# Ryan-Faulkner/Simultaneous-Diffusion-for-Pointclouds

Hardware: AMD Instinct MI355X
Metric: Langevin denoising steps/sec on 64×1024 range images, 1/2/4/8 MI355X (higher is better)
Workload: dtype fp32x3; 1 GPU; Line.yml simultaneous sampling step (score-net fwd + Langevin update + consistency merge), 64x1024x2 range images; views_per_gpu=4, megabatch_views=4, mode=viewsplit, conv_arithmetic=fp32x3, parallelism=views1

## Files before the change

simultaneous-diffusion-for-pointclouds_amd/csrc/common.h:

```cpp
#pragma once
#include <hip/hip_runtime.h>
#include <stdint.h>
#include <stdlib.h>

#include <type_traits>

#define SDP_DEV __device__ __forceinline__

typedef __attribute__((ext_vector_type(8))) __bf16 bf16x8;
typedef __attribute__((ext_vector_type(4))) __bf16 bf16x4;
typedef __attribute__((ext_vector_type(16))) float f32x16;
typedef __attribute__((ext_vector_type(4))) float f32x4;

namespace sdp {

template <int B, int E, class F>
SDP_DEV void static_for(F&& f) {
  if constexpr (B < E) {
    f(std::integral_constant<int, B>{});
    static_for<B + 1, E>(f);
  }
}

enum { MODE_F32 = 0, MODE_F32X3 = 1, MODE_BF16 = 2 };
enum { PRO_NONE = 0, PRO_ELU = 1, PRO_AFFINE_ELU = 2 };

typedef __attribute__((ext_vector_type(4))) int i32x4;
SDP_DEV i32x4 buffer_desc(const void* base, uint32_t bytes) {
  const uint64_t p = reinterpret_cast<uint64_t>(base);
  return i32x4{__builtin_amdgcn_readfirstlane((int)(uint32_t)p), __builtin_amdgcn_readfirstlane((int)((p >> 32) & 0xffff)),
               __builtin_amdgcn_readfirstlane((int)bytes), 0x00020000};
}
SDP_DEV void dma16_lds_opaque(i32x4 rsrc, uint32_t lds_byte, int voff, int soff) {
  asm volatile("s_mov_b32 m0, %0\n\ts_nop 0\n\tbuffer_load_dwordx4 %1, %2, %3 offen lds"
               :
               : "s"(__builtin_amdgcn_readfirstlane((int)lds_byte)), "v"(voff), "s"(rsrc),
                 "s"(__builtin_amdgcn_readfirstlane(soff))
               : "memory");
}

SDP_DEV float4 ldg4(const float* p, size_t i) { return *reinterpret_cast<const float4*>(p + i); }
SDP_DEV float4 bf4_to_f4(uint2 u) {
  return make_float4(__uint_as_float(u.x << 16), __uint_as_float(u.x & 0xffff0000u), __uint_as_float(u.y << 16),
                     __uint_as_float(u.y & 0xffff0000u));
}
SDP_DEV float4 ldg4(const __bf16* p, size_t i) { return bf4_to_f4(*reinterpret_cast<const uint2*>(p + i)); }
SDP_DEV uint32_t pack_bf2(float a, float b) {
  typedef __attribute__((ext_vector_type(2))) __bf16 bf16x2_t;
  const bf16x2_t v = {(__bf16)a, (__bf16)b};
  return __builtin_bit_cast(uint32_t, v);
}
SDP_DEV uint2 f4_to_bf4(float4 v) { return make_uint2(pack_bf2(v.x, v.y), pack_bf2(v.z, v.w)); }
SDP_DEV void stg4(float* p, size_t i, float4 v) { *reinterpret_cast<float4*>(p + i) = v; }
SDP_DEV void stg4(__bf16* p, size_t i, float4 v) { *reinterpret_cast<uint2*>(p + i) = f4_to_bf4(v); }
SDP_DEV float ldg1(const float* p, size_t i) { return p[i]; }
SDP_DEV float ldg1(const __bf16* p, size_t i) { return (float)p[i]; }

SDP_DEV float elu(float x) { return x > 0.f ? x : (__expf(x) - 1.0f); }
SDP_DEV float elu_max(float x) { return fmaxf(x, __expf(fminf(x, 0.f)) - 1.0f); }
SDP_DEV float elu_grad(float t, int form) {
  if (form == 2) return t > 0.f ? 1.f : t + 1.f;
  return t > 0.f ? 1.f : __expf(t);
}

struct ConvArgs {
  const float* in;
  const uint4* wf;
  const uint4* wf16;
  const float* bias;
  float* out;
  const float* res;
  float* out2;
  const float* res2;
  const float* up;
  const float* pro_ss;
  int ss_bstride;
  float* stats;
  int B, H, W, Cin, Cout;
  int dil, circular, pro_mode, epi_elu;
  int tiles_per_img;
  int strip_w;
  int groups_per_img;
  int cpair;
  unsigned long long* dbg;
  const float* aux;
  const float* epi_ss;
  int dact;
  int io16;
};

struct WgradArgs {
  const float* in;
  const float* pro_ss;
  int ss_bstride;
  int pro_mode;
  const float* dy;
  float* part;
  size_t part_floats;
  float* bpart;
  int B, H, W, Cin, Cout, dil, circular;
};

inline int conv_strip_w(int tile_rows, int tile_cols) {
  int sw = 1;
  while (sw * 2 * tile_rows <= 32 && tile_cols % (sw * 2) == 0) sw *= 2;
  return sw;
}

}
```

simultaneous-diffusion-for-pointclouds_amd/csrc/conv.hip:

```cpp
#include "conv_launch.h"

namespace sdp {

#ifndef SDP_CONV_NJ2
#define SDP_CONV_NJ2 1
#endif
#ifndef SDP_CONV_NJ2_BF16_W8
#define SDP_CONV_NJ2_BF16_W8 1
#endif

template <int MODE, bool PELU>
static hipError_t launch_elu(const ConvArgs& a, int ks, bool pool, int wm, int tc, bool half, hipStream_t st) {
  if (ks == 1)
    return pool ? conv_launch<MODE, 1, 64, 1, true, PELU>(a, st) : conv_launch<MODE, 1, 64, 1, false, PELU>(a, st);
  if (pool) return conv_launch<MODE, 1, 64, 3, true, PELU>(a, st);
  if constexpr (MODE != MODE_F32) {
    if (half) return SDP_CONV_NJ2 ? conv_launch_nj2<MODE, PELU, 4>(a, st) : conv_launch_half<MODE, PELU>(a, st);
    if (tc == 16) {
      if (!SDP_CONV_NJ2) return conv_launch<MODE, 1, 16, 3, false, PELU>(a, st);
      return (MODE == MODE_BF16 && SDP_CONV_NJ2_BF16_W8) ? conv_launch_nj2<MODE, PELU, 8>(a, st)
                                                         : conv_launch_nj2<MODE, PELU, 4>(a, st);
    }
  }
  if (wm == 2) return conv_launch<MODE, 2, 32, 3, false, PELU>(a, st);
  return tc == 64 ? conv_launch<MODE, 1, 64, 3, false, PELU>(a, st) : conv_launch<MODE, 1, 32, 3, false, PELU>(a, st);
}

template <int MODE>
static hipError_t launch_mode(const ConvArgs& a, int ks, bool pool, int wm, int tc, hipStream_t st, bool half = false) {
#ifdef SDP_CONV_BENCH_ONLY
  if constexpr (MODE != MODE_F32) {
    if (half) return SDP_CONV_NJ2 ? conv_launch_nj2<MODE, true, 4>(a, st) : conv_launch_half<MODE, true>(a, st);
    if (!SDP_CONV_NJ2) return conv_launch<MODE, 1, 16, 3, false, true>(a, st);
    return (MODE == MODE_BF16 && SDP_CONV_NJ2_BF16_W8) ? conv_launch_nj2<MODE, true, 8>(a, st)
                                                       : conv_launch_nj2<MODE, true, 4>(a, st);
  }
  if (wm == 2) return conv_launch<MODE, 2, 32, 3, false, true>(a, st);
  return conv_launch<MODE, 1, 32, 3, false, true>(a, st);
#else
  return a.pro_mode == PRO_NONE ? launch_elu<MODE, false>(a, ks, pool, wm, tc, half, st)
                                : launch_elu<MODE, true>(a, ks, pool, wm, tc, half, st);
#endif
}

hipError_t conv_mfma(int mode, ConvArgs a, int ks, bool pool, hipStream_t st, const char** why) {
  const int d = a.dil;
  if (a.Cin % 64 || a.Cout % 128) { *why = "conv: Cin%64 and Cout%128 required"; return hipErrorInvalidValue; }
  if (a.H % d || a.W % d) { *why = "conv: H,W must be multiples of the dilation"; return hipErrorInvalidValue; }
  const int Hs = a.H / d, Ws = a.W / d;
  const int wm = (a.Cout % 256 == 0) ? 1 : 2;
  const bool sh16 = mode != MODE_F32;
  int tc;
  if (sh16 && Ws % 16 == 0 && Hs % 8 == 0) tc = 16;
  else if (wm == 2) tc = 32;
  else tc = (Ws % 32 == 0 && Hs % 4 == 0) ? 32 : 64;
  if (!sh16 && tc == 16) tc = 32;
  if (ks == 1 || pool) tc = 64;
  const bool half = sh16 && wm == 2 && tc == 16 && ks == 3 && !pool;
  const int tr = (half ? 128 : wm * 128) / tc;
  if (Ws % tc || Hs % tr) { *why = "conv: sub-grid not divisible by the pixel tile"; return hipErrorInvalidValue; }
  if (sh16 && !a.wf16) { *why = "conv: bf16 modes need the 16x16 weight packing (#frag16)"; return hipErrorInvalidValue; }
  if (!sh16 && !a.wf) { *why = "conv: exact fp32 needs the 32x32 weight packing (#frag)"; return hipErrorInvalidValue; }
  if (ks == 1 && !pool && (d != 1 || wm != 1)) { *why = "conv: 1x1 needs d=1 and 256-multiple Cout"; return hipErrorInvalidValue; }
  if (pool && (d != 1 || wm != 1 || (a.H & 1) || (a.W & 1))) {
    *why = "conv: pooling needs d=1, even H,W and 256-multiple Cout";
    return hipErrorInvalidValue;
  }
  if (a.up && ((a.H & 1) || (a.W & 1) || a.H < 2 || a.W < 2)) { *why = "conv: upsample needs even H,W"; return hipErrorInvalidValue; }
  if (!a.circular && d != 1) { *why = "conv: zero padding only for d=1"; return hipErrorInvalidValue; }
  if (!a.pro_ss) { *why = "conv: prologue scale/shift table missing"; return hipErrorInvalidValue; }
  if (a.Cin > 1024 && a.ss_bstride == 0) { *why = "conv: identity table holds 1024 channels"; return hipErrorInvalidValue; }
  if (a.io16) {
#ifdef SDP_CONV_BENCH_ONLY
    if (mode == MODE_BF16 && ks == 3 && tc == 16 && !pool) return conv_launch_nj2<MODE_BF16, true, 4, true>(a, st);
#else
    if (mode != MODE_BF16) { *why = "conv: bf16 tensors (io16) need bf16 mode"; return hipErrorInvalidValue; }
    const bool pe = a.pro_mode != PRO_NONE;
    if (pool && ks == 1) return pe ? conv_launch<MODE_BF16, 1, 64, 1, true, true, true>(a, st)
                                   : conv_launch<MODE_BF16, 1, 64, 1, true, false, true>(a, st);
    if (pool) return pe ? conv_launch<MODE_BF16, 1, 64, 3, true, true, true>(a, st)
                        : conv_launch<MODE_BF16, 1, 64, 3, true, false, true>(a, st);
    if (ks == 3 && tc == 16)
      return pe ? conv_launch_nj2<MODE_BF16, true, 4, true>(a, st) : conv_launch_nj2<MODE_BF16, false, 4, true>(a, st);
#endif
    *why = "conv: no bf16-tensor (io16) kernel for this shape";
    return hipErrorInvalidValue;
  }
  switch (mode) {
    case MODE_F32: return launch_mode<MODE_F32>(a, ks, pool, wm, tc, st);
    case MODE_F32X3: return launch_mode<MODE_F32X3>(a, ks, pool, wm, tc, st, half);
    default: return launch_mode<MODE_BF16>(a, ks, pool, wm, tc, st, half);
  }
}

}
```

simultaneous-diffusion-for-pointclouds_amd/csrc/conv_inst.hip:

```cpp
#include "conv_kernel.h"
#include "conv_launch.h"

namespace sdp {


#ifndef SDP_FWD_TRN
#define SDP_FWD_TRN 0
#endif

#ifndef SDP_CONV_CPAIR
#define SDP_CONV_CPAIR 1
#endif

#ifndef SDP_NJ2_STRIP
#define SDP_NJ2_STRIP 1
#endif

template <int MODE, int WM, int TC, int KS, bool POOL, bool PELU, bool IO16>
hipError_t conv_launch(ConvArgs a, hipStream_t st) {
  using T = ConvTile<WM, TC, KS, 4, 4, IO16>;
  a.tiles_per_img = a.H * a.W / (T::TR * TC);
  a.groups_per_img = a.H * a.W / 128;
  a.strip_w = conv_strip_w(a.H / a.dil / T::TR, a.W / a.dil / TC);
  dim3 grid(a.B * a.tiles_per_img, a.Cout / T::NTILE);
  if constexpr (MODE != MODE_F32) {
    hipLaunchKernelGGL((conv_mfma_kernel<MODE, WM, TC, KS, POOL, POOL, PELU, 16, 4, (SDP_FWD_TRN && TC == 16 && !POOL), 4, IO16>),
                       grid, dim3(256), 0, st, a);
    return hipGetLastError();
  } else if constexpr (TC >= 32) {
    hipLaunchKernelGGL((conv_mfma_kernel<MODE, WM, TC, KS, POOL, POOL, PELU>), grid, dim3(256), 0, st, a);
    return hipGetLastError();
  }
  return hipErrorInvalidValue;
}

template <int MODE, bool PELU>
hipError_t conv_launch_half(ConvArgs a, hipStream_t st) {
  using T = ConvTile<1, 16, 3, 2>;
  a.tiles_per_img = a.H * a.W / (T::TR * 16);
  a.groups_per_img = a.H * a.W / 128;
  a.strip_w = 0;
  dim3 grid(a.B * a.tiles_per_img, a.Cout / T::NTILE);
  hipLaunchKernelGGL((conv_mfma_kernel<MODE, 1, 16, 3, false, false, PELU, 16, 2, (SDP_FWD_TRN != 0)>), grid,
                     dim3(T::NTH), 0, st, a);
  return hipGetLastError();
}

template <int MODE, bool PELU, int NW, bool IO16>
hipError_t conv_launch_nj2(ConvArgs a, hipStream_t st) {
  using T = ConvTile<1, 16, 3, NW, 2, IO16>;
  a.tiles_per_img = a.H * a.W / (T::TR * 16);
  a.groups_per_img = a.H * a.W / 128;
  a.cpair = (SDP_CONV_CPAIR && a.Cout == 2 * T::NTILE) ? 1 : 0;
  const bool strip = NW == 8 || SDP_NJ2_STRIP == 2 || (SDP_NJ2_STRIP == 1 && a.cpair);
  a.strip_w = strip ? conv_strip_w(a.H / a.dil / T::TR, a.W / a.dil / 16) : 0;
  dim3 grid(a.B * a.tiles_per_img * (a.cpair ? 2 : 1), a.cpair ? 1 : a.Cout / T::NTILE);
  hipLaunchKernelGGL((conv_mfma_kernel<MODE, 1, 16, 3, false, false, PELU, 16, NW, false, 2, IO16>), grid, dim3(T::NTH), 0,
                     st, a);
  return hipGetLastError();
}

template <int MODE, int WM, int TC, int KS, bool ZP, bool IO16>
hipError_t dgrad_launch(ConvArgs a, hipStream_t st) {
  using T = ConvTile<WM, TC, KS, 4, 4, IO16>;
  a.tiles_per_img = a.H * a.W / (T::TR * TC);
  a.groups_per_img = a.H * a.W / 128;
  dim3 grid(a.B * a.tiles_per_img, a.Cout / T::NTILE);
  if constexpr (TC < 32) {
    hipLaunchKernelGGL((conv_mfma_kernel<MODE, WM, TC, KS, false, ZP, false, 16, 4, true, 4, IO16>), grid, dim3(256), 0, st, a);
  } else {
    hipLaunchKernelGGL((conv_mfma_kernel<MODE, WM, TC, KS, false, ZP, false, 16, 4, false, 4, IO16>), grid, dim3(256), 0, st, a);
  }
  return hipGetLastError();
}

template <int S> struct FwdShape;
template <> struct FwdShape<0> { static constexpr int WM = 1, TC = 64, KS = 1; static constexpr bool POOL = true; };
template <> struct FwdShape<1> { static constexpr int WM = 1, TC = 64, KS = 3; static constexpr bool POOL = true; };
template <> struct FwdShape<2> { static constexpr int WM = 2, TC = 32, KS = 3; static constexpr bool POOL = false; };
template <> struct FwdShape<3> { static constexpr int WM = 1, TC = 64, KS = 3; static constexpr bool POOL = false; };
template <> struct FwdShape<4> { static constexpr int WM = 1, TC = 32, KS = 3; static constexpr bool POOL = false; };
template <> struct FwdShape<5> { static constexpr int WM = 1, TC = 16, KS = 3; static constexpr bool POOL = false; };
template <> struct FwdShape<8> { static constexpr int WM = 1, TC = 64, KS = 1; static constexpr bool POOL = false; };
template <int MODE>
hipError_t dgrad_launch_half(ConvArgs a, hipStream_t st) {
  using T = ConvTile<1, 16, 3, 2>;
  a.tiles_per_img = a.H * a.W / (T::TR * 16);
  a.groups_per_img = a.H * a.W / 128;
  dim3 grid(a.B * a.tiles_per_img, a.Cout / T::NTILE);
  hipLaunchKernelGGL((conv_mfma_kernel<MODE, 1, 16, 3, false, false, false, 16, 2, true>), grid, dim3(T::NTH), 0, st, a);
  return hipGetLastError();
}

template <int MODE, int NW, bool IO16>
hipError_t dgrad_launch_nj2(ConvArgs a, hipStream_t st) {
  using T = ConvTile<1, 16, 3, NW, 2, IO16>;
  a.tiles_per_img = a.H * a.W / (T::TR * 16);
  a.groups_per_img = a.H * a.W / 128;
  dim3 grid(a.B * a.tiles_per_img, a.Cout / T::NTILE);
  hipLaunchKernelGGL((conv_mfma_kernel<MODE, 1, 16, 3, false, false, false, 16, NW, true, 2, IO16>), grid, dim3(T::NTH), 0,
                     st, a);
  return hipGetLastError();
}

template <int S> struct DgradShape;
template <> struct DgradShape<0> { static constexpr int WM = 2, TC = 32, KS = 1; static constexpr bool ZP = false; };
template <> struct DgradShape<1> { static constexpr int WM = 2, TC = 32, KS = 3; static constexpr bool ZP = true; };
template <> struct DgradShape<2> { static constexpr int WM = 2, TC = 32, KS = 3; static constexpr bool ZP = false; };
template <> struct DgradShape<3> { static constexpr int WM = 1, TC = 64, KS = 3; static constexpr bool ZP = false; };
template <> struct DgradShape<4> { static constexpr int WM = 1, TC = 32, KS = 3; static constexpr bool ZP = false; };
template <> struct DgradShape<5> { static constexpr int WM = 1, TC = 16, KS = 3; static constexpr bool ZP = false; };

#if defined(SDP_INST) && SDP_INST >= 3000
constexpr int kS = SDP_INST % 10;
static_assert(kS == 0 || kS == 1 || kS == 7 || kS == 8, "SDP_INST: bad IO16 dgrad code");
#if SDP_INST % 10 == 0
template hipError_t dgrad_launch<MODE_BF16, 2, 32, 1, false, true>(ConvArgs, hipStream_t);
#elif SDP_INST % 10 == 1
template hipError_t dgrad_launch<MODE_BF16, 2, 32, 3, true, true>(ConvArgs, hipStream_t);
#else
template hipError_t dgrad_launch_nj2<MODE_BF16, kS == 7 ? 4 : 8, true>(ConvArgs, hipStream_t);
#endif
#elif defined(SDP_INST) && SDP_INST >= 2000
constexpr int kPelu = (SDP_INST / 10) % 10, kS = SDP_INST % 10;
static_assert(kPelu <= 1 && (kS == 0 || kS == 1 || kS == 6 || kS == 9), "SDP_INST: bad IO16 forward code");
#if SDP_INST % 10 == 0
template hipError_t conv_launch<MODE_BF16, 1, 64, 1, true, (kPelu != 0), true>(ConvArgs, hipStream_t);
#elif SDP_INST % 10 == 1
template hipError_t conv_launch<MODE_BF16, 1, 64, 3, true, (kPelu != 0), true>(ConvArgs, hipStream_t);
#else
template hipError_t conv_launch_nj2<MODE_BF16, (kPelu != 0), kS == 9 ? 4 : 8, true>(ConvArgs, hipStream_t);
#endif
#elif defined(SDP_INST) && SDP_INST < 1000 && (SDP_INST % 10 == 6 || SDP_INST % 10 == 9)
constexpr int kMode = SDP_INST / 100 - 1, kPelu = (SDP_INST / 10) % 10;
static_assert(kMode >= 1 && kMode <= 2 && kPelu <= 1, "SDP_INST: bad 32-Cout-wave forward code");
template hipError_t conv_launch_nj2<kMode, (kPelu != 0), SDP_INST % 10 == 9 ? 4 : 8>(ConvArgs, hipStream_t);
#elif defined(SDP_INST) && SDP_INST < 1000 && SDP_INST % 10 == 7
constexpr int kMode = SDP_INST / 100 - 1, kPelu = (SDP_INST / 10) % 10;
static_assert(kMode >= 1 && kMode <= 2 && kPelu <= 1, "SDP_INST: bad 2-wave forward code");
template hipError_t conv_launch_half<kMode, (kPelu != 0)>(ConvArgs, hipStream_t);
#elif defined(SDP_INST) && SDP_INST < 1000
constexpr int kMode = SDP_INST / 100 - 1, kPelu = (SDP_INST / 10) % 10, kShape = SDP_INST % 10;
static_assert(kMode >= 0 && kMode <= 2 && kPelu <= 1 && (kShape <= 5 || kShape == 8) &&
                  (kShape < 5 || kShape == 8 || kMode != MODE_F32),
              "SDP_INST: bad forward code");
using FS = FwdShape<kShape>;
template hipError_t conv_launch<kMode, FS::WM, FS::TC, FS::KS, FS::POOL, (kPelu != 0)>(ConvArgs, hipStream_t);
#elif defined(SDP_INST) && (SDP_INST % 10 == 7 || SDP_INST % 10 == 8)
constexpr int kMode = (SDP_INST / 10) % 10;
static_assert(SDP_INST / 100 == 10 && (kMode == MODE_F32X3 || kMode == MODE_BF16), "SDP_INST: bad dgrad code");
template hipError_t dgrad_launch_nj2<kMode, SDP_INST % 10 == 7 ? 4 : 8>(ConvArgs, hipStream_t);
#elif defined(SDP_INST) && SDP_INST % 10 == 6
constexpr int kMode = (SDP_INST / 10) % 10;
static_assert(SDP_INST / 100 == 10 && (kMode == MODE_F32X3 || kMode == MODE_BF16), "SDP_INST: bad dgrad code");
template hipError_t dgrad_launch_half<kMode>(ConvArgs, hipStream_t);
#elif defined(SDP_INST)
constexpr int kMode = (SDP_INST / 10) % 10, kShape = SDP_INST % 10;
static_assert(SDP_INST / 100 == 10 && (kMode == MODE_F32X3 || kMode == MODE_BF16) && kShape <= 5,
              "SDP_INST: bad dgrad code");
using DS = DgradShape<kShape>;
template hipError_t dgrad_launch<kMode, DS::WM, DS::TC, DS::KS, DS::ZP>(ConvArgs, hipStream_t);
#elif defined(SDP_CONV_BENCH_ONLY)
template hipError_t conv_launch<MODE_F32, 2, 32, 3, false, true>(ConvArgs, hipStream_t);
template hipError_t conv_launch<MODE_F32, 1, 32, 3, false, true>(ConvArgs, hipStream_t);
template hipError_t conv_launch<MODE_F32X3, 1, 16, 3, false, true>(ConvArgs, hipStream_t);
template hipError_t conv_launch<MODE_BF16, 1, 16, 3, false, true>(ConvArgs, hipStream_t);
template hipError_t conv_launch_half<MODE_F32X3, true>(ConvArgs, hipStream_t);
template hipError_t conv_launch_half<MODE_BF16, true>(ConvArgs, hipStream_t);
template hipError_t conv_launch_nj2<MODE_F32X3, true, 4>(ConvArgs, hipStream_t);
template hipError_t conv_launch_nj2<MODE_F32X3, true, 8>(ConvArgs, hipStream_t);
template hipError_t conv_launch_nj2<MODE_BF16, true, 4>(ConvArgs, hipStream_t);
template hipError_t conv_launch_nj2<MODE_BF16, true, 8>(ConvArgs, hipStream_t);
template hipError_t conv_launch_nj2<MODE_BF16, true, 4, true>(ConvArgs, hipStream_t);
template hipError_t dgrad_launch_nj2<MODE_BF16, 4, true>(ConvArgs, hipStream_t);
#else
#error "conv_inst.hip: build with -DSDP_INST=<code> (Makefile) or -DSDP_CONV_BENCH_ONLY (tools/conv_bench)"
#endif

}
```

simultaneous-diffusion-for-pointclouds_amd/csrc/conv_kernel.h:

```cpp
#pragma once
#include <type_traits>

#include "common.h"

namespace sdp {

#ifndef SDP_KO
#define SDP_KO 0
#endif

#ifndef SDP_DMA_AUX
#define SDP_DMA_AUX 0
#endif
#ifndef SDP_STORE_AUX
#define SDP_STORE_AUX 0
#endif
#ifndef SDP_STORE_AUX16
#define SDP_STORE_AUX16 SDP_STORE_AUX
#endif

#ifdef SDP_TIMING
#define SDP_T(i) do { if (tid == 0) tclk[i] = __builtin_amdgcn_s_memtime(); } while (0)
#else
#define SDP_T(i) do { } while (0)
#endif

constexpr int PSTRIDE = 144;

template <int WM, int TC, int KS, int NW = 4, int NJ = 4, bool IO16 = false>
struct ConvTile {
  static constexpr int NTH = 64 * NW;
  static constexpr int WN = NW / WM;
  static constexpr int RW = 128 / TC;
  static constexpr int TR = WM * RW;
  static constexpr int NTILE = WN * 16 * NJ;
  static constexpr int WPC = 4 * (NJ == 2 ? 2 : 1) / NW;
  static constexpr int HALO = KS == 3 ? 1 : 0;
  static constexpr int PC = TC + 2 * HALO;
  static constexpr int PR = TR + 2 * HALO;
  static constexpr int NPIX = PR * PC;
  static constexpr int UPP = IO16 ? 4 : 8;
  static constexpr int NU = (NPIX * UPP + NTH - 1) / NTH;
  static constexpr int PATCH_BYTES = NU * (NTH / UPP) * PSTRIDE;
  static constexpr int RAW_BYTES = NU * NTH * 16;
  static constexpr int PIPE_BYTES = 2 * PATCH_BYTES + RAW_BYTES;
  static constexpr int EPI_BYTES = WM * 64 * (NTILE + 8) * 4;
  static constexpr int LDS_BYTES = PIPE_BYTES > EPI_BYTES ? PIPE_BYTES : EPI_BYTES;
  static_assert(LDS_BYTES * WPC <= 160 * 1024, "LDS budget (WPC workgroups per CU)");
};

SDP_DEV float4 ld4(const float* p) { return *reinterpret_cast<const float4*>(p); }

template <int NU, int NT, int NSTG_ = 5>
struct XformPlan {
  static constexpr int tap_of(int k) { return k * NT / NU; }
  static constexpr int first(int tap) {
    int k = 0;
    while (k < NU && tap_of(k) < tap) ++k;
    return k;
  }
  static constexpr int count(int tap) {
    int n = 0;
    for (int k = 0; k < NU; ++k) n += tap_of(k) == tap ? 1 : 0;
    return n;
  }
  static constexpr int max_count() {
    int m = 0;
    for (int t = 0; t < NT; ++t) m = count(t) > m ? count(t) : m;
    return m;
  }
  static constexpr int NSTG = NSTG_;
  static constexpr int stage_blk(int q, int Q, int NBLK) { return 2 + q * (NBLK - 2) / (Q > 0 ? Q : 1); }
};

template <int MODE, int WM, int TC, int KS, bool POOL, bool ZP, bool PELU, int SH = 32, int NW = 4, bool TRN = false,
          int NJ = 4, bool IO16 = false>
__global__ __launch_bounds__(64 * NW, NJ == 2 ? 2 : 1) void conv_mfma_kernel(ConvArgs a) {
#if defined(__HIP_DEVICE_COMPILE__)
  static_assert(!IO16 || MODE == MODE_BF16, "the bf16 tape runs in bf16 mode");
  constexpr int ES = IO16 ? 2 : 4;
  constexpr int CPU = IO16 ? 8 : 4;
  constexpr int USH = IO16 ? 2 : 3;
  constexpr int PPU = CPU / 2;
  constexpr bool COPY = IO16 && !PELU;
  static_assert((SH == 32) == (MODE == MODE_F32), "bf16 modes: 16x16 shape; exact fp32: 32x32");
  static_assert(NW == 4 || (SH == 16 && !POOL), "2-wave workgroups: the 16x16 non-pooled forward only");
  static_assert(NJ == 4 || (SH == 16 && !POOL && KS == 3 && WM == 1), "32-Cout waves: the 16x16 3x3 tiles only");
  using T = ConvTile<WM, TC, KS, NW, NJ, IO16>;
  constexpr int NTH = T::NTH;
  constexpr int NT = KS * KS;
  constexpr bool TRANS = TRN && SH == 16 && !POOL;
  constexpr int NU = T::NU;
  constexpr int XT = NT >= 4 ? 4 : NT;
  __shared__ __attribute__((aligned(16))) char lds[T::LDS_BYTES];
  char* const raw = lds + 2 * T::PATCH_BYTES;

  const int tid = threadIdx.x, lane = tid & 63, wave = tid >> 6;
#ifdef SDP_TIMING
  unsigned long long tclk[8] = {0, 0, 0, 0, 0, 0, 0, 0};
  unsigned long long tbar = 0;
  const unsigned long long rt0 = __builtin_amdgcn_s_memrealtime();
#endif
  SDP_T(0);
  const int wm = WM == 1 ? 0 : (wave & 1), wn = WM == 1 ? wave : (wave >> 1);
  const int d = a.dil, Hs = a.H / d, Ws = a.W / d;
  const int tiles_c = Ws / TC, tiles_rc = (Hs / T::TR) * tiles_c;
  const int nwg = gridDim.x;
  int t = (nwg & 7) ? (int)blockIdx.x : ((int)blockIdx.x & 7) * (nwg >> 3) + ((int)blockIdx.x >> 3);
  const int cblk = a.cpair ? (t & 1) : (int)blockIdx.y;
  if (a.cpair) t >>= 1;
  const int b = t / a.tiles_per_img;
  const int tile = t - b * a.tiles_per_img;
  t = tile;
  const int ph = t / tiles_rc;
  t -= ph * tiles_rc;
  const int ph_r = ph / d, ph_c = ph - (ph / d) * d;
  int trow, tcol;
  if (a.strip_w) {
    const int R = Hs / T::TR, sw = a.strip_w;
    const int strip = t / (R * sw), w_ = t - strip * (R * sw);
    trow = w_ / sw;
    tcol = strip * sw + (w_ - trow * sw);
  } else {
    trow = t / tiles_c;
    tcol = t % tiles_c;
  }
  const int sr0 = trow * T::TR, sc0 = tcol * TC;
  const int n0 = cblk * T::NTILE;
  const int wrow0 = wm * T::RW;

  const int Cin = a.Cin, Cout = a.Cout;
  const int nchunks = Cin / 32;
  const int NB = Cout / 32;
  const int f0 = n0 / 16 + wn * NJ;
  const int nbg0 = f0 / 2;

  f32x16 acc[4][2];
  f32x4 acc4[8][NJ];
  if constexpr (SH == 32) {
    static_for<0, 4>([&](auto i) {
      static_for<0, 2>([&](auto j) {
#pragma unroll
        for (int r = 0; r < 16; ++r) acc[i][j][r] = 0.f;
      });
    });
  } else {
    static_for<0, 8>([&](auto i) {
      static_for<0, NJ>([&](auto j) {
#pragma unroll
        for (int r = 0; r < 4; ++r) acc4[i][j][r] = 0.f;
      });
    });
  }

  const bool c16 = SH == 16 && a.wf16 != nullptr;
  const __amdgpu_buffer_rsrc_t wrs =
      __builtin_amdgcn_make_buffer_rsrc((void*)(c16 ? a.wf16 : a.wf), 0, 0x7fffffff, 0x00020000);
  const int wv0 = ((nbg0 + 0) * 64 + lane) * 64, wv1 = ((nbg0 + 1) * 64 + lane) * 64;
  typedef __attribute__((ext_vector_type(4))) unsigned u32x4;
  constexpr int NBUF = (NT % 3 == 0) ? 3 : 2;
  uint4 bq[NBUF][NJ / 2][4];
  int wq16[NJ];
  const int wlo16 = __builtin_amdgcn_readfirstlane(c16 ? 1024 : 16);
  {
    const int g = lane >> 4, h = g & 1, sg = g >> 1;
    static_for<0, NJ>([&](auto njc) {
      constexpr int nj = decltype(njc)::value;
      const int L = 16 * (nj & 1) + (lane & 15) + 32 * h;
      wq16[nj] = c16 ? ((f0 + nj) * 128 + lane) * 16 : ((nbg0 + (nj >> 1)) * 64 + L) * 64 + sg * 32;
    });
  }
  auto load_b = [&](auto buf, int chunk, int tap) __attribute__((always_inline)) {
    constexpr int J = decltype(buf)::value;
    if constexpr (SDP_KO & 4) return;
    const int so = __builtin_amdgcn_readfirstlane(((chunk * NT + tap) * NB) * 4096);
    if constexpr (SH == 32) {
      static_for<0, 4>([&](auto q) {
        const u32x4 v0 = __builtin_amdgcn_raw_buffer_load_b128(wrs, wv0 + q * 16, so, 0);
        const u32x4 v1 = __builtin_amdgcn_raw_buffer_load_b128(wrs, wv1 + q * 16, so, 0);
        bq[J][0][q] = make_uint4(v0.x, v0.y, v0.z, v0.w);
        bq[J][1][q] = make_uint4(v1.x, v1.y, v1.z, v1.w);
      });
    } else {
      static_for<0, NJ>([&](auto njc) {
        constexpr int nj = decltype(njc)::value;
        const u32x4 vh = __builtin_amdgcn_raw_buffer_load_b128(wrs, wq16[nj], so, 0);
        bq[J][nj >> 1][2 * (nj & 1)] = make_uint4(vh.x, vh.y, vh.z, vh.w);
        if constexpr (MODE != MODE_BF16) {
          const u32x4 vl = __builtin_amdgcn_raw_buffer_load_b128(wrs, wq16[nj] + wlo16, so, 0);
          bq[J][nj >> 1][2 * (nj & 1) + 1] = make_uint4(vl.x, vl.y, vl.z, vl.w);
        }
      });
    }
  };

  const char* inb = reinterpret_cast<const char*>(a.in) + (size_t)b * a.H * a.W * Cin * ES;
  const float* ssb = a.pro_ss + (size_t)b * a.ss_bstride;
  const int my_cv = tid & (T::UPP - 1);
  float4 ssv[2][PPU];
  auto load_ss = [&](auto buf, int chunk) __attribute__((always_inline)) {
    constexpr int SB = decltype(buf)::value;
    static_for<0, PPU>([&](auto kc) { ssv[SB][kc] = ld4(ssb + (chunk * 32 + my_cv * CPU) * 2 + 4 * decltype(kc)::value); });
  };

  const __amdgpu_buffer_rsrc_t irs =
      __builtin_amdgcn_make_buffer_rsrc((void*)inb, 0, a.H * a.W * Cin * ES, 0x00020000);
  int uoff[NU];
  unsigned uvalid = 0;
  static_for<0, NU>([&](auto kc) {
    constexpr int k = decltype(kc)::value;
    int u = tid + k * NTH;
    bool valid = u < T::NPIX * T::UPP;
    u = valid ? u : 0;
    const int pix = u >> USH, cv = u & (T::UPP - 1);
    const int pr = pix / T::PC, pc = pix - pr * T::PC;
    int sr = sr0 - T::HALO + pr, sc = sc0 - T::HALO + pc;
    if (a.circular) {
      sr = sr < 0 ? sr + Hs : (sr >= Hs ? sr - Hs : sr);
      sc = sc < 0 ? sc + Ws : (sc >= Ws ? sc - Ws : sc);
    } else {
      valid = valid && sr >= 0 && sr < Hs && sc >= 0 && sc < Ws;
      sr = min(max(sr, 0), Hs - 1);
      sc = min(max(sc, 0), Ws - 1);
    }
    const int y = sr * d + ph_r, x = sc * d + ph_c;
    uoff[k] = ((y * a.W + x) * Cin + cv * CPU) * ES;
    uvalid |= (valid ? 1u : 0u) << k;
  });
  auto load_unit = [&](auto kc, int chunk) __attribute__((always_inline)) {
    constexpr int k = decltype(kc)::value;
    if constexpr (SDP_KO & 1) return;
    const int base = __builtin_amdgcn_readfirstlane(((tid & ~63) + k * NTH) * 16);
    __builtin_amdgcn_raw_ptr_buffer_load_lds(
        irs, reinterpret_cast<__attribute__((address_space(3))) void*>(reinterpret_cast<uintptr_t>(raw + base)), 16,
        uoff[k], chunk * 32 * ES, 0, SDP_DMA_AUX);
  };
  const i32x4 irs_o = buffer_desc(inb, (uint32_t)(a.H * a.W * Cin * ES));
  auto load_unit_o = [&](auto kc, int chunk) __attribute__((always_inline)) {
    constexpr int k = decltype(kc)::value;
    if constexpr (SDP_KO & 1) return;
    const uint32_t base = (uint32_t)(uintptr_t)(raw + ((tid & ~63) + k * NTH) * 16);
    dma16_lds_opaque(irs_o, base, uoff[k], chunk * 32 * ES);
  };
  auto xform_load = [&](auto kc) __attribute__((always_inline)) {
    constexpr int k = decltype(kc)::value;
    return *reinterpret_cast<const float4*>(raw + (tid + k * NTH) * 16);
  };
  auto xform_store = [&](auto kc, auto pb, float4 v) __attribute__((always_inline)) {
    constexpr int k = decltype(kc)::value;
    constexpr int PB = decltype(pb)::value;
    const int pix = (tid + k * NTH) >> USH;
    if constexpr (COPY) {
      uint4 u = __builtin_bit_cast(uint4, v);
      if constexpr (ZP) {
        if (!((uvalid >> k) & 1u)) u = make_uint4(0u, 0u, 0u, 0u);
      }
      *reinterpret_cast<uint4*>(lds + PB * T::PATCH_BYTES + pix * PSTRIDE + my_cv * 16) = u;
      return;
    }
    if constexpr (IO16) {
      const uint4 u = __builtin_bit_cast(uint4, v);
      const float4 lo = bf4_to_f4(make_uint2(u.x, u.y)), hi = bf4_to_f4(make_uint2(u.z, u.w));
      float x8[8] = {lo.x, lo.y, lo.z, lo.w, hi.x, hi.y, hi.z, hi.w};
#pragma unroll
      for (int e = 0; e < 8; ++e) {
        const float4 sv = ssv[PB][e >> 1];
        x8[e] = fmaf(x8[e], (e & 1) ? sv.z : sv.x, (e & 1) ? sv.w : sv.y);
        if constexpr (PELU) x8[e] = elu_max(x8[e]);
        if constexpr (ZP) {
          if (!((uvalid >> k) & 1u)) x8[e] = 0.f;
        }
      }
      *reinterpret_cast<uint4*>(lds + PB * T::PATCH_BYTES + pix * PSTRIDE + my_cv * 16) =
          make_uint4(pack_bf2(x8[0], x8[1]), pack_bf2(x8[2], x8[3]), pack_bf2(x8[4], x8[5]), pack_bf2(x8[6], x8[7]));
      return;
    }
    const float4 ssv0 = ssv[PB][0], ssv1 = ssv[PB][1];
    v.x = fmaf(v.x, ssv0.x, ssv0.y);
    v.y = fmaf(v.y, ssv0.z, ssv0.w);
    v.z = fmaf(v.z, ssv1.x, ssv1.y);
    v.w = fmaf(v.w, ssv1.z, ssv1.w);
    if constexpr (PELU) {
      v.x = elu_max(v.x); v.y = elu_max(v.y); v.z = elu_max(v.z); v.w = elu_max(v.w);
    }
    if constexpr (ZP) {
      if (!((uvalid >> k) & 1u)) v = make_float4(0.f, 0.f, 0.f, 0.f);
    }
    char* dst = lds + PB * T::PATCH_BYTES + pix * PSTRIDE;
    if constexpr (MODE == MODE_F32) {
      *reinterpret_cast<float4*>(dst + my_cv * 16) = v;
    } else {
      bf16x4 hi;
      hi[0] = (__bf16)v.x; hi[1] = (__bf16)v.y; hi[2] = (__bf16)v.z; hi[3] = (__bf16)v.w;
      *reinterpret_cast<bf16x4*>(dst + my_cv * 8) = hi;
      if constexpr (MODE == MODE_F32X3) {
        bf16x4 lo;
        lo[0] = (__bf16)(v.x - (float)hi[0]);
        lo[1] = (__bf16)(v.y - (float)hi[1]);
        lo[2] = (__bf16)(v.z - (float)hi[2]);
        lo[3] = (__bf16)(v.w - (float)hi[3]);
        *reinterpret_cast<bf16x4*>(dst + 64 + my_cv * 8) = lo;
      }
    }
  };
  auto xform_unit = [&](auto kc, auto pb) __attribute__((always_inline)) { xform_store(kc, pb, xform_load(kc)); };
  auto xform_piece = [&](auto kc, auto hc, auto pb, float4 v4) __attribute__((always_inline)) {
    constexpr int k = decltype(kc)::value, h = decltype(hc)::value, PB = decltype(pb)::value;
    if constexpr (SDP_KO & 2) return;
    const int pix = (tid + k * NTH) >> USH;
    float x0, x1;
    if constexpr (IO16) {
      const uint32_t w = __float_as_uint(h == 0 ? v4.x : h == 1 ? v4.y : h == 2 ? v4.z : v4.w);
      x0 = __uint_as_float(w << 16);
      x1 = __uint_as_float(w & 0xffff0000u);
    } else {
      x0 = h ? v4.z : v4.x;
      x1 = h ? v4.w : v4.y;
    }
    const float4 sv = ssv[PB][h];
    x0 = fmaf(x0, sv.x, sv.y);
    x1 = fmaf(x1, sv.z, sv.w);
    if constexpr (PELU) {
      x0 = elu_max(x0);
      x1 = elu_max(x1);
    }
    if constexpr (ZP) {
      const bool ok = (uvalid >> k) & 1u;
      x0 = ok ? x0 : 0.f;
      x1 = ok ? x1 : 0.f;
    }
    typedef __attribute__((ext_vector_type(2))) __bf16 bf16x2;
    bf16x2 hi;
    hi[0] = (__bf16)x0;
    hi[1] = (__bf16)x1;
    char* dst = lds + PB * T::PATCH_BYTES + pix * PSTRIDE + my_cv * (2 * CPU) + h * 4;
    *reinterpret_cast<bf16x2*>(dst) = hi;
    if constexpr (MODE == MODE_F32X3) {
      bf16x2 lo;
      lo[0] = (__bf16)(x0 - (float)hi[0]);
      lo[1] = (__bf16)(x1 - (float)hi[1]);
      *reinterpret_cast<bf16x2*>(dst + 64) = lo;
    }
  };

  SDP_T(1);
  load_b(std::integral_constant<int, 0>{}, 0, 0);
  static_for<1, NBUF - 1>([&](auto j) { load_b(j, 0, decltype(j)::value); });
  load_ss(std::integral_constant<int, 0>{}, 0);
  static_for<0, NU>([&](auto k) { load_unit(k, 0); });
  static_for<0, NU>([&](auto k) { xform_unit(k, std::integral_constant<int, 0>{}); });
  if (nchunks > 1) {
    load_ss(std::integral_constant<int, 1>{}, 1);
    static_for<0, NU>([&](auto k) { load_unit(k, 1); });
  }
  __syncthreads();
  SDP_T(2);

  const int a_lane_off16 = (lane & 15) * PSTRIDE + (lane >> 4) * 16;
  auto read_a = [&](const char* pat, auto tap_c, auto s_c, bf16x8* hi, bf16x8* lo) __attribute__((always_inline)) {
    constexpr int tap = decltype(tap_c)::value, s = decltype(s_c)::value;
    constexpr int kh = (KS == 3) ? tap / 3 : 0, kw = (KS == 3) ? tap % 3 : 0;
    static_for<0, 4>([&](auto mbc) {
      constexpr int i = decltype(mbc)::value, mb = 4 * s + i;
      constexpr int mr = mb / (TC / 16), mc = (mb % (TC / 16)) * 16;
      const char* src = pat + ((wrow0 + mr + kh) * T::PC + mc + kw) * PSTRIDE + a_lane_off16;
      hi[i] = *reinterpret_cast<const bf16x8*>(src);
      if constexpr (MODE == MODE_F32X3) lo[i] = *reinterpret_cast<const bf16x8*>(src + 64);
    });
  };

  auto do_chunk = [&](auto parity, int chunk) __attribute__((always_inline)) {
    constexpr int P = decltype(parity)::value;
    const char* pat = lds + P * T::PATCH_BYTES;
    bf16x8 pre_hi[4], pre_lo[4];
    if constexpr (MODE != MODE_F32) read_a(pat, std::integral_constant<int, 0>{}, std::integral_constant<int, 0>{},
                                           pre_hi, pre_lo);
    static_for<0, NT>([&](auto tap_c) {
      constexpr int tap = decltype(tap_c)::value;
      constexpr int DIST = NBUF - 1;
      constexpr int CUR = NBUF >= 3 ? tap % NBUF : (tap + P) & 1;
      constexpr int NXT = NBUF >= 3 ? (tap + DIST) % NBUF : (tap + 1 + P) & 1;
      if constexpr (tap + DIST < NT) load_b(std::integral_constant<int, NXT>{}, chunk, tap + DIST);
      else load_b(std::integral_constant<int, NXT>{}, min(chunk + 1, nchunks - 1), tap + DIST - NT);
      __builtin_amdgcn_sched_barrier(0);
      constexpr int NX = (tap < XT) ? (NU - tap + XT - 1) / XT : 0;
      float4 xv[NX > 0 ? NX : 1];
      auto xform_loads = [&]() __attribute__((always_inline)) {
        static_for<0, NX>([&](auto j) { xv[j] = xform_load(std::integral_constant<int, tap + XT * j>{}); });
      };
      auto xform_stores = [&]() __attribute__((always_inline)) {
        static_for<0, NX>([&](auto j) {
          xform_store(std::integral_constant<int, tap + XT * j>{}, std::integral_constant<int, 1 - P>{}, xv[j]);
        });
      };
      auto dmas = [&]() __attribute__((always_inline)) {
        if constexpr (tap == NT - 1) load_ss(std::integral_constant<int, P>{}, min(chunk + 2, nchunks - 1));
        static_for<0, NU>([&](auto kc) {
          constexpr int dt = NT > XT ? XT : 0;
          if constexpr (dt == tap) load_unit(kc, chunk + 2);
        });
      };
      if constexpr (MODE == MODE_F32) {
        xform_loads();
        xform_stores();
        if constexpr (NT == 1) __builtin_amdgcn_sched_barrier(0);
        dmas();
        const int kh = (KS == 3) ? tap / 3 : 0, kw = (KS == 3) ? tap % 3 : 0;
#pragma unroll
        for (int half = 0; half < 2; ++half) {
          float av[4][8];
          static_for<0, 4>([&](auto mbc) {
            constexpr int mb = decltype(mbc)::value;
            constexpr int mr = mb / (TC / 32), mc = (mb % (TC / 32)) * 32;
            const int pix = (wrow0 + mr + kh) * T::PC + mc + (lane & 31) + kw;
            const char* src = pat + pix * PSTRIDE + (lane >> 5) * 64 + half * 32;
            const float4 f0 = *reinterpret_cast<const float4*>(src);
            const float4 f1 = *reinterpret_cast<const float4*>(src + 16);
            av[mb][0] = f0.x; av[mb][1] = f0.y; av[mb][2] = f0.z; av[mb][3] = f0.w;
            av[mb][4] = f1.x; av[mb][5] = f1.y; av[mb][6] = f1.z; av[mb][7] = f1.w;
          });
#pragma unroll
          for (int kk = 0; kk < 8; ++kk) {
            const int k = half * 8 + kk;
            static_for<0, 2>([&](auto nbc) {
              constexpr int nb = decltype(nbc)::value;
              const uint4 bv = bq[CUR][nb][k >> 2];
              const uint32_t bw = (k & 3) == 0 ? bv.x : (k & 3) == 1 ? bv.y : (k & 3) == 2 ? bv.z : bv.w;
              const float bf = __uint_as_float(bw);
              static_for<0, 4>([&](auto mbc) {
                constexpr int mb = decltype(mbc)::value;
                acc[mb][nb] = __builtin_amdgcn_mfma_f32_32x32x2f32(av[mb][kk], bf, acc[mb][nb], 0, 0, 0);
              });
            });
          }
        }
      } else {
        float4 xv[NX > 0 ? NX : 1];
        static_for<0, NX>([&](auto j) { xv[j] = xform_load(std::integral_constant<int, tap + XT * j>{}); });
        bf16x8 c0_hi[4], c0_lo[4], c1_hi[4], c1_lo[4];
        static_for<0, 4>([&](auto mb) {
          c0_hi[mb] = pre_hi[mb];
          if constexpr (MODE == MODE_F32X3) c0_lo[mb] = pre_lo[mb];
        });
        read_a(pat, tap_c, std::integral_constant<int, 1>{}, c1_hi, c1_lo);
        if constexpr (tap + 1 < NT)
          read_a(pat, std::integral_constant<int, tap + 1>{}, std::integral_constant<int, 0>{}, pre_hi, pre_lo);
        if constexpr (NT > 1) dmas();
        constexpr int NBLK = 8 * NJ;
        static_for<0, NBLK>([&](auto blk_c) {
          constexpr int blk = decltype(blk_c)::value;
          {
            constexpr int s = blk / (4 * NJ), nj = (blk / 4) % NJ, i = blk & 3, mb = 4 * s + i;
            const uint4 h4 = bq[CUR][nj >> 1][2 * (nj & 1)], l4 = bq[CUR][nj >> 1][2 * (nj & 1) + 1];
            const bf16x8 bhi = *reinterpret_cast<const bf16x8*>(&h4);
            const bf16x8 blo = *reinterpret_cast<const bf16x8*>(&l4);
            const bf16x8 ahi = s == 0 ? c0_hi[i] : c1_hi[i];
            if constexpr (TRANS) {
              if constexpr (MODE == MODE_F32X3) {
                const bf16x8 alo = s == 0 ? c0_lo[i] : c1_lo[i];
                acc4[mb][nj] = __builtin_amdgcn_mfma_f32_16x16x32_bf16(bhi, alo, acc4[mb][nj], 0, 0, 0);
                acc4[mb][nj] = __builtin_amdgcn_mfma_f32_16x16x32_bf16(blo, ahi, acc4[mb][nj], 0, 0, 0);
              }
              acc4[mb][nj] = __builtin_amdgcn_mfma_f32_16x16x32_bf16(bhi, ahi, acc4[mb][nj], 0, 0, 0);
            } else {
              if constexpr (MODE == MODE_F32X3) {
                const bf16x8 alo = s == 0 ? c0_lo[i] : c1_lo[i];
                acc4[mb][nj] = __builtin_amdgcn_mfma_f32_16x16x32_bf16(alo, bhi, acc4[mb][nj], 0, 0, 0);
                acc4[mb][nj] = __builtin_amdgcn_mfma_f32_16x16x32_bf16(ahi, blo, acc4[mb][nj], 0, 0, 0);
              }
              acc4[mb][nj] = __builtin_amdgcn_mfma_f32_16x16x32_bf16(ahi, bhi, acc4[mb][nj], 0, 0, 0);
            }
          }
          if constexpr (COPY) {
            if constexpr (blk < NX) xform_store(std::integral_constant<int, tap + XT * blk>{}, std::integral_constant<int, 1 - P>{},
                                                xv[blk]);
          } else if constexpr (blk < PPU * NX) {
            xform_piece(std::integral_constant<int, tap + XT * (blk / PPU)>{}, std::integral_constant<int, blk % PPU>{},
                        std::integral_constant<int, 1 - P>{}, xv[blk / PPU]);
          }
          __builtin_amdgcn_sched_barrier(0);
        });
        if constexpr (NT == 1) dmas();
      }
    });
#ifdef SDP_TIMING
    const unsigned long long tb0 = __builtin_amdgcn_s_memtime();
#endif
    __builtin_amdgcn_s_waitcnt(0xc07f);
    if constexpr (!(SDP_KO & 8)) __builtin_amdgcn_s_barrier();
#ifdef SDP_TIMING
    tbar += __builtin_amdgcn_s_memtime() - tb0;
#endif
  };
  using XP = XformPlan<NU, NT, (MODE == MODE_BF16 && !IO16) ? 8 : 5>;
  constexpr int NQ = MODE == MODE_F32X3 ? 8 : 4;
  constexpr int NWL = NJ * (MODE == MODE_F32X3 ? 2 : 1);
  constexpr int NBLK = 8 * NJ;
  static_assert(NQ <= NBLK / 2 && 2 * NWL <= NBLK, "the tap's fillers fit its blocks");
  using I0 = std::integral_constant<int, 0>;
  using I1 = std::integral_constant<int, 1>;
  auto read_a1 = [&](const char* pat, auto tap_c, auto s_c, auto i_c, auto lo_c) __attribute__((always_inline)) {
    constexpr int tap = decltype(tap_c)::value, s = decltype(s_c)::value, i = decltype(i_c)::value;
    constexpr int kh = tap / 3, kw = tap % 3, mb = 4 * s + i;
    constexpr int mr = mb / (TC / 16), mc = (mb % (TC / 16)) * 16;
    return *reinterpret_cast<const bf16x8*>(pat + ((wrow0 + mr + kh) * T::PC + mc + kw) * PSTRIDE + a_lane_off16 +
                                            (decltype(lo_c)::value ? 64 : 0));
  };
  auto load_b1 = [&](auto buf, auto q_c, int chunk, int tap) __attribute__((always_inline)) {
    constexpr int J = decltype(buf)::value, q = decltype(q_c)::value;
    constexpr int nj = MODE == MODE_F32X3 ? (q >> 1) : q, part = MODE == MODE_F32X3 ? (q & 1) : 0;
    if constexpr (SDP_KO & 4) return;
    const int so = __builtin_amdgcn_readfirstlane(((chunk * NT + tap) * NB) * 4096 + (part ? wlo16 : 0));
    const u32x4 v = __builtin_amdgcn_raw_buffer_load_b128(wrs, wq16[nj], so, 0);
    bq[J][nj >> 1][2 * (nj & 1) + part] = make_uint4(v.x, v.y, v.z, v.w);
  };
  auto do_chunk9 = [&](auto parity, int chunk) __attribute__((always_inline)) {
    constexpr int P = decltype(parity)::value;
    const char* pat = lds + P * T::PATCH_BYTES;
    bf16x8 ca[2][4], cb[2][4];
    static_for<0, 4>([&](auto i) {
      ca[0][i] = read_a1(pat, I0{}, I0{}, i, I0{});
      if constexpr (MODE == MODE_F32X3) ca[1][i] = read_a1(pat, I0{}, I0{}, i, I1{});
    });
    load_ss(std::integral_constant<int, P>{}, min(chunk + 2, nchunks - 1));
    static_for<0, NT>([&](auto tap_c) {
      constexpr int tap = decltype(tap_c)::value;
      constexpr int CUR = tap % 3, NXT = (tap + 2) % 3;
      constexpr int U0 = XP::first(tap), UN = XP::count(tap), Q = COPY ? UN : UN * PPU * XP::NSTG;
      constexpr int UNA = UN > 0 ? UN : 1;
      const int wchunk = tap + 2 < NT ? chunk : min(chunk + 1, nchunks - 1);
      constexpr int wtap = tap + 2 < NT ? tap + 2 : tap + 2 - NT;
      float4 xr[UNA];
      float py0[PPU * UNA], py1[PPU * UNA], pe0[PPU * UNA], pe1[PPU * UNA];
      uint32_t phi[PPU * UNA], plo[PPU * UNA];
      auto stage = [&](auto pc_c, auto st_c) __attribute__((always_inline)) {
        constexpr int pc = decltype(pc_c)::value, st = decltype(st_c)::value;
        constexpr int j = pc / PPU, h = pc % PPU, k = U0 + j, PB = 1 - P;
        if constexpr (SDP_KO & 2) return;
        if constexpr (COPY) {
          xform_store(std::integral_constant<int, U0 + decltype(pc_c)::value>{}, std::integral_constant<int, PB>{},
                      xr[decltype(pc_c)::value]);
          return;
        }
        auto raw2 = [&](float& r0, float& r1) __attribute__((always_inline)) {
          const float4 v = xr[j];
          if constexpr (IO16) {
            const uint32_t w = __float_as_uint(h == 0 ? v.x : h == 1 ? v.y : h == 2 ? v.z : v.w);
            r0 = __uint_as_float(w << 16);
            r1 = __uint_as_float(w & 0xffff0000u);
          } else {
            r0 = h ? v.z : v.x;
            r1 = h ? v.w : v.y;
          }
        };
        if constexpr (XP::NSTG == 8) {
          const float4 v = xr[j];
          const float4 sv = ssv[PB][h];
          if constexpr (st == 0) {
            py0[pc] = fmaf(h ? v.z : v.x, sv.x, sv.y);
            if constexpr (PELU) pe0[pc] = fminf(py0[pc], 0.f);
          } else if constexpr (st == 1) {
            py1[pc] = fmaf(h ? v.w : v.y, sv.z, sv.w);
            if constexpr (PELU) pe1[pc] = fminf(py1[pc], 0.f);
          } else if constexpr (st == 2) {
            if constexpr (PELU) pe0[pc] = __expf(pe0[pc]);
          } else if constexpr (st == 3) {
            if constexpr (PELU) pe1[pc] = __expf(pe1[pc]);
          } else if constexpr (st == 4) {
            if constexpr (PELU) py0[pc] = fmaxf(py0[pc], pe0[pc] - 1.0f);
            if constexpr (ZP) py0[pc] = ((uvalid >> k) & 1u) ? py0[pc] : 0.f;
          } else if constexpr (st == 5) {
            if constexpr (PELU) py1[pc] = fmaxf(py1[pc], pe1[pc] - 1.0f);
            if constexpr (ZP) py1[pc] = ((uvalid >> k) & 1u) ? py1[pc] : 0.f;
          } else if constexpr (st == 6) {
            typedef __attribute__((ext_vector_type(2))) __bf16 bf16x2;
            bf16x2 hi;
            hi[0] = (__bf16)py0[pc];
            hi[1] = (__bf16)py1[pc];
            phi[pc] = *reinterpret_cast<const uint32_t*>(&hi);
          } else {
            const int pix = (tid + k * NTH) >> 3;
            *reinterpret_cast<uint32_t*>(lds + PB * T::PATCH_BYTES + pix * PSTRIDE + my_cv * 8 + h * 4) = phi[pc];
          }
          return;
        }
        if constexpr (st == 0) {
          float r0, r1;
          raw2(r0, r1);
          const float4 sv = ssv[PB][h];
          py0[pc] = fmaf(r0, sv.x, sv.y);
          py1[pc] = fmaf(r1, sv.z, sv.w);
          if constexpr (PELU) {
            pe0[pc] = fminf(py0[pc], 0.f);
            pe1[pc] = fminf(py1[pc], 0.f);
          }
        } else if constexpr (st == 1) {
          if constexpr (PELU) {
            pe0[pc] = __expf(pe0[pc]);
            pe1[pc] = __expf(pe1[pc]);
          }
        } else if constexpr (st == 2) {
          if constexpr (PELU) {
            py0[pc] = fmaxf(py0[pc], pe0[pc] - 1.0f);
            py1[pc] = fmaxf(py1[pc], pe1[pc] - 1.0f);
          }
          if constexpr (ZP) {
            const bool ok = (uvalid >> k) & 1u;
            py0[pc] = ok ? py0[pc] : 0.f;
            py1[pc] = ok ? py1[pc] : 0.f;
          }
        } else if constexpr (st == 3) {
          typedef __attribute__((ext_vector_type(2))) __bf16 bf16x2;
          bf16x2 hi;
          hi[0] = (__bf16)py0[pc];
          hi[1] = (__bf16)py1[pc];
          phi[pc] = *reinterpret_cast<const uint32_t*>(&hi);
          if constexpr (MODE == MODE_F32X3) {
            bf16x2 lo;
            lo[0] = (__bf16)(py0[pc] - (float)hi[0]);
            lo[1] = (__bf16)(py1[pc] - (float)hi[1]);
            plo[pc] = *reinterpret_cast<const uint32_t*>(&lo);
          }
        } else {
          const int pix = (tid + k * NTH) >> USH;
          char* dst = lds + PB * T::PATCH_BYTES + pix * PSTRIDE + my_cv * (2 * CPU) + h * 4;
          *reinterpret_cast<uint32_t*>(dst) = phi[pc];
          if constexpr (MODE == MODE_F32X3) *reinterpret_cast<uint32_t*>(dst + 64) = plo[pc];
        }
      };
      static_for<0, NBLK>([&](auto blk_c) {
        constexpr int blk = decltype(blk_c)::value;
        constexpr int s = blk / (4 * NJ), nj = (blk / 4) % NJ, i = blk & 3, mb = 4 * s + i;
        if constexpr (blk < UN) xr[blk] = xform_load(std::integral_constant<int, U0 + blk>{});
        {
          const uint4 h4 = bq[CUR][nj >> 1][2 * (nj & 1)], l4 = bq[CUR][nj >> 1][2 * (nj & 1) + 1];
          const bf16x8 bhi = *reinterpret_cast<const bf16x8*>(&h4);
          const bf16x8 blo = *reinterpret_cast<const bf16x8*>(&l4);
          const bf16x8 ahi = s == 0 ? ca[0][i] : cb[0][i];
          if constexpr (TRANS) {
            if constexpr (MODE == MODE_F32X3) {
              const bf16x8 alo = s == 0 ? ca[1][i] : cb[1][i];
              acc4[mb][nj] = __builtin_amdgcn_mfma_f32_16x16x32_bf16(bhi, alo, acc4[mb][nj], 0, 0, 0);
              acc4[mb][nj] = __builtin_amdgcn_mfma_f32_16x16x32_bf16(blo, ahi, acc4[mb][nj], 0, 0, 0);
            }
            acc4[mb][nj] = __builtin_amdgcn_mfma_f32_16x16x32_bf16(bhi, ahi, acc4[mb][nj], 0, 0, 0);
          } else {
            if constexpr (MODE == MODE_F32X3) {
              const bf16x8 alo = s == 0 ? ca[1][i] : cb[1][i];
              acc4[mb][nj] = __builtin_amdgcn_mfma_f32_16x16x32_bf16(alo, bhi, acc4[mb][nj], 0, 0, 0);
              acc4[mb][nj] = __builtin_amdgcn_mfma_f32_16x16x32_bf16(ahi, blo, acc4[mb][nj], 0, 0, 0);
            }
            acc4[mb][nj] = __builtin_amdgcn_mfma_f32_16x16x32_bf16(ahi, bhi, acc4[mb][nj], 0, 0, 0);
          }
        }
        if constexpr (blk < NQ) {
          constexpr int q = blk, ii = MODE == MODE_F32X3 ? (q >> 1) : q, lo = MODE == MODE_F32X3 ? (q & 1) : 0;
          cb[lo][ii] = read_a1(pat, tap_c, I1{}, std::integral_constant<int, ii>{}, std::integral_constant<int, lo>{});
        }
        if constexpr ((blk & 1) && (blk >> 1) < NWL)
          load_b1(std::integral_constant<int, NXT>{}, std::integral_constant<int, (blk >> 1)>{}, wchunk, wtap);
        if constexpr (tap + 1 < NT && blk >= NBLK / 2 && blk < NBLK / 2 + NQ) {
          constexpr int q = blk - NBLK / 2, ii = MODE == MODE_F32X3 ? (q >> 1) : q, lo = MODE == MODE_F32X3 ? (q & 1) : 0;
          ca[lo][ii] = read_a1(pat, std::integral_constant<int, tap + 1>{}, I0{}, std::integral_constant<int, ii>{},
                               std::integral_constant<int, lo>{});
        }
        static_for<0, Q>([&](auto q_c) {
          constexpr int q = decltype(q_c)::value;
          if constexpr (XP::stage_blk(q, Q, NBLK) == blk) {
            if constexpr (COPY) stage(std::integral_constant<int, q>{}, std::integral_constant<int, 0>{});
            else stage(std::integral_constant<int, q / XP::NSTG>{}, std::integral_constant<int, q % XP::NSTG>{});
          }
        });
        if constexpr (UN > 0 && blk >= NBLK - UN)
          load_unit_o(std::integral_constant<int, U0 + blk - (NBLK - UN)>{}, chunk + 2);
        __builtin_amdgcn_sched_barrier(0);
      });
    });
    __builtin_amdgcn_s_waitcnt(0xc07f);
    if constexpr (!(SDP_KO & 8)) __builtin_amdgcn_s_barrier();
  };
  static_assert(NT % 2 == 1, "parity bookkeeping assumes an odd tap count");
#ifndef SDP_DGRAD16_TAPS
#define SDP_DGRAD16_TAPS 0
#endif
  if constexpr (MODE != MODE_F32 && NT == 9 && (!TRANS || (IO16 && SDP_DGRAD16_TAPS))) {
    static_assert(XP::max_count() * PPU * XP::NSTG <= 2 * (NBLK - 2), "at most two transform stages per block");
    for (int chunk = 0; chunk < nchunks; chunk += 2) {
      do_chunk9(std::integral_constant<int, 0>{}, chunk);
      do_chunk9(std::integral_constant<int, 1>{}, chunk + 1);
    }
  } else {
    for (int chunk = 0; chunk < nchunks; chunk += 2) {
      do_chunk(std::integral_constant<int, 0>{}, chunk);
      do_chunk(std::integral_constant<int, 1>{}, chunk + 1);
    }
  }

  SDP_T(3);
  if (TRANS && (!a.dact || TC < 32 || NW != 4)) {
    if constexpr (TRANS) {
    __builtin_amdgcn_s_waitcnt(0);
    const int Ho = a.H, Wo = a.W;
    const size_t bo = (size_t)b * Ho * Wo * Cout;
    const int img_bytes = Ho * Wo * Cout * ES;
    auto rs = [&](const float* p) {
      return __builtin_amdgcn_make_buffer_rsrc((void*)(reinterpret_cast<const char*>(p) + bo * ES), 0, img_bytes, 0x00020000);
    };
    const int lq = lane >> 4, lcol = lane & 15;
    constexpr int CB = TC / 16;
    const int voff = (lcol * d * Cout + 4 * lq) * ES;
    auto soff = [&](int mb, int nj) {
      const int mr = mb / CB, mc = (mb % CB) * 16;
      const int y = (sr0 + wrow0 + mr) * d + ph_r, x = (sc0 + mc) * d + ph_c;
      return __builtin_amdgcn_readfirstlane(((y * Wo + x) * Cout + n0 + wn * 16 * NJ + nj * 16) * ES);
    };
    auto ld = [&](__amdgpu_buffer_rsrc_t r, int so) {
      if constexpr (IO16) {
        typedef __attribute__((ext_vector_type(2))) unsigned u32x2;
        const u32x2 q = __builtin_amdgcn_raw_buffer_load_b64(r, voff, so, 0);
        return bf4_to_f4(make_uint2(q.x, q.y));
      } else {
        const u32x4 q = __builtin_amdgcn_raw_buffer_load_b128(r, voff, so, 0);
        return make_float4(__uint_as_float(q.x), __uint_as_float(q.y), __uint_as_float(q.z), __uint_as_float(q.w));
      }
    };
    auto st = [&](float4 v, __amdgpu_buffer_rsrc_t r, int so, auto aux_c) {
      constexpr int AUX = decltype(aux_c)::value;
      if constexpr (IO16) {
        typedef __attribute__((ext_vector_type(2))) unsigned u32x2;
        const uint2 w = f4_to_bf4(v);
        __builtin_amdgcn_raw_buffer_store_b64(u32x2{w.x, w.y}, r, voff, so, AUX);
      } else {
        const u32x4 q = {__float_as_uint(v.x), __float_as_uint(v.y), __float_as_uint(v.z), __float_as_uint(v.w)};
        __builtin_amdgcn_raw_buffer_store_b128(q, r, voff, so, AUX);
      }
    };
    auto rs_or_out = [&](const float* p) { return rs(p ? p : a.out); };
    const __amdgpu_buffer_rsrc_t ors = rs(a.out), xrs = rs_or_out(a.aux), rrs = rs_or_out(a.res), o2rs = rs_or_out(a.out2),
                                 r2rs = rs_or_out(a.res2);
    static_for<0, NJ>([&](auto njc) {
      constexpr int nj = decltype(njc)::value;
      __builtin_amdgcn_sched_barrier(0);
      const int co0 = n0 + wn * 16 * NJ + nj * 16 + 4 * lq;
      float4 hq[8], rq[8], s0 = make_float4(1.f, 0.f, 1.f, 0.f), s1 = s0;
      if (a.dact) static_for<0, 8>([&](auto mb) { hq[mb] = ld(xrs, soff(mb, nj)); });
      if (a.dact == 3) {
        s0 = ld4(a.epi_ss + ((size_t)b * Cout + co0) * 2);
        s1 = ld4(a.epi_ss + ((size_t)b * Cout + co0) * 2 + 4);
      }
      if (a.res) static_for<0, 8>([&](auto mb) { rq[mb] = ld(rrs, soff(mb, nj)); });
      const float4 bias4 = a.bias ? ld4(a.bias + co0) : make_float4(0.f, 0.f, 0.f, 0.f);
      const float4 esc = make_float4(s0.x, s0.z, s1.x, s1.z), esh = make_float4(s0.y, s0.w, s1.y, s1.w);
      float4 v[8];
      static_for<0, 8>([&](auto mbc) {
        constexpr int mb = decltype(mbc)::value;
        const f32x4 q = acc4[mb][nj];
        v[mb] = make_float4(q[0] + bias4.x, q[1] + bias4.y, q[2] + bias4.z, q[3] + bias4.w);
      });
      if (a.up) {
        const int Hi = a.H / 2, Wi = a.W / 2;
        const float shh = (float)(Hi - 1) / (float)(a.H - 1), sww = (float)(Wi - 1) / (float)(a.W - 1);
        const size_t ub = (size_t)b * Hi * Wi * Cout + co0;
        auto lup = [&](size_t e) { return IO16 ? ldg4(reinterpret_cast<const __bf16*>(a.up), e) : ldg4(a.up, e); };
#pragma unroll
        for (int mb = 0; mb < 8; ++mb) {
          const int mr = mb / CB, mc = (mb % CB) * 16;
          const int y = (sr0 + wrow0 + mr) * d + ph_r, x = (sc0 + mc + lcol) * d + ph_c;
          const float fy = shh * (float)y, fx = sww * (float)x;
          const int y0 = (int)fy, x0 = (int)fx;
          const int yp = y0 < Hi - 1 ? 1 : 0, xp = x0 < Wi - 1 ? 1 : 0;
          const float ly1 = fy - (float)y0, ly0 = 1.f - ly1, lx1 = fx - (float)x0, lx0 = 1.f - lx1;
          const float4 v00 = lup(ub + ((size_t)y0 * Wi + x0) * Cout), v01 = lup(ub + ((size_t)y0 * Wi + x0 + xp) * Cout);
          const float4 v10 = lup(ub + ((size_t)(y0 + yp) * Wi + x0) * Cout);
          const float4 v11 = lup(ub + ((size_t)(y0 + yp) * Wi + x0 + xp) * Cout);
          auto bil = [&](float a00, float a01, float a10, float a11) {
            return ly0 * (lx0 * a00 + lx1 * a01) + ly1 * (lx0 * a10 + lx1 * a11);
          };
          v[mb].x = v[mb].x + bil(v00.x, v01.x, v10.x, v11.x);
          v[mb].y = v[mb].y + bil(v00.y, v01.y, v10.y, v11.y);
          v[mb].z = v[mb].z + bil(v00.z, v01.z, v10.z, v11.z);
          v[mb].w = v[mb].w + bil(v00.w, v01.w, v10.w, v11.w);
        }
      }
      if (a.dact) {
        static_for<0, 8>([&](auto mbc) {
          constexpr int mb = decltype(mbc)::value;
          float4 h = hq[mb];
          if (a.dact == 3) h = make_float4(fmaf(h.x, esc.x, esh.x), fmaf(h.y, esc.y, esh.y), fmaf(h.z, esc.z, esh.z),
                                           fmaf(h.w, esc.w, esh.w));
          v[mb] = make_float4(v[mb].x * elu_grad(h.x, a.dact), v[mb].y * elu_grad(h.y, a.dact),
                              v[mb].z * elu_grad(h.z, a.dact), v[mb].w * elu_grad(h.w, a.dact));
        });
      }
      if (a.res) {
        static_for<0, 8>([&](auto mbc) {
          constexpr int mb = decltype(mbc)::value;
          const float4 r = rq[mb];
          v[mb] = make_float4(r.x + v[mb].x, r.y + v[mb].y, r.z + v[mb].z, r.w + v[mb].w);
        });
      }
      if (a.out2) {
        static_for<0, 8>([&](auto mbc) {
          constexpr int mb = decltype(mbc)::value;
          const float4 r2 = ld(r2rs, soff(mb, nj));
          st(make_float4(v[mb].x + r2.x, v[mb].y + r2.y, v[mb].z + r2.z, v[mb].w + r2.w), o2rs, soff(mb, nj),
             std::integral_constant<int, 0>{});
        });
      }
      if (a.epi_elu) {
#pragma unroll
        for (int mb = 0; mb < 8; ++mb) v[mb] = make_float4(elu(v[mb].x), elu(v[mb].y), elu(v[mb].z), elu(v[mb].w));
      }
      if constexpr (!(SDP_KO & 16)) {
        static_for<0, 8>([&](auto mbc) {
          constexpr int mb = decltype(mbc)::value;
          st(v[mb], ors, soff(mb, nj), std::integral_constant<int, IO16 ? SDP_STORE_AUX16 : SDP_STORE_AUX>{});
        });
      }
      if (a.stats) {
        float mean[4], m2[4];
        static_for<0, 4>([&](auto rc) {
          constexpr int r = decltype(rc)::value;
          auto comp = [&](const float4& q) { return r == 0 ? q.x : r == 1 ? q.y : r == 2 ? q.z : q.w; };
          float s = 0.f;
#pragma unroll
          for (int mb = 0; mb < 8; ++mb) s += comp(v[mb]);
          mean[r] = s * 0.125f;
          float q2 = 0.f;
#pragma unroll
          for (int mb = 0; mb < 8; ++mb) {
            const float dv = comp(v[mb]) - mean[r];
            q2 = fmaf(dv, dv, q2);
          }
          m2[r] = q2;
        });
        auto merge = [&](auto ctl_c, float n) {
          constexpr int CTL = decltype(ctl_c)::value;
#pragma unroll
          for (int r = 0; r < 4; ++r) {
            const float mp = __int_as_float(__builtin_amdgcn_mov_dpp(__float_as_int(mean[r]), CTL, 0xf, 0xf, false));
            const float qp = __int_as_float(__builtin_amdgcn_mov_dpp(__float_as_int(m2[r]), CTL, 0xf, 0xf, false));
            const float dm = mean[r] - mp;
            m2[r] = m2[r] + qp + dm * dm * (0.5f * n);
            mean[r] = 0.5f * (mean[r] + mp);
          }
        };
        merge(std::integral_constant<int, 0xB1>{}, 8.f);
        merge(std::integral_constant<int, 0x4E>{}, 16.f);
        merge(std::integral_constant<int, 0x141>{}, 32.f);
        merge(std::integral_constant<int, 0x140>{}, 64.f);
        if (lcol == 0) {
          float4* sp = reinterpret_cast<float4*>(reinterpret_cast<float2*>(a.stats) +
                                                 ((size_t)b * a.groups_per_img + tile * WM + wm) * Cout + co0);
          sp[0] = make_float4(mean[0], m2[0], mean[1], m2[1]);
          sp[1] = make_float4(mean[2], m2[2], mean[3], m2[3]);
        }
      }
    });
    }
  } else if (SH == 16 && !TRANS && (!a.dact || TC < 32 || NW != 4)) {
    if constexpr (SH == 16 && !TRANS) {
    __builtin_amdgcn_s_waitcnt(0);
    const int Ho = POOL ? a.H / 2 : a.H, Wo = POOL ? a.W / 2 : a.W;
    const size_t bo = (size_t)b * Ho * Wo * Cout;
    const int img_bytes = Ho * Wo * Cout * ES;
    auto rs = [&](const float* p) {
      return __builtin_amdgcn_make_buffer_rsrc((void*)(reinterpret_cast<const char*>(p ? p : a.out) + bo * ES), 0, img_bytes,
                                               0x00020000);
    };
    const __amdgpu_buffer_rsrc_t ors = rs(a.out), rrs = rs(a.res), o2rs = rs(a.out2), r2rs = rs(a.res2), xrs = rs(a.aux);
    const int lq = lane >> 4, lcol = lane & 15;
    constexpr int CB = TC / 16;
    constexpr int NF = POOL ? CB : 8;
    constexpr int PER = POOL ? 2 : 4;
    constexpr int NV = NF * PER;
    const int xs = (POOL ? 1 : d) * Cout * ES;
    int vbase[NF];
    static_for<0, NF>([&](auto fc) {
      constexpr int f = decltype(fc)::value;
      const int co = n0 + wn * 16 * NJ + lcol;
      if constexpr (POOL) {
        vbase[f] = (((sr0 >> 1) * Wo + ((sc0 + f * 16) >> 1) + 2 * lq) * Cout + co) * ES;
      } else {
        constexpr int mr = f / CB, mc = (f % CB) * 16;
        const int y = (sr0 + wrow0 + mr) * d + ph_r, x = (sc0 + mc + 4 * lq) * d + ph_c;
        vbase[f] = ((y * Wo + x) * Cout + co) * ES;
      }
    });
#define SDP_EPI16_OFF(i, nj) vbase[(i) / PER], __builtin_amdgcn_readfirstlane(((i) % PER) * xs + (nj) * 16 * ES)
    auto ld1 = [&](__amdgpu_buffer_rsrc_t r, int vo, int so) __attribute__((always_inline)) {
      if constexpr (IO16) return __uint_as_float((uint32_t)__builtin_amdgcn_raw_buffer_load_b16(r, vo, so, 0) << 16);
      else return __uint_as_float(__builtin_amdgcn_raw_buffer_load_b32(r, vo, so, 0));
    };
    auto store_vals = [&](const float (&w)[NV], __amdgpu_buffer_rsrc_t r, auto nj_c, auto aux_c) __attribute__((always_inline)) {
      constexpr int NJC = decltype(nj_c)::value, AUX = decltype(aux_c)::value;
      if constexpr (IO16) {
        constexpr int HP = PER / 2;
        const bool odd = lane & 1;
#pragma unroll
        for (int f = 0; f < NF; ++f) {
          const int vb = vbase[f] + (odd ? HP * xs - 2 : 0);
#pragma unroll
          for (int k = 0; k < HP; ++k) {
            const float mine = odd ? w[f * PER + HP + k] : w[f * PER + k];
            const float send = odd ? w[f * PER + k] : w[f * PER + HP + k];
            const float got = __int_as_float(__builtin_amdgcn_mov_dpp(__float_as_int(send), 0xB1, 0xf, 0xf, false));
            const uint32_t pk = odd ? pack_bf2(got, mine) : pack_bf2(mine, got);
            __builtin_amdgcn_raw_buffer_store_b32(pk, r, vb, __builtin_amdgcn_readfirstlane(k * xs + NJC * 16 * ES), AUX);
          }
        }
      } else {
#pragma unroll
        for (int i = 0; i < NV; ++i) __builtin_amdgcn_raw_buffer_store_b32(__float_as_uint(w[i]), r, SDP_EPI16_OFF(i, NJC), AUX);
      }
    };
    float pre[NJ][NV], biasv[NJ];
    static_for<0, NJ>([&](auto nj) { biasv[nj] = a.bias ? a.bias[n0 + wn * 16 * NJ + nj * 16 + lcol] : 0.f; });
    if (a.res || a.out2) {
      const __amdgpu_buffer_rsrc_t prs = a.res ? rrs : r2rs;
      static_for<0, NJ>([&](auto njc) {
#pragma unroll
        for (int i = 0; i < NV; ++i) pre[njc][i] = ld1(prs, SDP_EPI16_OFF(i, decltype(njc)::value));
      });
    }
    static_for<0, NJ>([&](auto njc) {
      constexpr int nj = decltype(njc)::value;
      const int co = n0 + wn * 16 * NJ + nj * 16 + lcol;
      const float bias = biasv[nj];
      float v[NV];
      if constexpr (POOL) {
        static_for<0, CB>([&](auto fc) {
          constexpr int f = decltype(fc)::value;
          static_for<0, 2>([&](auto kc) {
            constexpr int k = decltype(kc)::value;
            const float a00 = acc4[f][nj][2 * k], a01 = acc4[f][nj][2 * k + 1];
            const float a10 = acc4[f + CB][nj][2 * k], a11 = acc4[f + CB][nj][2 * k + 1];
            v[f * 2 + k] = ((((a00 + bias) + (a10 + bias)) + (a01 + bias)) + (a11 + bias)) / 4.0f;
          });
        });
      } else {
        static_for<0, 8>([&](auto fc) {
          constexpr int f = decltype(fc)::value;
#pragma unroll
          for (int r = 0; r < 4; ++r) v[f * 4 + r] = acc4[f][nj][r] + bias;
        });
      }
      if (a.up) {
        const int Hi = a.H / 2, Wi = a.W / 2;
        const float shh = (float)(Hi - 1) / (float)(a.H - 1), sww = (float)(Wi - 1) / (float)(a.W - 1);
        const size_t ub = (size_t)b * Hi * Wi * Cout + co;
        auto lu = [&](size_t e) { return IO16 ? ldg1(reinterpret_cast<const __bf16*>(a.up), e) : ldg1(a.up, e); };
#pragma unroll
        for (int i = 0; i < NV; ++i) {
          const int f = i / PER, k = i % PER;
          const int mr = f / CB, mc = (f % CB) * 16;
          const int y = (sr0 + wrow0 + mr) * d + ph_r, x = (sc0 + mc + 4 * lq + k) * d + ph_c;
          const float fy = shh * (float)y, fx = sww * (float)x;
          const int y0 = (int)fy, x0 = (int)fx;
          const int yp = y0 < Hi - 1 ? 1 : 0, xp = x0 < Wi - 1 ? 1 : 0;
          const float ly1 = fy - (float)y0, ly0 = 1.f - ly1, lx1 = fx - (float)x0, lx0 = 1.f - lx1;
          const float v00 = lu(ub + ((size_t)y0 * Wi + x0) * Cout), v01 = lu(ub + ((size_t)y0 * Wi + x0 + xp) * Cout);
          const float v10 = lu(ub + ((size_t)(y0 + yp) * Wi + x0) * Cout);
          const float v11 = lu(ub + ((size_t)(y0 + yp) * Wi + x0 + xp) * Cout);
          v[i] = v[i] + (ly0 * (lx0 * v00 + lx1 * v01) + ly1 * (lx0 * v10 + lx1 * v11));
        }
      }
      if (a.dact) {
        float esc = 1.f, esh = 0.f;
        if (a.dact == 3) {
          esc = a.epi_ss[((size_t)b * Cout + co) * 2];
          esh = a.epi_ss[((size_t)b * Cout + co) * 2 + 1];
        }
#pragma unroll
        for (int i = 0; i < NV; ++i) {
          float h = ld1(xrs, SDP_EPI16_OFF(i, nj));
          if (a.dact == 3) h = fmaf(h, esc, esh);
          v[i] = v[i] * elu_grad(h, a.dact);
        }
      }
      if (a.res) {
#pragma unroll
        for (int i = 0; i < NV; ++i) v[i] = pre[nj][i] + v[i];
      }
      if (a.out2) {
        float r2[NV];
#pragma unroll
        for (int i = 0; i < NV; ++i)
          r2[i] = a.res ? ld1(r2rs, SDP_EPI16_OFF(i, nj)) : pre[nj][i];
#pragma unroll
        for (int i = 0; i < NV; ++i) r2[i] = v[i] + r2[i];
        store_vals(r2, o2rs, njc, std::integral_constant<int, 0>{});
      }
      if (a.epi_elu) {
#pragma unroll
        for (int i = 0; i < NV; ++i) v[i] = elu(v[i]);
      }
      if constexpr (!(SDP_KO & 16))
        store_vals(v, ors, njc, std::integral_constant<int, IO16 ? SDP_STORE_AUX16 : SDP_STORE_AUX>{});
      if (a.stats) {
        float sum = 0.f;
#pragma unroll
        for (int i = 0; i < NV; ++i) sum += v[i];
        float mean = sum * (1.0f / NV);
        float m2 = 0.f;
#pragma unroll
        for (int i = 0; i < NV; ++i) {
          const float dv = v[i] - mean;
          m2 = fmaf(dv, dv, m2);
        }
        float mp = __shfl_xor(mean, 16), qp = __shfl_xor(m2, 16), dm = mean - mp;
        m2 = m2 + qp + dm * dm * (0.5f * NV);
        mean = 0.5f * (mean + mp);
        mp = __shfl_xor(mean, 32);
        qp = __shfl_xor(m2, 32);
        dm = mean - mp;
        m2 = m2 + qp + dm * dm * (float)NV;
        mean = 0.5f * (mean + mp);
        if (lq == 0) {
          float2* st = reinterpret_cast<float2*>(a.stats) + ((size_t)b * a.groups_per_img + tile * WM + wm) * Cout + co;
          *st = make_float2(mean, m2);
        }
      }
    });
#undef SDP_EPI16_OFF
    }
  } else if (a.dact) {
    if constexpr (TC >= 32 && NW == 4 && SH == 16) {
    __builtin_amdgcn_s_waitcnt(0);
    __syncthreads();
    constexpr int SROW = T::NTILE + 8;
    constexpr int SP = WM * 64;
    constexpr int CG = T::NTILE / 4;
    constexpr int PL = 256 / CG;
    constexpr int NPO = POOL ? SP / 4 : SP;
    static_assert(SP * SROW * 4 <= T::LDS_BYTES, "epilogue staging fits the LDS");
    float* stage = reinterpret_cast<float*>(lds);
    const int cg = tid % CG, pl = tid / CG;
    const int co0 = n0 + cg * 4;
    const float4 bias4 = a.bias ? ld4(a.bias + co0) : make_float4(0.f, 0.f, 0.f, 0.f);
    float4 es0 = make_float4(1.f, 0.f, 1.f, 0.f), es1 = es0;
    if (a.dact == 3) {
      es0 = ld4(a.epi_ss + ((size_t)b * Cout + co0) * 2);
      es1 = ld4(a.epi_ss + ((size_t)b * Cout + co0) * 2 + 4);
    }
    const int Ho = POOL ? a.H / 2 : a.H, Wo = POOL ? a.W / 2 : a.W;
    using TA = std::conditional_t<IO16, __bf16, float>;
    auto tp = [](const float* p) { return reinterpret_cast<const TA*>(p); };
    TA* const outb = reinterpret_cast<TA*>(a.out) + (size_t)b * Ho * Wo * Cout;
    float4 sK[WM], s1[WM], s2[WM];
    int sn[WM];
    static_for<0, WM>([&](auto g) {
      sK[g] = make_float4(0.f, 0.f, 0.f, 0.f); s1[g] = sK[g]; s2[g] = sK[g]; sn[g] = 0;
    });
    static_for<0, 2>([&](auto hc) {
      constexpr int h = decltype(hc)::value;
      {
        if constexpr (!POOL && TRANS) {
          static_for<0, 4>([&](auto ic) {
            constexpr int i = decltype(ic)::value;
            static_for<0, 4>([&](auto njc) {
              constexpr int nj = decltype(njc)::value;
              float* dst = stage + (wm * 64 + 16 * i + (lane & 15)) * SROW + wn * 64 + nj * 16 + 4 * (lane >> 4);
              const f32x4 q = acc4[4 * h + i][nj];
              *reinterpret_cast<float4*>(dst) = make_float4(q[0], q[1], q[2], q[3]);
            });
          });
        } else if constexpr (!POOL) {
          static_for<0, 4>([&](auto ic) {
            constexpr int i = decltype(ic)::value;
            static_for<0, 4>([&](auto njc) {
              constexpr int nj = decltype(njc)::value;
              float* dst = stage + (wm * 64 + 16 * i + 4 * (lane >> 4)) * SROW + wn * 64 + nj * 16 + (lane & 15);
  #pragma unroll
              for (int r = 0; r < 4; ++r) dst[r * SROW] = acc4[4 * h + i][nj][r];
            });
          });
        }
      }
      __syncthreads();
      auto pix = [&](int j, int& y, int& x, int& g) __attribute__((always_inline)) {
        if constexpr (POOL) {
          y = (sr0 + wrow0) >> 1;
          x = (sc0 + 32 * h + 2 * j) >> 1;
          g = 0;
        } else {
          const int ws = j >> 6, q = j & 63;
          const int mb = 2 * h + (q >> 5);
          const int row = ws * T::RW + mb / (TC / 32), col = (mb % (TC / 32)) * 32 + (q & 31);
          y = (sr0 + row) * d + ph_r;
          x = (sc0 + col) * d + ph_c;
          g = ws;
        }
      };
      const size_t bo = (size_t)b * Ho * Wo * Cout;
      struct Ops { float4 h, r, q; };
      auto fetch = [&](int j) __attribute__((always_inline)) {
        Ops o;
        int y, x, g;
        pix(min(j, NPO - 1), y, x, g);
        const size_t oi = bo + ((size_t)y * Wo + x) * Cout + co0;
        o.h = a.aux ? ldg4(tp(a.aux), oi) : make_float4(0.f, 0.f, 0.f, 0.f);
        o.r = a.res ? ldg4(tp(a.res), oi) : make_float4(0.f, 0.f, 0.f, 0.f);
        o.q = a.out2 ? ldg4(tp(a.res2), oi) : make_float4(0.f, 0.f, 0.f, 0.f);
        return o;
      };
      Ops nx = fetch(pl);
      for (int j = pl; j < NPO; j += PL) {
        const Ops cu = nx;
        nx = fetch(j + PL);
        float4 v;
        int y, x, g;
        pix(j, y, x, g);
        if constexpr (POOL) {
          const float* s0 = stage + (2 * j) * SROW + cg * 4;
          const float4 o00 = ld4(s0), o01 = ld4(s0 + SROW), o10 = ld4(s0 + 32 * SROW), o11 = ld4(s0 + 33 * SROW);
          auto pool1 = [&](float a00, float a10, float a01, float a11, float bb) {
            return ((((a00 + bb) + (a10 + bb)) + (a01 + bb)) + (a11 + bb)) / 4.0f;
          };
          v.x = pool1(o00.x, o10.x, o01.x, o11.x, bias4.x);
          v.y = pool1(o00.y, o10.y, o01.y, o11.y, bias4.y);
          v.z = pool1(o00.z, o10.z, o01.z, o11.z, bias4.z);
          v.w = pool1(o00.w, o10.w, o01.w, o11.w, bias4.w);
        } else {
          const float4 o = ld4(stage + j * SROW + cg * 4);
          v = make_float4(o.x + bias4.x, o.y + bias4.y, o.z + bias4.z, o.w + bias4.w);
        }
        const size_t oidx = ((size_t)y * Wo + x) * Cout + co0;
        if (a.up) {
          const int Hi = a.H / 2, Wi = a.W / 2;
          const float sh = (float)(Hi - 1) / (float)(a.H - 1), sw = (float)(Wi - 1) / (float)(a.W - 1);
          const float fy = sh * (float)y, fx = sw * (float)x;
          const int y0 = (int)fy, x0 = (int)fx;
          const int yp = y0 < Hi - 1 ? 1 : 0, xp = x0 < Wi - 1 ? 1 : 0;
          const float ly1 = fy - (float)y0, ly0 = 1.f - ly1, lx1 = fx - (float)x0, lx0 = 1.f - lx1;
          const TA* ub = tp(a.up) + (size_t)b * Hi * Wi * Cout + co0;
          const float4 v00 = ldg4(ub, ((size_t)y0 * Wi + x0) * Cout), v01 = ldg4(ub, ((size_t)y0 * Wi + x0 + xp) * Cout);
          const float4 v10 = ldg4(ub, ((size_t)(y0 + yp) * Wi + x0) * Cout);
          const float4 v11 = ldg4(ub, ((size_t)(y0 + yp) * Wi + x0 + xp) * Cout);
          auto bil = [&](float a00, float a01, float a10, float a11) {
            return ly0 * (lx0 * a00 + lx1 * a01) + ly1 * (lx0 * a10 + lx1 * a11);
          };
          v.x = v.x + bil(v00.x, v01.x, v10.x, v11.x);
          v.y = v.y + bil(v00.y, v01.y, v10.y, v11.y);
          v.z = v.z + bil(v00.z, v01.z, v10.z, v11.z);
          v.w = v.w + bil(v00.w, v01.w, v10.w, v11.w);
        }
        if (a.dact) {
          float4 h4 = cu.h;
          if (a.dact == 3)
            h4 = make_float4(fmaf(h4.x, es0.x, es0.y), fmaf(h4.y, es0.z, es0.w), fmaf(h4.z, es1.x, es1.y),
                             fmaf(h4.w, es1.z, es1.w));
          v = make_float4(v.x * elu_grad(h4.x, a.dact), v.y * elu_grad(h4.y, a.dact), v.z * elu_grad(h4.z, a.dact),
                          v.w * elu_grad(h4.w, a.dact));
        }
        if (a.res) v = make_float4(cu.r.x + v.x, cu.r.y + v.y, cu.r.z + v.z, cu.r.w + v.w);
        if (a.out2)
          stg4(reinterpret_cast<TA*>(a.out2), bo + oidx, make_float4(v.x + cu.q.x, v.y + cu.q.y, v.z + cu.q.z, v.w + cu.q.w));
        if (a.epi_elu) v = make_float4(elu(v.x), elu(v.y), elu(v.z), elu(v.w));
        if constexpr (!(SDP_KO & 16)) stg4(outb, oidx, v);
        static_for<0, WM>([&](auto gc) {
          constexpr int gg = decltype(gc)::value;
          if (gg == g) {
            if (sn[gg] == 0) sK[gg] = v;
            const float4 dv = make_float4(v.x - sK[gg].x, v.y - sK[gg].y, v.z - sK[gg].z, v.w - sK[gg].w);
            s1[gg] = make_float4(s1[gg].x + dv.x, s1[gg].y + dv.y, s1[gg].z + dv.z, s1[gg].w + dv.w);
            s2[gg] = make_float4(fmaf(dv.x, dv.x, s2[gg].x), fmaf(dv.y, dv.y, s2[gg].y), fmaf(dv.z, dv.z, s2[gg].z),
                                 fmaf(dv.w, dv.w, s2[gg].w));
            ++sn[gg];
          }
        });
      }
      __syncthreads();
    });

    if (a.stats) {
      float2* part = reinterpret_cast<float2*>(lds);
      static_for<0, WM>([&](auto gc) {
        constexpr int gg = decltype(gc)::value;
        const float n = (float)sn[gg], inv = sn[gg] ? 1.f / n : 0.f;
        const float k4[4] = {sK[gg].x, sK[gg].y, sK[gg].z, sK[gg].w};
        const float a4[4] = {s1[gg].x, s1[gg].y, s1[gg].z, s1[gg].w};
        const float q4[4] = {s2[gg].x, s2[gg].y, s2[gg].z, s2[gg].w};
  #pragma unroll
        for (int c = 0; c < 4; ++c) {
          const float mean = k4[c] + a4[c] * inv;
          const float m2 = fmaxf(q4[c] - a4[c] * a4[c] * inv, 0.f);
          part[(gg * PL + pl) * T::NTILE + cg * 4 + c] = make_float2(mean, m2);
        }
      });
      __syncthreads();
      constexpr int PER = (POOL ? 32 : 128) / PL;
      for (int i = tid; i < WM * T::NTILE; i += 256) {
        const int gg = i / T::NTILE, co = i % T::NTILE;
        float mean = 0.f;
        for (int k = 0; k < PL; ++k) mean += part[(gg * PL + k) * T::NTILE + co].x;
        mean *= 1.f / PL;
        float m2 = 0.f;
        for (int k = 0; k < PL; ++k) {
          const float2 pk = part[(gg * PL + k) * T::NTILE + co];
          const float dm = pk.x - mean;
          m2 += pk.y + (float)PER * dm * dm;
        }
        float2* st = reinterpret_cast<float2*>(a.stats) + ((size_t)b * a.groups_per_img + tile * WM + gg) * Cout + n0 + co;
        *st = make_float2(mean, m2);
      }
    }
    }
  } else {
    if constexpr (SH == 32) {
    __builtin_amdgcn_s_waitcnt(0);
    {
      const int Ho = POOL ? a.H / 2 : a.H, Wo = POOL ? a.W / 2 : a.W;
      const size_t bo = (size_t)b * Ho * Wo * Cout;
      const int img_bytes = Ho * Wo * Cout * 4;
      auto rs = [&](const float* p) { return __builtin_amdgcn_make_buffer_rsrc((void*)(p ? p + bo : a.out + bo), 0, img_bytes, 0x00020000); };
      const __amdgpu_buffer_rsrc_t ors = rs(a.out), rrs = rs(a.res), xrs = rs(a.aux), o2rs = rs(a.out2), r2rs = rs(a.res2);
      const int lhalf = lane >> 5, lcol = lane & 31;
      constexpr int CB = TC / 32;
      constexpr int NV = POOL ? 16 : 64;
      constexpr int PER = POOL ? 8 : 16;
      const int xs = (POOL ? 1 : d) * Cout * 4;
      int vbase[POOL ? CB : 4];
      static_for<0, (POOL ? CB : 4)>([&](auto fc) {
        constexpr int f = decltype(fc)::value;
        const int co = n0 + wn * 64 + lcol;
        if constexpr (POOL) {
          vbase[f] = (((sr0 >> 1) * Wo + ((sc0 + f * 32) >> 1) + 2 * lhalf) * Cout + co) * 4;
        } else {
          constexpr int mr = f / CB, mc = (f % CB) * 32;
          const int y = (sr0 + wrow0 + mr) * d + ph_r, x = (sc0 + mc + 4 * lhalf) * d + ph_c;
          vbase[f] = ((y * Wo + x) * Cout + co) * 4;
        }
      });
      auto mstep = [](int k) { return POOL ? ((((k & 1) * 2 + (k >> 1) * 4) & 3) + 8 * (((k & 1) * 2 + (k >> 1) * 4) >> 2)) / 2
                                           : (k & 3) + 8 * (k >> 2); };
  #define SDP_EPI_OFF(i, nb) vbase[(i) / PER], __builtin_amdgcn_readfirstlane(mstep((i) % PER) * xs + (nb) * 128)
      float pre[2][NV], biasv[2];
      static_for<0, 2>([&](auto nb) { biasv[nb] = a.bias ? a.bias[n0 + wn * 64 + nb * 32 + lcol] : 0.f; });
      if (a.res || a.out2) {
        const __amdgpu_buffer_rsrc_t prs = a.res ? rrs : r2rs;
        static_for<0, 2>([&](auto nbc) {
  #pragma unroll
          for (int i = 0; i < NV; ++i)
            pre[nbc][i] = __uint_as_float(__builtin_amdgcn_raw_buffer_load_b32(prs, SDP_EPI_OFF(i, decltype(nbc)::value), 0));
        });
      }
      static_for<0, 2>([&](auto nbc) {
        constexpr int nb = decltype(nbc)::value;
        const int co = n0 + wn * 64 + nb * 32 + lcol;
        const float bias = biasv[nb];
        float v[NV];
        if constexpr (POOL) {
          static_for<0, CB>([&](auto mbc) {
            constexpr int mb = decltype(mbc)::value;
            static_for<0, 8>([&](auto kc) {
              constexpr int k = decltype(kc)::value;
              constexpr int r = (k & 1) * 2 + (k >> 1) * 4;
              const float a00 = acc[mb][nb][r], a01 = acc[mb][nb][r + 1];
              const float a10 = acc[mb + CB][nb][r], a11 = acc[mb + CB][nb][r + 1];
              v[mb * 8 + k] = ((((a00 + bias) + (a10 + bias)) + (a01 + bias)) + (a11 + bias)) / 4.0f;
            });
          });
        } else {
          static_for<0, 4>([&](auto mbc) {
            constexpr int mb = decltype(mbc)::value;
  #pragma unroll
            for (int r = 0; r < 16; ++r) v[mb * 16 + r] = acc[mb][nb][r] + bias;
          });
        }
        if (a.up) {
          const int Hi = a.H / 2, Wi = a.W / 2;
          const float shh = (float)(Hi - 1) / (float)(a.H - 1), sww = (float)(Wi - 1) / (float)(a.W - 1);
          const float* ub = a.up + (size_t)b * Hi * Wi * Cout + co;
  #pragma unroll
          for (int i = 0; i < NV; ++i) {
            const int f = i / PER, k = i % PER;
            const int mr = f / CB, mc = (f % CB) * 32;
            const int y = (sr0 + wrow0 + mr) * d + ph_r, x = (sc0 + mc + 4 * lhalf + mstep(k)) * d + ph_c;
            const float fy = shh * (float)y, fx = sww * (float)x;
            const int y0 = (int)fy, x0 = (int)fx;
            const int yp = y0 < Hi - 1 ? 1 : 0, xp = x0 < Wi - 1 ? 1 : 0;
            const float ly1 = fy - (float)y0, ly0 = 1.f - ly1, lx1 = fx - (float)x0, lx0 = 1.f - lx1;
            const float v00 = ub[((size_t)y0 * Wi + x0) * Cout], v01 = ub[((size_t)y0 * Wi + x0 + xp) * Cout];
            const float v10 = ub[((size_t)(y0 + yp) * Wi + x0) * Cout];
            const float v11 = ub[((size_t)(y0 + yp) * Wi + x0 + xp) * Cout];
            v[i] = v[i] + (ly0 * (lx0 * v00 + lx1 * v01) + ly1 * (lx0 * v10 + lx1 * v11));
          }
        }
        if (a.dact) {
          float esc = 1.f, esh = 0.f;
          if (a.dact == 3) {
            esc = a.epi_ss[((size_t)b * Cout + co) * 2];
            esh = a.epi_ss[((size_t)b * Cout + co) * 2 + 1];
          }
  #pragma unroll
          for (int i = 0; i < NV; ++i) {
            float h = __uint_as_float(__builtin_amdgcn_raw_buffer_load_b32(xrs, SDP_EPI_OFF(i, nb), 0));
            if (a.dact == 3) h = fmaf(h, esc, esh);
            v[i] = v[i] * elu_grad(h, a.dact);
          }
        }
        if (a.res) {
  #pragma unroll
          for (int i = 0; i < NV; ++i) v[i] = pre[nb][i] + v[i];
        }
        if (a.out2) {
          float r2[NV];
  #pragma unroll
          for (int i = 0; i < NV; ++i)
            r2[i] = a.res ? __uint_as_float(__builtin_amdgcn_raw_buffer_load_b32(r2rs, SDP_EPI_OFF(i, nb), 0)) : pre[nb][i];
  #pragma unroll
          for (int i = 0; i < NV; ++i) __builtin_amdgcn_raw_buffer_store_b32(__float_as_uint(v[i] + r2[i]), o2rs, SDP_EPI_OFF(i, nb), 0);
        }
        if (a.epi_elu) {
  #pragma unroll
          for (int i = 0; i < NV; ++i) v[i] = elu(v[i]);
        }
        if constexpr (!(SDP_KO & 16)) {
  #pragma unroll
          for (int i = 0; i < NV; ++i) __builtin_amdgcn_raw_buffer_store_b32(__float_as_uint(v[i]), ors, SDP_EPI_OFF(i, nb), SDP_STORE_AUX);
        }
        if (a.stats) {
          float sum = 0.f;
  #pragma unroll
          for (int i = 0; i < NV; ++i) sum += v[i];
          const float mean_l = sum * (1.0f / NV);
          float m2_l = 0.f;
  #pragma unroll
          for (int i = 0; i < NV; ++i) {
            const float dv = v[i] - mean_l;
            m2_l = fmaf(dv, dv, m2_l);
          }
          const float mean_p = __shfl_xor(mean_l, 32), m2_p = __shfl_xor(m2_l, 32);
          const float dm = mean_l - mean_p;
          const float mean = 0.5f * (mean_l + mean_p);
          const float m2 = m2_l + m2_p + dm * dm * (0.5f * NV);
          if (lhalf == 0) {
            float2* st = reinterpret_cast<float2*>(a.stats) + ((size_t)b * a.groups_per_img + tile * WM + wm) * Cout + co;
            *st = make_float2(mean, m2);
          }
        }
      });
  #undef SDP_EPI_OFF
    }
    }
  }
#ifdef SDP_TIMING
  SDP_T(4);
  if (tid == 0) {
    unsigned long long* o = a.dbg + blockIdx.x * 8;
    o[0] = tclk[0]; o[1] = tclk[1]; o[2] = tclk[2]; o[3] = tclk[3]; o[4] = tclk[4]; o[5] = tbar;
    o[6] = rt0; o[7] = __builtin_amdgcn_s_memrealtime();
  }
#endif
#endif
}

}
```

simultaneous-diffusion-for-pointclouds_amd/csrc/conv_launch.h:

```cpp
#pragma once
#include "common.h"

namespace sdp {

template <int MODE, int WM, int TC, int KS, bool POOL, bool PELU, bool IO16 = false>
hipError_t conv_launch(ConvArgs a, hipStream_t st);

template <int MODE, bool PELU>
hipError_t conv_launch_half(ConvArgs a, hipStream_t st);

template <int MODE, bool PELU, int NW, bool IO16 = false>
hipError_t conv_launch_nj2(ConvArgs a, hipStream_t st);

template <int MODE>
hipError_t dgrad_launch_half(ConvArgs a, hipStream_t st);

template <int MODE, int NW, bool IO16 = false>
hipError_t dgrad_launch_nj2(ConvArgs a, hipStream_t st);

template <int MODE, int WM, int TC, int KS, bool ZP, bool IO16 = false>
hipError_t dgrad_launch(ConvArgs a, hipStream_t st);


}
```

simultaneous-diffusion-for-pointclouds_amd/csrc/net.hip:

```cpp
#include <algorithm>
#include <cmath>
#include <cstdlib>
#include <cstring>
#include <map>
#include <stdexcept>
#include <string>
#include <vector>


#include "net_internal.h"

using namespace sdp;

namespace {

struct Buf {
  float* p;
  int H, W, C;
};

struct Fwd {
  sdp_net* net;
  int B;
  hipStream_t st;
  float* stats;
  float* ss;
  float* mv;

  struct Opt {
    int pro = PRO_NONE;
    bool bias = true;
    const float* res = nullptr;
    const float* up = nullptr;
    float* out2 = nullptr;
    const float* res2 = nullptr;
    bool epi_elu = false;
    bool stats = false;
    int dil = 1;
    bool circular = true;
    bool pool = false;
  };

  void conv(const Buf& in, const std::string& wkey, const Buf& out, const Opt& o) {
    const auto& hp = net->host.at(wkey + ".weight");
    ConvArgs a{};
    a.in = in.p;
    a.wf = net->mode == MODE_F32 ? reinterpret_cast<const uint4*>(net->P(wkey + ".weight#frag")) : nullptr;
    a.wf16 = net->mode == MODE_F32 ? nullptr : reinterpret_cast<const uint4*>(net->P(wkey + ".weight#frag16"));
    a.bias = o.bias ? net->P(wkey + ".bias") : nullptr;
    a.out = out.p;
    a.res = o.res;
    a.out2 = o.out2;
    a.res2 = o.res2;
    a.up = o.up;
    a.pro_ss = o.pro == PRO_AFFINE_ELU ? ss : net->P("#ident_ss");
    a.ss_bstride = o.pro == PRO_AFFINE_ELU ? 2 * in.C : 0;
    a.stats = o.stats ? stats : nullptr;
    a.B = B;
    a.H = in.H;
    a.W = in.W;
    a.Cin = in.C;
    a.Cout = out.C;
    a.dil = o.dil;
    a.circular = o.circular ? 1 : 0;
    a.pro_mode = o.pro;
    a.epi_elu = o.epi_elu ? 1 : 0;
    if ((int)hp.shape[1] != in.C || (int)hp.shape[0] != out.C) throw std::runtime_error("conv shape mismatch " + wkey);
    const char* why = "conv launch";
    const int ks = (int)hp.shape[2];
    sdp_net::ProfRec rec;
    if (net->profile) {
      rec.cls = "conv" + std::to_string(ks) + "x" + std::to_string(ks) + " " + std::to_string(in.C) + "->" +
                std::to_string(out.C) + " @" + std::to_string(in.H) + "x" + std::to_string(in.W) + " d" +
                std::to_string(o.dil) + (o.pool ? " pool" : "");
      rec.flops = 2.0 * B * in.H * in.W * (double)in.C * out.C * ks * ks;
      rec.bytes = 4.0 * B * ((double)in.H * in.W * in.C + (double)out.H * out.W * out.C) + 4.0 * out.C * in.C * ks * ks;
      rec.a = net->event();
      rec.b = net->event();
      chk(hipEventRecord(rec.a, st), "hipEventRecord");
    }
    hipError_t e = conv_mfma(net->mode, a, ks, o.pool, st, &why);
    if (e != hipSuccess) throw std::runtime_error(std::string(why) + " (" + wkey + ")");
    if (net->profile) {
      chk(hipEventRecord(rec.b, st), "hipEventRecord");
      net->prof.push_back(rec);
    }
  }

  template <class F>
  void prof_launch(const std::string& cls, double bytes, F&& launch) {
    sdp_net::ProfRec rec;
    if (net->profile) {
      rec.cls = cls;
      rec.flops = 0;
      rec.bytes = bytes;
      rec.a = net->event();
      rec.b = net->event();
      chk(hipEventRecord(rec.a, st), "hipEventRecord");
    }
    launch();
    if (net->profile) {
      chk(hipEventRecord(rec.b, st), "hipEventRecord");
      net->prof.push_back(rec);
    }
  }

  void norm(const std::string& nkey, int T, float cnt, int C) {
    prof_launch("inpp_finalize C" + std::to_string(C), (double)B * T * C * 8 + (double)B * C * 8, [&] {
      chk(inpp_finalize(stats, B, T, cnt, C, net->P(nkey + ".alpha"), net->P(nkey + ".gamma"), net->P(nkey + ".beta"),
                        ss, st, nullptr, mv),
          "inpp_finalize");
    });
  }
  void pool(const Buf& X, const Buf& P) {
    const double bytes = 2.0 * B * X.H * X.W * X.C * 4;
    prof_launch("maxpool5 " + std::to_string(X.C) + " @" + std::to_string(X.H) + "x" + std::to_string(X.W), bytes,
                [&] { chk(maxpool5(X.p, P.p, B, X.H, X.W, X.C, st), "maxpool5"); });
  }
  static int tiles(const Buf& b) { return b.H * b.W / 128; }

  void resblock(const std::string& k, const Buf& x, const Buf& t1, const Buf& t2, const Buf& out, bool down, int dil,
                bool want_stats, int x_tiles, float x_cnt) {
    norm(k + ".normalize1", x_tiles, x_cnt, x.C);
    Opt o1;
    o1.pro = PRO_AFFINE_ELU;
    o1.stats = true;
    o1.dil = dil;
    conv(x, k + ".conv1", t1, o1);
    norm(k + ".normalize2", tiles(t1), 128.f, t1.C);
    Opt o2;
    o2.pro = PRO_AFFINE_ELU;
    o2.stats = want_stats;
    o2.dil = dil;
    if (down && dil == 1) {
      const Buf xp{out.p, x.H / 2, x.W / 2, x.C};
      prof_launch("avgpool2 " + std::to_string(x.C) + " @" + std::to_string(x.H) + "x" + std::to_string(x.W),
                  1.25 * B * x.H * x.W * x.C * 4, [&] { chk(avgpool2(x.p, xp.p, B, x.H, x.W, x.C, st), "avgpool2"); });
      Opt os;
      os.circular = false;
      conv(xp, k + ".shortcut.conv", t2, os);
      o2.circular = false;
      o2.pool = true;
      o2.res = t2.p;
      conv(t1, k + ".conv2.conv", out, o2);
    } else if (down) {
      Opt os;
      os.dil = dil;
      conv(x, k + ".shortcut", t2, os);
      o2.res = t2.p;
      conv(t1, k + ".conv2", out, o2);
    } else {
      o2.res = x.p;
      conv(t1, k + ".conv2", out, o2);
    }
  }

  Buf rcu(const std::string& k, Buf x, int nblocks, const Buf& tmp, const Buf& o0, const Buf& o1, bool final_elu,
          bool final_stats) {
    Buf outs[2] = {o0, o1};
    for (int i = 0; i < nblocks; ++i) {
      Opt a;
      a.pro = PRO_ELU;
      a.bias = false;
      conv(x, k + "." + std::to_string(i + 1) + "_1_conv", tmp, a);
      Opt b;
      b.pro = PRO_ELU;
      b.bias = false;
      b.res = x.p;
      b.epi_elu = final_elu && i == nblocks - 1;
      b.stats = final_stats && i == nblocks - 1;
      const Buf& y = outs[i & 1];
      conv(tmp, k + "." + std::to_string(i + 1) + "_2_conv", y, b);
      x = y;
    }
    return x;
  }

  Buf crp(const std::string& k, const Buf& X, const Buf& P, const Buf& Qp, const Buf& R, const Buf& S) {
    pool(X, P);
    Opt a;
    a.bias = false;
    a.out2 = R.p;
    a.res2 = X.p;
    conv(P, k + ".convs.0", Qp, a);
    pool(Buf{Qp.p, X.H, X.W, X.C}, P);
    Opt b;
    b.bias = false;
    b.res = R.p;
    conv(P, k + ".convs.1", S, b);
    return S;
  }
};

}

static void forward_impl(sdp_net* net, const float* x, const int64_t* labels, float* out, int B, void* ws,
                         size_t ws_bytes, hipStream_t st, const LangevinArgs* lg = nullptr) {
  const int H = net->d.H, W = net->d.W, C = net->d.ngf, C2 = 2 * C;
  const int h = H / 2, w = W / 2;
  const size_t F = (size_t)B * H * W * C, Q = (size_t)B * h * w * C2;
  char* p = reinterpret_cast<char*>(ws);
  char* end = p + ws_bytes;
  auto take = [&](size_t n) {
    float* q = reinterpret_cast<float*>(p);
    p += ((n * 4 + 255) / 256) * 256;
    if (p > end) throw std::runtime_error("workspace too small");
    return q;
  };
  Fwd f{net, B, st, nullptr, nullptr, nullptr};
  f.stats = take((size_t)B * (H * W / 64) * C2 * 2);
  f.ss = take((size_t)B * C2 * 2);
  f.mv = take((size_t)B * C2 * 4);
  auto full = [&]() { return Buf{take(F), H, W, C}; };
  auto half = [&]() { return Buf{take(Q), h, w, C2}; };
  Buf L1 = full(), FA = full(), FB = full(), FC = full(), FD = full(), FE = full();
  Buf L2 = half(), L3 = half(), L4 = half(), QA = half(), QB = half(), QC = half(), QD = half(), QE = half();
  auto half128 = [&](const Buf& b) { return Buf{b.p, h, w, C}; };

  using Opt = Fwd::Opt;
  f.prof_launch("begin_conv 4->128 @" + std::to_string(H) + "x" + std::to_string(W),
                (double)B * H * W * (2 * 4 + C * 4) + (double)B * (H * W / 64) * C * 8, [&] {
                  chk(begin_conv(x, net->P("begin_conv.weight"), net->P("begin_conv.bias"), FA.p, f.stats, B, H, W, st, net->mode),
                      "begin_conv");
                });
  f.resblock("res1.0", FA, FB, FD, FC, false, 1, true, H * W / 64, 64.f);
  f.resblock("res1.1", FC, FB, FD, L1, false, 1, true, Fwd::tiles(FC), 128.f);
  f.resblock("res2.0", L1, FB, QA, QB, true, 1, true, Fwd::tiles(L1), 128.f);
  f.resblock("res2.1", QB, QA, QC, L2, false, 1, true, Fwd::tiles(L1), 32.f);
  f.resblock("res3.0", L2, QA, QB, QC, true, 2, true, Fwd::tiles(L2), 128.f);
  f.resblock("res3.1", QC, QA, QB, L3, false, 2, true, Fwd::tiles(QC), 128.f);
  f.resblock("res4.0", L3, QA, QB, QC, true, 4, true, Fwd::tiles(L3), 128.f);
  f.resblock("res4.1", QC, QA, QB, L4, false, 4, false, Fwd::tiles(QC), 128.f);

  Buf a1 = f.rcu("refine1.adapt_convs.0", L4, 2, QA, QB, QC, true, false);
  Buf x2 = f.crp("refine1.crp", a1, QA, QB, QD, QE);
  Buf ref1 = f.rcu("refine1.output_convs", x2, 1, QA, QB, QC, false, false);
  Buf hA = f.rcu("refine2.adapt_convs.0", L3, 2, QA, QC, QD, false, false);
  Buf hB = f.rcu("refine2.adapt_convs.1", ref1, 2, QA, QC, QE, false, false);
  {
    Opt o;
    f.conv(hA, "refine2.msf.convs.0", QA, o);
    Opt o1;
    o1.res = QA.p;
    o1.epi_elu = true;
    f.conv(hB, "refine2.msf.convs.1", QB, o1);
  }
  x2 = f.crp("refine2.crp", QB, QA, QC, QD, QE);
  Buf ref2 = f.rcu("refine2.output_convs", x2, 1, QA, QB, QC, false, false);
  hA = f.rcu("refine3.adapt_convs.0", L2, 2, QA, QC, QD, false, false);
  hB = f.rcu("refine3.adapt_convs.1", ref2, 2, QA, QC, QE, false, false);
  {
    Opt o;
    f.conv(hA, "refine3.msf.convs.0", half128(QA), o);
    Opt o1;
    o1.res = QA.p;
    o1.epi_elu = true;
    f.conv(hB, "refine3.msf.convs.1", half128(QB), o1);
  }
  x2 = f.crp("refine3.crp", half128(QB), half128(QA), half128(QC), half128(QD), half128(QE));
  Buf ref3 = f.rcu("refine3.output_convs", x2, 1, half128(QA), half128(QB), half128(QC), false, false);
  hA = f.rcu("refine4.adapt_convs.0", L1, 2, FA, FB, FC, false, false);
  hB = f.rcu("refine4.adapt_convs.1", ref3, 2, half128(QA), half128(QC), half128(QD), false, false);
  {
    Opt o;
    f.conv(hB, "refine4.msf.convs.1", half128(QA), o);
    Opt o1;
    o1.up = QA.p;
    o1.epi_elu = true;
    f.conv(hA, "refine4.msf.convs.0", FD, o1);
  }
  x2 = f.crp("refine4.crp", FD, FA, FB, FE, FC);
  Buf o = f.rcu("refine4.output_convs", x2, 3, FA, FB, FD, false, true);
  f.norm("normalizer", Fwd::tiles(o), 128.f, C);
  const double lg_bytes = lg ? (double)B * 2 * H * W * (20 + (out ? 4 : 0) + (lg->noise ? 4 : 0)) : B * 2.0 * H * W * 4;
  f.prof_launch(std::string(lg ? "end_conv+langevin" : "end_conv") + " 128->2 @" + std::to_string(H) + "x" +
                    std::to_string(W),
                (double)B * H * W * C * 4 + lg_bytes, [&] {
                  chk(end_conv(o.p, f.ss, net->P("end_conv.weight"), net->P("end_conv.bias"), net->P("sigmas"), labels,
                               out, B, H, W, C, st, lg, net->mode),
                      "end_conv");
                });
}

static size_t workspace_bytes_one(const sdp_net* net, int B) {
  const int H = net->d.H, W = net->d.W, C = net->d.ngf, C2 = 2 * C;
  const size_t F = (size_t)B * H * W * C, Q = (size_t)B * (H / 2) * (W / 2) * C2;
  auto r = [](size_t n) { return ((n * 4 + 255) / 256) * 256; };
  return r((size_t)B * (H * W / 64) * C2 * 2) + r((size_t)B * C2 * 2) + r((size_t)B * C2 * 4) + 6 * r(F) + 8 * r(Q);
}

constexpr int kSplitDefault = 2;
static int split_ways(const sdp_net* net) { return net->split > 0 ? net->split : kSplitDefault; }

static void split_part(int B, int k, int p, int& first, int& count) {
  first = (int)((long)B * p / k);
  count = (int)((long)B * (p + 1) / k) - first;
}

static size_t workspace_bytes(const sdp_net* net, int B) {
  size_t need = workspace_bytes_one(net, B);
  const int k = std::min(B, split_ways(net));
  if (k > 1) {
    size_t sum = 0;
    for (int p = 0; p < k; ++p) {
      int f, c;
      split_part(B, k, p, f, c);
      sum += workspace_bytes_one(net, c);
    }
    need = std::max(need, sum);
  }
  return need;
}

static void forward_split(sdp_net* net, const float* x, const int64_t* labels, float* out, int B, void* ws,
                          size_t ws_bytes, hipStream_t st, const LangevinArgs* lg) {
  const int k = std::min(B, split_ways(net));
  if (k < 2 || net->profile) {
    forward_impl(net, x, labels, out, B, ws, ws_bytes, st, lg);
    return;
  }
  for (int p = 0; p + 1 < k; ++p) {
    if (!net->aux_stream[p])
      chk(hipStreamCreateWithFlags(&net->aux_stream[p], hipStreamNonBlocking), "hipStreamCreate");
    if (!net->ev_join[p]) chk(hipEventCreateWithFlags(&net->ev_join[p], hipEventDisableTiming), "hipEventCreate");
  }
  if (!net->ev_fork) chk(hipEventCreateWithFlags(&net->ev_fork, hipEventDisableTiming), "hipEventCreate");
  const size_t per = (size_t)2 * net->d.H * net->d.W;
  char* w = reinterpret_cast<char*>(ws);
  chk(hipEventRecord(net->ev_fork, st), "hipEventRecord");
  for (int p = k - 1; p >= 0; --p) {
    int f, c;
    split_part(B, k, p, f, c);
    const size_t wb = workspace_bytes_one(net, c);
    hipStream_t s = p ? net->aux_stream[p - 1] : st;
    if (p) chk(hipStreamWaitEvent(s, net->ev_fork, 0), "hipStreamWaitEvent");
    LangevinArgs l{};
    if (lg) {
      l = *lg;
      l.x = lg->x + f * per;
      l.ref = lg->ref + f * per;
      l.mask = lg->mask + f * per;
      if (lg->noise) l.noise = lg->noise + f * per;
      if (lg->lik) l.lik = lg->lik + f * per;
      l.offset = lg->offset + f * per / 4;
    }
    forward_impl(net, x + f * per, labels + f, out ? out + f * per : nullptr, c, w, wb, s, lg ? &l : nullptr);
    w += wb;
    if (p) chk(hipEventRecord(net->ev_join[p - 1], s), "hipEventRecord");
  }
  for (int p = 0; p + 1 < k; ++p) chk(hipStreamWaitEvent(st, net->ev_join[p], 0), "hipStreamWaitEvent");
}

static thread_local std::string g_err;

int sdp_fail(const std::string& m) {
  g_err = m;
  return -1;
}
static int fail(const std::string& m) { return sdp_fail(m); }

extern "C" {

int sdp_version(void) { return SDP_VERSION; }
const char* sdp_last_error(void) { return g_err.c_str(); }

int sdp_net_create(const sdp_net_desc* desc, sdp_net** out) {
  if (!desc || !out) return fail("sdp_net_create: null argument");
  if (desc->ngf != 128 || desc->channels != 2) return fail("sdp_net_create: only ngf=128, channels=2 are built");
  if (desc->H % 8 || desc->W % 128) return fail("sdp_net_create: H must be a multiple of 8 and W of 128");
  if (desc->precision < 0 || desc->precision > 2) return fail("sdp_net_create: bad precision");
  sdp_net* n = new sdp_net();
  n->d = *desc;
  n->mode = desc->precision;
  *out = n;
  return 0;
}

int sdp_net_set_param(sdp_net* net, const char* key, const float* data, const int64_t* shape, int ndim) {
  if (!net || !key || !data || (ndim > 0 && !shape)) return fail("sdp_net_set_param: null argument");
  HostParam hp;
  size_t n = 1;
  for (int i = 0; i < ndim; ++i) {
    hp.shape.push_back(shape[i]);
    n *= (size_t)shape[i];
  }
  hp.data.assign(data, data + n);
  net->host[key] = std::move(hp);
  net->finalized = false;
  return 0;
}

int sdp_net_finalize(sdp_net* net) {
  if (!net) return fail("sdp_net_finalize: null net");
  try {
    net->release();
    if (!net->host.count("sigmas")) return fail("sdp_net_finalize: missing sigmas");
    auto upload = [&](const std::string& k, const void* src, size_t bytes) {
      void* d = nullptr;
      chk(hipMalloc(&d, bytes), "hipMalloc");
      chk(hipMemcpy(d, src, bytes, hipMemcpyHostToDevice), "hipMemcpy");
      net->dev[k] = d;
    };
    net->layout.clear();
    size_t off = 0;
    std::vector<std::string> order;
    try {
      order = grad_completion_order(net);
    } catch (const std::exception&) {
      order.clear();
    }
    std::map<std::string, bool> placed;
    for (auto& kv : net->host)
      if (kv.first != "sigmas") order.push_back(kv.first);
    for (const auto& k : order) {
      auto it = net->host.find(k);
      if (it == net->host.end() || k == "sigmas" || placed[k]) continue;
      placed[k] = true;
      net->layout.push_back({k, off, it->second.data.size()});
      off += (it->second.data.size() + 63) / 64 * 64;
    }
    net->arena_floats = off;
    chk(hipMalloc(&net->arena, off * 4), "hipMalloc");
    net->arena_owned = true;
    for (auto& e : net->layout) {
      chk(hipMemcpy(net->arena + e.offset, net->host[e.key].data.data(), e.numel * 4, hipMemcpyHostToDevice), "hipMemcpy");
      net->dev[e.key] = net->arena + e.offset;
    }
    upload("sigmas", net->host["sigmas"].data.data(), net->host["sigmas"].data.size() * 4);
    for (auto& kv : net->host) {
      const HostParam& hp = kv.second;
      if (net->is_conv_w(kv.first) && (hp.shape[0] % 32 || hp.shape[1] % 32))
        return fail("sdp_net_finalize: conv channels must be /32: " + kv.first);
    }
    std::vector<float> ident(2 * 1024);
    for (size_t i = 0; i < ident.size(); i += 2) ident[i] = 1.f;
    upload("#ident_ss", ident.data(), ident.size() * 4);
    hipStream_t st;
    chk(hipStreamCreateWithFlags(&st, hipStreamNonBlocking), "hipStreamCreate");
    net->repack(st);
    chk(hipStreamSynchronize(st), "hipStreamSynchronize");
    chk(hipStreamDestroy(st), "hipStreamDestroy");
    net->finalized = true;
  } catch (const std::exception& e) {
    return fail(std::string("sdp_net_finalize: ") + e.what());
  }
  return 0;
}

int sdp_net_param_arena_floats(const sdp_net* net, size_t* n) {
  if (!net || !n || !net->finalized) return fail("sdp_net_param_arena_floats: finalize first");
  *n = net->arena_floats;
  return 0;
}

int sdp_net_param_count(const sdp_net* net, int* n) {
  if (!net || !n || !net->finalized) return fail("sdp_net_param_count: finalize first");
  *n = (int)net->layout.size();
  return 0;
}

int sdp_net_param_info(const sdp_net* net, int i, char* key, size_t cap, size_t* offset, size_t* numel) {
  if (!net || !net->finalized || i < 0 || i >= (int)net->layout.size() || !key || cap == 0)
    return fail("sdp_net_param_info: bad argument");
  const auto& e = net->layout[i];
  std::strncpy(key, e.key.c_str(), cap - 1);
  key[cap - 1] = 0;
  if (offset) *offset = e.offset;
  if (numel) *numel = e.numel;
  return 0;
}

int sdp_net_bind_params(sdp_net* net, float* arena, void* stream) {
  if (!net || !arena || !net->finalized) return fail("sdp_net_bind_params: bad argument");
  try {
    hipStream_t st = reinterpret_cast<hipStream_t>(stream);
    if (arena != net->arena)
      chk(hipMemcpyAsync(arena, net->arena, net->arena_floats * 4, hipMemcpyDeviceToDevice, st), "hipMemcpyAsync");
    chk(hipStreamSynchronize(st), "hipStreamSynchronize");
    if (net->arena_owned) chk(hipFree(net->arena), "hipFree");
    net->arena = arena;
    net->arena_owned = false;
    for (auto& e : net->layout) net->dev[e.key] = arena + e.offset;
  } catch (const std::exception& e) {
    return fail(std::string("sdp_net_bind_params: ") + e.what());
  }
  return 0;
}

int sdp_net_repack(sdp_net* net, void* stream) {
  if (!net || !net->finalized) return fail("sdp_net_repack: finalize first");
  try {
    net->repack(reinterpret_cast<hipStream_t>(stream));
  } catch (const std::exception& e) {
    return fail(std::string("sdp_net_repack: ") + e.what());
  }
  return 0;
}

int sdp_net_workspace_size(const sdp_net* net, int B, size_t* bytes) {
  if (!net || !bytes || B <= 0) return fail("sdp_net_workspace_size: bad argument");
  *bytes = workspace_bytes(net, B);
  return 0;
}

int sdp_net_forward(sdp_net* net, const float* x, const int64_t* labels, float* out, int B, void* ws, size_t ws_bytes,
                    void* stream) {
  if (!net || !x || !labels || !out || !ws || B <= 0) return fail("sdp_net_forward: bad argument");
  if (!net->finalized) return fail("sdp_net_forward: call sdp_net_finalize first");
  if (ws_bytes < workspace_bytes(net, B)) return fail("sdp_net_forward: workspace too small");
  const hipStream_t st = reinterpret_cast<hipStream_t>(stream);
  try {
    forward_split(net, x, labels, out, B, ws, ws_bytes, st, nullptr);
  } catch (const std::exception& e) {
    return fail(std::string("sdp_net_forward: ") + e.what());
  }
  return 0;
}

int sdp_net_forward_langevin(sdp_net* net, float* x, const int64_t* labels, int B, const sdp_langevin_params* lp,
                             void* ws, size_t ws_bytes, void* stream) {
  if (!net || !x || !labels || !lp || !lp->ref || !lp->mask || !ws || B <= 0)
    return fail("sdp_net_forward_langevin: bad argument");
  if (!net->finalized) return fail("sdp_net_forward_langevin: call sdp_net_finalize first");
  if (ws_bytes < workspace_bytes(net, B)) return fail("sdp_net_forward_langevin: workspace too small");
  const LangevinArgs lg{x,         lp->ref,          lp->mask,  lp->noise,    lp->seed,         lp->offset, lp->step_size,
                        lp->noise_scale, lp->grad_ref, lp->nan_to_num, lp->lik_out, lp->absmax_bits};
  try {
    forward_split(net, x, labels, lp->grad_out, B, ws, ws_bytes, reinterpret_cast<hipStream_t>(stream), &lg);
  } catch (const std::exception& e) {
    return fail(std::string("sdp_net_forward_langevin: ") + e.what());
  }
  return 0;
}

int sdp_net_set_split(sdp_net* net, int ways) {
  if (!net || ways < 0 || ways > SDP_MAX_SPLIT) return fail("sdp_net_set_split: ways must be 0 (default) .. 4");
  net->split = ways;
  return 0;
}

int sdp_net_profile_enable(sdp_net* net, int enable) {
  if (!net) return fail("sdp_net_profile_enable: null net");
  net->profile = enable != 0;
  return 0;
}

int sdp_net_profile_read(sdp_net* net, char* buf, size_t cap, int* n_launches) {
  if (!net || !buf || cap == 0) return fail("sdp_net_profile_read: bad argument");
  struct Agg { int n = 0; double ms = 0, flops = 0, bytes = 0; };
  std::map<std::string, Agg> agg;
  try {
    for (auto& r : net->prof) {
      chk(hipEventSynchronize(r.b), "hipEventSynchronize");
      float ms = 0.f;
      chk(hipEventElapsedTime(&ms, r.a, r.b), "hipEventElapsedTime");
      Agg& g = agg[r.cls];
      g.n += 1;
      g.ms += ms;
      g.flops = r.flops;
      g.bytes = r.bytes;
      net->ev_pool.push_back(r.a);
      net->ev_pool.push_back(r.b);
    }
  } catch (const std::exception& e) {
    return fail(std::string("sdp_net_profile_read: ") + e.what());
  }
  if (n_launches) *n_launches = (int)net->prof.size();
  net->prof.clear();
  std::string out;
  for (auto& kv : agg)
    out += kv.first + "\t" + std::to_string(kv.second.n) + "\t" + std::to_string(kv.second.ms) + "\t" +
           std::to_string(kv.second.flops) + "\t" + std::to_string(kv.second.bytes) + "\n";
  std::strncpy(buf, out.c_str(), cap - 1);
  buf[cap - 1] = 0;
  return 0;
}

int sdp_net_destroy(sdp_net* net) {
  delete net;
  return 0;
}

int sdp_langevin_step(float* x, const float* grad, const float* ref, const int32_t* mask, const float* noise,
                      uint64_t seed, uint64_t offset, float step_size, float noise_scale, float grad_ref, int nan_to_num,
                      int B, int C, int HW, float* lik_out, uint32_t* absmax_bits, void* stream) {
  if (!x || !grad || !ref || !mask || B <= 0 || C <= 0 || HW <= 0) return fail("sdp_langevin_step: bad argument");
  if (HW % 4) return fail("sdp_langevin_step: H*W must be a multiple of 4");
  hipError_t e = langevin_step(x, grad, ref, mask, noise, seed, offset, step_size, noise_scale, grad_ref, nan_to_num, B,
                               C, HW, lik_out, absmax_bits, reinterpret_cast<hipStream_t>(stream));
  return e == hipSuccess ? 0 : fail(std::string("sdp_langevin_step: ") + hipGetErrorString(e));
}

int sdp_axpy_step(float* x, const float* g, float a, const float* lik, const int32_t* mask, const float* ref, float b,
                  int n, void* stream) {
  if (!x || n <= 0 || (g && !lik) || (!g && (!mask || !ref))) return fail("sdp_axpy_step: bad argument");
  hipError_t e = axpy_step(x, g, a, lik, mask, ref, b, (size_t)n, reinterpret_cast<hipStream_t>(stream));
  return e == hipSuccess ? 0 : fail(std::string("sdp_axpy_step: ") + hipGetErrorString(e));
}

}
```

simultaneous-diffusion-for-pointclouds_amd/csrc/net_internal.h:

```cpp
#pragma once
#include <cstring>
#include <map>
#include <memory>
#include <stdexcept>
#include <string>
#include <vector>

#include "../../include/sdp.h"
#include "kernels.h"

namespace sdp {

struct HostParam {
  std::vector<int64_t> shape;
  std::vector<float> data;
};

struct ParamEntry {
  std::string key;
  size_t offset, numel;
};

inline void chk(hipError_t e, const char* what) {
  if (e != hipSuccess) throw std::runtime_error(std::string(what) + ": " + hipGetErrorString(e));
}

constexpr int SDP_MAX_SPLIT = 4;

struct TrainPlan;
void destroy_plan(TrainPlan* p);

}

struct sdp_net {
  struct ProfRec {
    std::string cls;
    double flops;
    double bytes = 0;
    hipEvent_t a, b;
  };
  sdp_net_desc d;
  bool profile = false;
  std::vector<ProfRec> prof;
  std::vector<hipEvent_t> ev_pool;
  std::map<std::string, sdp::HostParam> host;
  std::map<std::string, void*> dev;
  std::vector<sdp::ParamEntry> layout;
  float* arena = nullptr;
  size_t arena_floats = 0;
  bool arena_owned = false;
  bool finalized = false;
  bool train_packs = false;
  bool tape16 = true;
  int mode = sdp::MODE_F32X3;
  sdp::TrainPlan* plan = nullptr;
  int split = 0;
  hipStream_t aux_stream[sdp::SDP_MAX_SPLIT - 1] = {};
  hipEvent_t ev_fork = nullptr, ev_join[sdp::SDP_MAX_SPLIT - 1] = {};

  ~sdp_net() {
    release();
    for (auto& s : aux_stream)
      if (s) (void)hipStreamDestroy(s);
    for (auto& e : ev_join)
      if (e) (void)hipEventDestroy(e);
    if (ev_fork) (void)hipEventDestroy(ev_fork);
    for (auto& r : prof) {
      (void)hipEventDestroy(r.a);
      (void)hipEventDestroy(r.b);
    }
    for (auto e : ev_pool) (void)hipEventDestroy(e);
  }
  void release() {
    for (auto& kv : dev) {
      const bool in_arena = arena && kv.second >= (void*)arena && kv.second < (void*)(arena + arena_floats);
      if (!in_arena) (void)hipFree(kv.second);
    }
    dev.clear();
    if (pack_dev) (void)hipFree(pack_dev);
    pack_dev = nullptr;
    pack_dev_n = 0;
    pack_host.clear();
    if (arena_owned && arena) (void)hipFree(arena);
    arena = nullptr;
    arena_owned = false;
    if (plan) sdp::destroy_plan(plan);
    plan = nullptr;
  }
  hipEvent_t event() {
    if (!ev_pool.empty()) {
      hipEvent_t e = ev_pool.back();
      ev_pool.pop_back();
      return e;
    }
    hipEvent_t e;
    if (hipEventCreate(&e) != hipSuccess) throw std::runtime_error("hipEventCreate");
    return e;
  }
  const float* P(const std::string& k) const {
    auto it = dev.find(k);
    if (it == dev.end()) throw std::runtime_error("missing parameter " + k);
    return reinterpret_cast<const float*>(it->second);
  }
  float* grad_of(float* grads, const std::string& k) const {
    for (auto& e : layout)
      if (e.key == k) return grads + e.offset;
    throw std::runtime_error("no parameter " + k);
  }
  bool is_conv_w(const std::string& k) const {
    auto it = host.find(k);
    return it != host.end() && it->second.shape.size() == 4 && k != "begin_conv.weight" && k != "end_conv.weight";
  }
  std::vector<sdp::PackDesc> pack_host;
  sdp::PackDesc* pack_dev = nullptr;
  size_t pack_dev_n = 0, pack_total = 0;
  void repack(hipStream_t st) {
    std::vector<sdp::PackDesc> d;
    size_t total = 0;
    for (auto& kv : host) {
      if (!is_conv_w(kv.first)) continue;
      const auto& s = kv.second.shape;
      for (int dg = 0; dg < 5; ++dg) {
        if (dg == 0 && mode != sdp::MODE_F32) continue;
        if (dg == 1 || dg == 2) continue;
        if (dg == 3 && mode == sdp::MODE_F32) continue;
        if (dg == 4 && (!train_packs || mode == sdp::MODE_F32)) continue;
        const std::string fk = kv.first + (dg == 0 ? "#frag" : dg == 3 ? "#frag16" : "#dfrag16");
        const int nt = (int)(s[2] * s[3]);
        const size_t n = (size_t)s[0] * s[1] * nt;
        if (!dev.count(fk)) {
          void* p = nullptr;
          sdp::chk(hipMalloc(&p, n * 4), "hipMalloc");
          dev[fk] = p;
        }
        d.push_back(sdp::PackDesc{P(kv.first), reinterpret_cast<uint32_t*>(dev[fk]), (int)s[0], (int)s[1], nt, dg,
                                  total});
        total += n;
      }
    }
    const bool same = d.size() == pack_host.size() &&
                      std::equal(d.begin(), d.end(), pack_host.begin(), [](const sdp::PackDesc& x, const sdp::PackDesc& y) {
                        return x.w == y.w && x.out == y.out && x.begin == y.begin && x.dgrad == y.dgrad;
                      });
    if (!same) {
      if (pack_dev_n < d.size()) {
        if (pack_dev) sdp::chk(hipFree(pack_dev), "hipFree");
        sdp::chk(hipMalloc(&pack_dev, d.size() * sizeof(sdp::PackDesc)), "hipMalloc");
        pack_dev_n = d.size();
      }
      pack_host = d;
      sdp::chk(hipMemcpyAsync(pack_dev, pack_host.data(), d.size() * sizeof(sdp::PackDesc), hipMemcpyHostToDevice, st),
               "hipMemcpyAsync");
      pack_total = total;
    }
    sdp::chk(sdp::pack_weights_multi(pack_dev, (int)pack_host.size(), pack_total, mode, st), "pack_weights_multi");
  }
};

int sdp_fail(const std::string& m);

namespace sdp {
std::vector<std::string> grad_completion_order(sdp_net* net);
}
```

simultaneous-diffusion-for-pointclouds_amd/csrc/train_aux.hip:

```cpp
#include "common.h"
#include "kernels.h"

namespace sdp {

SDP_DEV float wsum(float v) {
#pragma unroll
  for (int o = 32; o > 0; o >>= 1) v += __shfl_xor(v, o);
  return v;
}

SDP_DEV uint32_t pack_slot(const float* __restrict__ w, int Cout, int Cin, int NT, int mode, int dgrad, size_t i) {
  const int Co = dgrad ? Cin : Cout;
  const int NB = Co / 32;
  const int slot = i & 15;
  size_t r = i >> 4;
  const int lane = r & 63;
  r >>= 6;
  const int nb = r % NB;
  r /= NB;
  const int tap = r % NT;
  const int ch = r / NT;
  const int co = nb * 32 + (lane & 31), h = lane >> 5;
  auto wv = [&](int ci) -> float {
    return dgrad ? w[((size_t)ci * Cin + co) * NT + (NT - 1 - tap)] : w[((size_t)co * Cin + ci) * NT + tap];
  };
  if (mode == MODE_F32) return __float_as_uint(wv(ch * 32 + 16 * h + slot));
  const int s = slot >> 3, hl = (slot >> 2) & 1, j0 = (slot & 3) * 2;
  uint32_t pk = 0;
  for (int e = 0; e < 2; ++e) {
    const float f = wv(ch * 32 + 16 * s + 8 * h + j0 + e);
    const __bf16 hi = (__bf16)f;
    const __bf16 q = hl ? (__bf16)(f - (float)hi) : hi;
    pk |= (uint32_t)__builtin_bit_cast(uint16_t, q) << (16 * e);
  }
  return pk;
}

SDP_DEV uint32_t pack_slot16(const float* __restrict__ w, int Cout, int Cin, int NT, int mode, int dgrad, size_t i) {
  const int NF = (dgrad ? Cin : Cout) / 16;
  const int word = i & 3;
  const int lane = (i >> 2) & 63;
  const int hl = (i >> 8) & 1;
  size_t r = i >> 9;
  const int nf = r % NF;
  r /= NF;
  const int tap = r % NT;
  const int ch = r / NT;
  const int co = nf * 16 + (lane & 15);
  uint32_t pk = 0;
  for (int e = 0; e < 2; ++e) {
    const int ci = ch * 32 + 8 * (lane >> 4) + word * 2 + e;
    const float f = dgrad ? w[((size_t)ci * Cin + co) * NT + (NT - 1 - tap)] : w[((size_t)co * Cin + ci) * NT + tap];
    const __bf16 hi = (__bf16)f;
    const __bf16 q = (hl && mode == MODE_F32X3) ? (__bf16)(f - (float)hi) : hi;
    pk |= (uint32_t)__builtin_bit_cast(uint16_t, q) << (16 * e);
  }
  return pk;
}

__global__ void pack_weights_kernel(const float* __restrict__ w, uint32_t* __restrict__ out, int Cout, int Cin, int NT,
                                    int mode, int dgrad) {
  const size_t n = (size_t)Cout * Cin * NT;
  for (size_t i = blockIdx.x * (size_t)blockDim.x + threadIdx.x; i < n; i += (size_t)gridDim.x * blockDim.x)
    out[i] = pack_slot(w, Cout, Cin, NT, mode, dgrad, i);
}

__global__ void pack_weights_multi_kernel(const PackDesc* __restrict__ d, int mode) {
  const PackDesc e = d[blockIdx.y];
  const size_t n = (size_t)e.Cout * e.Cin * e.NT;
  for (size_t j = blockIdx.x * (size_t)blockDim.x + threadIdx.x; j < n; j += (size_t)gridDim.x * blockDim.x)
    e.out[j] = e.dgrad >= 3 ? pack_slot16(e.w, e.Cout, e.Cin, e.NT, mode, e.dgrad == 4, j)
                            : pack_slot(e.w, e.Cout, e.Cin, e.NT, mode, e.dgrad, j);
}

hipError_t pack_weights_multi(const PackDesc* d, int nd, size_t total, int mode, hipStream_t st) {
  if (nd <= 0) return hipSuccess;
  (void)total;
  hipLaunchKernelGGL(pack_weights_multi_kernel, dim3(512, nd), dim3(256), 0, st, d, mode);
  return hipGetLastError();
}

hipError_t pack_weights(const float* w, uint32_t* out, int Cout, int Cin, int k, int mode, int dgrad, hipStream_t st) {
  const size_t n = (size_t)Cout * Cin * k * k;
  const int grid = (int)std::min<size_t>((n + 255) / 256, 4096);
  hipLaunchKernelGGL(pack_weights_kernel, dim3(grid), dim3(256), 0, st, w, out, Cout, Cin, k * k, mode, dgrad);
  return hipGetLastError();
}

constexpr int INPP_GRP = 512, INPP_NT = 1024;
template <typename TA>
__global__ __launch_bounds__(INPP_NT) void inpp_bwd_reduce_kernel(const TA* __restrict__ g, const TA* __restrict__ h,
                                                                  const float4* __restrict__ nst, float2* __restrict__ part,
                                                                  int HW, int C) {
  __shared__ float2 red[INPP_NT * 4];
  const int b = blockIdx.y, grp = blockIdx.x, ngrp = gridDim.x;
  const int C4 = C / 4, PL = INPP_NT / C4, tid = threadIdx.x;
  const int c4 = tid % C4, pl = tid / C4;
  const size_t base = ((size_t)b * HW + (size_t)grp * INPP_GRP) * C;
  float4 mu, rs;
  {
    const float4 n0 = nst[(size_t)b * C + c4 * 4], n1 = nst[(size_t)b * C + c4 * 4 + 1];
    const float4 n2 = nst[(size_t)b * C + c4 * 4 + 2], n3 = nst[(size_t)b * C + c4 * 4 + 3];
    mu = make_float4(n0.x, n1.x, n2.x, n3.x);
    rs = make_float4(n0.y, n1.y, n2.y, n3.y);
  }
  float sg[4] = {0.f, 0.f, 0.f, 0.f}, sx[4] = {0.f, 0.f, 0.f, 0.f};
  const int npp = INPP_GRP / PL;
  for (int j = 0; j < npp; j += 4) {
    float4 gv[4], hv[4];
#pragma unroll
    for (int u = 0; u < 4; ++u) {
      const size_t o = base + (size_t)(pl + (j + u) * PL) * C + c4 * 4;
      gv[u] = ldg4(g, o);
      hv[u] = ldg4(h, o);
    }
#pragma unroll
    for (int u = 0; u < 4; ++u) {
      sg[0] += gv[u].x; sg[1] += gv[u].y; sg[2] += gv[u].z; sg[3] += gv[u].w;
      sx[0] = fmaf(gv[u].x, (hv[u].x - mu.x) * rs.x, sx[0]);
      sx[1] = fmaf(gv[u].y, (hv[u].y - mu.y) * rs.y, sx[1]);
      sx[2] = fmaf(gv[u].z, (hv[u].z - mu.z) * rs.z, sx[2]);
      sx[3] = fmaf(gv[u].w, (hv[u].w - mu.w) * rs.w, sx[3]);
    }
  }
#pragma unroll
  for (int k = 0; k < 4; ++k) red[(pl * C4 + c4) * 4 + k] = make_float2(sg[k], sx[k]);
  __syncthreads();
  for (int i = tid; i < C; i += INPP_NT) {
    float a0 = 0.f, a1 = 0.f;
    for (int k = 0; k < PL; ++k) {
      const float2 v = red[(k * C4 + i / 4) * 4 + (i & 3)];
      a0 += v.x;
      a1 += v.y;
    }
    part[((size_t)b * ngrp + grp) * C + i] = make_float2(a0, a1);
  }
}

__global__ __launch_bounds__(1024) void inpp_bwd_finalize_kernel(const float2* __restrict__ part, int ngrp, float N,
                                                                 const float4* __restrict__ nst,
                                                                 const float* __restrict__ alpha,
                                                                 const float* __restrict__ gamma, int C,
                                                                 float4* __restrict__ coef, float* __restrict__ ppart) {
  __shared__ double r0[1024], r1[1024];
  const int b = blockIdx.x, tid = threadIdx.x, Gt = 1024 / C, gi = tid / C, c = tid % C;
  double s0 = 0.0, s1 = 0.0;
  for (int k = gi; k < ngrp; k += Gt) {
    const float2 v = part[((size_t)b * ngrp + k) * C + c];
    s0 += v.x;
    s1 += v.y;
  }
  r0[tid] = s0;
  r1[tid] = s1;
  __syncthreads();
  if (gi == 0)
    for (int k = 1; k < Gt; ++k) {
      s0 += r0[k * C + c];
      s1 += r1[k * C + c];
    }
  __syncthreads();
  const float4 ns = nst[(size_t)b * C + c];
  const double Gc = s0, Gx = s1;
  const double al = alpha[c], gm = gamma[c];
  const double dmh = al * gm * Gc;
  if (gi == 0) r0[c] = dmh * ns.z;
  __syncthreads();
  for (int s = C / 2; s > 0; s >>= 1) {
    if (gi == 0 && c < s) r0[c] += r0[c + s];
    __syncthreads();
  }
  const double A = r0[0];
  const double du = (double)ns.w * (dmh - (double)ns.z * A / (C - 1));
  if (gi == 0) r1[c] = du;
  __syncthreads();
  for (int s = C / 2; s > 0; s >>= 1) {
    if (gi == 0 && c < s) r1[c] += r1[c + s];
    __syncthreads();
  }
  if (gi != 0) return;
  const double dmu = du - r1[0] / C;
  const double rs = ns.y;
  const double k1 = gm * rs;
  const double k2 = -gm * rs * rs * Gx / N;
  const double k3 = -gm * rs * Gc / N + dmu / N;
  coef[(size_t)b * C + c] = make_float4((float)k1, (float)k2, (float)k3, ns.x);
  float* pp = ppart + ((size_t)b * C + c) * 3;
  pp[0] = (float)(gm * (double)ns.z * Gc);
  pp[1] = (float)(Gx + al * (double)ns.z * Gc);
  pp[2] = (float)Gc;
}

__global__ void inpp_bwd_params_kernel(const float* __restrict__ ppart, int B, int C, float* __restrict__ dalpha,
                                       float* __restrict__ dgamma, float* __restrict__ dbeta) {
  const int c = blockIdx.x * blockDim.x + threadIdx.x;
  if (c >= C) return;
  double a = 0.0, g = 0.0, be = 0.0;
  for (int b = 0; b < B; ++b) {
    const float* pp = ppart + ((size_t)b * C + c) * 3;
    a += pp[0];
    g += pp[1];
    be += pp[2];
  }
  dalpha[c] = (float)a;
  dgamma[c] = (float)g;
  dbeta[c] = (float)be;
}

template <typename TA>
__global__ __launch_bounds__(256) void inpp_bwd_apply_kernel(const TA* __restrict__ g, const TA* __restrict__ h,
                                                             const float4* __restrict__ coef, const TA* __restrict__ r1,
                                                             const TA* __restrict__ r2, TA* __restrict__ out, int HW,
                                                             int C) {
  const int C4 = C / 4;
  const int b = blockIdx.y;
  const size_t n4 = (size_t)HW * C4, off = (size_t)b * n4;
  const size_t i0 = blockIdx.x * (size_t)blockDim.x + threadIdx.x, stride = (size_t)gridDim.x * blockDim.x;
  const int c = (int)(i0 % C4) * 4;
  const float4* cf = coef + (size_t)b * C + c;
  const float4 k0 = cf[0], kk1 = cf[1], kk2 = cf[2], kk3 = cf[3];
#pragma unroll 2
  for (size_t i = i0; i < n4; i += stride) {
    const size_t e = (off + i) * 4;
    const float4 gv = ldg4(g, e), hv = ldg4(h, e);
    float4 v = make_float4(fmaf(k0.x, gv.x, fmaf(k0.y, hv.x - k0.w, k0.z)), fmaf(kk1.x, gv.y, fmaf(kk1.y, hv.y - kk1.w, kk1.z)),
                           fmaf(kk2.x, gv.z, fmaf(kk2.y, hv.z - kk2.w, kk2.z)), fmaf(kk3.x, gv.w, fmaf(kk3.y, hv.w - kk3.w, kk3.z)));
    if (r1) {
      const float4 t = ldg4(r1, e);
      v = make_float4(v.x + t.x, v.y + t.y, v.z + t.z, v.w + t.w);
    }
    if (r2) {
      const float4 t = ldg4(r2, e);
      v = make_float4(v.x + t.x, v.y + t.y, v.z + t.z, v.w + t.w);
    }
    stg4(out, e, v);
  }
}

static int grid_for(size_t n) { return (int)std::min<size_t>((n + 255) / 256, 256 * 32); }

template <typename TA>
static hipError_t inpp_backward_t(const TA* g, const TA* h, const float* nst, const float* alpha, const float* gamma,
                                  int B, int HW, int C, float* part, float* coef, float* ppart, float* dalpha,
                                  float* dgamma, float* dbeta, const TA* r1, const TA* r2, TA* out, hipStream_t st) {
  if (HW % INPP_GRP || C % 4 || C > 512 || (256 % (C / 4)) || (INPP_GRP / (INPP_NT / (C / 4))) % 4) return hipErrorInvalidValue;
  const int ngrp = HW / INPP_GRP;
  hipLaunchKernelGGL(inpp_bwd_reduce_kernel<TA>, dim3(ngrp, B), dim3(INPP_NT), 0, st, g, h,
                     reinterpret_cast<const float4*>(nst), reinterpret_cast<float2*>(part), HW, C);
  hipLaunchKernelGGL(inpp_bwd_finalize_kernel, dim3(B), dim3(1024), 0, st, reinterpret_cast<const float2*>(part), ngrp,
                     (float)HW, reinterpret_cast<const float4*>(nst), alpha, gamma, C, reinterpret_cast<float4*>(coef),
                     ppart);
  hipLaunchKernelGGL(inpp_bwd_params_kernel, dim3((C + 255) / 256), dim3(256), 0, st, ppart, B, C, dalpha, dgamma, dbeta);
  const size_t n4 = (size_t)HW * C / 4;
  const int nb = (int)std::min<size_t>((n4 + 255) / 256, 2048);
  hipLaunchKernelGGL(inpp_bwd_apply_kernel<TA>, dim3(nb, B), dim3(256), 0, st, g, h,
                     reinterpret_cast<const float4*>(coef), r1, r2, out, HW, C);
  return hipGetLastError();
}

hipError_t inpp_backward(const float* g, const float* h, const float* nst, const float* alpha, const float* gamma, int B,
                         int HW, int C, float* part, float* coef, float* ppart, float* dalpha, float* dgamma,
                         float* dbeta, const float* r1, const float* r2, float* out, hipStream_t st, bool h16) {
  if (!h16) return inpp_backward_t(g, h, nst, alpha, gamma, B, HW, C, part, coef, ppart, dalpha, dgamma, dbeta, r1, r2, out, st);
  auto H = [](const float* p) { return reinterpret_cast<const __bf16*>(p); };
  return inpp_backward_t(H(g), H(h), nst, alpha, gamma, B, HW, C, part, coef, ppart, dalpha, dgamma, dbeta, H(r1), H(r2),
                         reinterpret_cast<__bf16*>(out), st);
}

template <typename TA>
__global__ void unpool_kernel(const TA* __restrict__ dout, TA* __restrict__ dst, int H, int W, int C, size_t n4) {
  const int C4 = C / 4;
  for (size_t i = blockIdx.x * (size_t)blockDim.x + threadIdx.x; i < n4; i += (size_t)gridDim.x * blockDim.x) {
    const int c4 = i % C4;
    size_t p = i / C4;
    const int x = p % W;
    p /= W;
    const int y = p % H;
    const size_t b = p / H;
    const float4 v = ldg4(dout, (((b * (H / 2) + y / 2) * (W / 2) + x / 2) * C4 + c4) * 4);
    stg4(dst, i * 4, make_float4(v.x * 0.25f, v.y * 0.25f, v.z * 0.25f, v.w * 0.25f));
  }
}

constexpr int MPB_W = 32, MPB_CB = 32;
template <typename TA>
__global__ __launch_bounds__(256) void maxpool5_bwd_kernel(const TA* __restrict__ dp, const uchar4* __restrict__ idx,
                                                           const TA* __restrict__ res, TA* __restrict__ dst, int H,
                                                           int W, int C, int rpb) {
  constexpr int C4B = MPB_CB / 4, PC = MPB_W + 4, RU = PC * C4B;
  __shared__ float4 sd[5 * RU];
  __shared__ uchar4 si[5 * RU];
  const int tid = threadIdx.x;
  const int tw = W / MPB_W, tc = C / MPB_CB, nch = (H + rpb - 1) / rpb;
  int t = blockIdx.x;
  const int cb = t % tc;
  t /= tc;
  const int tx = t % tw;
  t /= tw;
  const int chunk = t % nch;
  const size_t b = t / nch;
  const int y0 = chunk * rpb, y1 = min(H, y0 + rpb), x0 = tx * MPB_W, c40 = cb * C4B, C4 = C / 4;
  float4 d[2];
  uchar4 k[2];
  auto fetch = [&](int row) {
#pragma unroll
    for (int h = 0; h < 2; ++h) {
      const int u = tid + h * 256, xx = x0 - 2 + u / C4B;
      if (u < RU && row >= 0 && row < H && xx >= 0 && xx < W) {
        const size_t j = ((b * H + row) * W + xx) * C4 + c40 + u % C4B;
        d[h] = ldg4(dp, j * 4);
        k[h] = idx[j];
      } else {
        d[h] = make_float4(0.f, 0.f, 0.f, 0.f);
        k[h] = make_uchar4(255, 255, 255, 255);
      }
    }
  };
  auto put = [&](int slot) {
#pragma unroll
    for (int h = 0; h < 2; ++h) {
      const int u = tid + h * 256;
      if (u < RU) {
        sd[slot * RU + u] = d[h];
        si[slot * RU + u] = k[h];
      }
    }
  };
  for (int r = 0; r < 4; ++r) {
    fetch(y0 - 2 + r);
    put(r);
  }
  fetch(y0 + 2);
  const int c4 = tid % C4B, col = tid / C4B;
  int base = 0;
  for (int y = y0; y < y1; ++y) {
    put(base == 0 ? 4 : base - 1);
    __syncthreads();
    fetch(y + 3);
    const size_t o = ((b * H + y) * W + x0 + col) * C4 + c40 + c4;
    float4 s = res ? ldg4(res, o * 4) : make_float4(0.f, 0.f, 0.f, 0.f);
#pragma unroll
    for (int dy = -2; dy <= 2; ++dy) {
      int sl = base + dy + 2;
      sl = sl >= 5 ? sl - 5 : sl;
#pragma unroll
      for (int dx = -2; dx <= 2; ++dx) {
        const int u = sl * RU + (col + 2 + dx) * C4B + c4;
        const uchar4 kk = si[u];
        const unsigned char want = (unsigned char)((2 - dy) * 5 + (2 - dx));
        if (kk.x == want || kk.y == want || kk.z == want || kk.w == want) {
          const float4 dd = sd[u];
          if (kk.x == want) s.x += dd.x;
          if (kk.y == want) s.y += dd.y;
          if (kk.z == want) s.z += dd.z;
          if (kk.w == want) s.w += dd.w;
        }
      }
    }
    stg4(dst, o * 4, s);
    base = base == 4 ? 0 : base + 1;
    __syncthreads();
  }
}

constexpr int MPH_W = 32, MPH_C = 64;
__global__ __launch_bounds__(256) void maxpool5_bwd_h16_kernel(const __bf16* __restrict__ dp, const uint8_t* __restrict__ idx,
                                                               const __bf16* __restrict__ res, __bf16* __restrict__ dst,
                                                               int H, int W, int C, int rpb) {
  constexpr int C8B = MPH_C / 8, PC = MPH_W + 4, RU = PC * C8B;
  __shared__ uint4 sd[5 * RU];
  __shared__ uint2 si[5 * RU];
  const int tid = threadIdx.x;
  const int tw = W / MPH_W, tc = C / MPH_C, nch = (H + rpb - 1) / rpb;
  int t = blockIdx.x;
  const int cb = t % tc;
  t /= tc;
  const int tx = t % tw;
  t /= tw;
  const int chunk = t % nch;
  const size_t b = t / nch;
  const int y0 = chunk * rpb, y1 = min(H, y0 + rpb), x0 = tx * MPH_W;
  uint4 d[2];
  uint2 k[2];
  auto fetch = [&](int row) {
#pragma unroll
    for (int h = 0; h < 2; ++h) {
      const int u = tid + h * 256, xx = x0 - 2 + u / C8B;
      if (u < RU && row >= 0 && row < H && xx >= 0 && xx < W) {
        const size_t e = ((b * H + row) * W + xx) * C + cb * MPH_C + (u % C8B) * 8;
        d[h] = *reinterpret_cast<const uint4*>(dp + e);
        k[h] = *reinterpret_cast<const uint2*>(idx + e);
      } else {
        d[h] = make_uint4(0u, 0u, 0u, 0u);
        k[h] = make_uint2(0xffffffffu, 0xffffffffu);
      }
    }
  };
  auto put = [&](int slot) {
#pragma unroll
    for (int h = 0; h < 2; ++h) {
      const int u = tid + h * 256;
      if (u < RU) {
        sd[slot * RU + u] = d[h];
        si[slot * RU + u] = k[h];
      }
    }
  };
  for (int r = 0; r < 4; ++r) {
    fetch(y0 - 2 + r);
    put(r);
  }
  fetch(y0 + 2);
  const int c8 = tid % C8B, col = tid / C8B;
  int base = 0;
  for (int y = y0; y < y1; ++y) {
    put(base == 0 ? 4 : base - 1);
    __syncthreads();
    fetch(y + 3);
    const size_t o = ((b * H + y) * W + x0 + col) * C + cb * MPH_C + c8 * 8;
    float s[8] = {0.f, 0.f, 0.f, 0.f, 0.f, 0.f, 0.f, 0.f};
    if (res) {
      const uint4 rv = *reinterpret_cast<const uint4*>(res + o);
      const float4 lo = bf4_to_f4(make_uint2(rv.x, rv.y)), hi = bf4_to_f4(make_uint2(rv.z, rv.w));
      s[0] = lo.x; s[1] = lo.y; s[2] = lo.z; s[3] = lo.w; s[4] = hi.x; s[5] = hi.y; s[6] = hi.z; s[7] = hi.w;
    }
#pragma unroll
    for (int dy = -2; dy <= 2; ++dy) {
      int sl = base + dy + 2;
      sl = sl >= 5 ? sl - 5 : sl;
#pragma unroll
      for (int dx = -2; dx <= 2; ++dx) {
        const int u = sl * RU + (col + 2 + dx) * C8B + c8;
        const uint2 kk = si[u];
        const uint32_t want = (uint32_t)((2 - dy) * 5 + (2 - dx)) * 0x01010101u;
        const uint32_t e0 = kk.x ^ want, e1 = kk.y ^ want;
        const uint32_t z0 = (e0 - 0x01010101u) & ~e0 & 0x80808080u, z1 = (e1 - 0x01010101u) & ~e1 & 0x80808080u;
        if (z0 | z1) {
          const uint4 dd = sd[u];
          const uint32_t w[4] = {dd.x, dd.y, dd.z, dd.w};
#pragma unroll
          for (int e = 0; e < 8; ++e) {
            const uint32_t byte = ((e < 4 ? kk.x : kk.y) >> (8 * (e & 3))) & 0xffu;
            const float v = (e & 1) ? __uint_as_float(w[e >> 1] & 0xffff0000u) : __uint_as_float(w[e >> 1] << 16);
            if (byte == ((2 - dy) * 5 + (2 - dx))) s[e] += v;
          }
        }
      }
    }
    *reinterpret_cast<uint4*>(dst + o) = make_uint4(pack_bf2(s[0], s[1]), pack_bf2(s[2], s[3]), pack_bf2(s[4], s[5]),
                                                     pack_bf2(s[6], s[7]));
    base = base == 4 ? 0 : base + 1;
    __syncthreads();
  }
}

SDP_DEV void up_weights(int o, int n_lo, float scale, int* i0, int* i1, float* w0, float* w1) {
  const float f = scale * (float)o;
  const int a = (int)f;
  const int ap = a < n_lo - 1 ? 1 : 0;
  *i0 = a;
  *i1 = a + ap;
  *w1 = f - (float)a;
  *w0 = 1.f - *w1;
}

template <typename TA>
__global__ void upsample_bwd_kernel(const TA* __restrict__ g, TA* __restrict__ dlow, int H, int W, int C,
                                    int accumulate, size_t n4) {
  const int h = H / 2, w = W / 2, C4 = C / 4;
  const float sh = (float)(h - 1) / (float)(H - 1), sw = (float)(w - 1) / (float)(W - 1);
  for (size_t i = blockIdx.x * (size_t)blockDim.x + threadIdx.x; i < n4; i += (size_t)gridDim.x * blockDim.x) {
    const int c4 = i % C4;
    size_t p = i / C4;
    const int j = p % w;
    p /= w;
    const int ii = p % h;
    const size_t b = p / h;
    const int ylo = max(0, (int)floorf((float)(ii - 1) / sh) - 1), yhi = min(H - 1, (int)ceilf((float)(ii + 1) / sh) + 1);
    const int xlo = max(0, (int)floorf((float)(j - 1) / sw) - 1), xhi = min(W - 1, (int)ceilf((float)(j + 1) / sw) + 1);
    float4 s = make_float4(0.f, 0.f, 0.f, 0.f);
    for (int y = ylo; y <= yhi; ++y) {
      int a0, a1;
      float u0, u1;
      up_weights(y, h, sh, &a0, &a1, &u0, &u1);
      const float wy = (a0 == ii ? u0 : 0.f) + (a1 == ii ? u1 : 0.f);
      if (wy == 0.f) continue;
      for (int x = xlo; x <= xhi; ++x) {
        int b0, b1;
        float v0, v1;
        up_weights(x, w, sw, &b0, &b1, &v0, &v1);
        const float wx = (b0 == j ? v0 : 0.f) + (b1 == j ? v1 : 0.f);
        if (wx == 0.f) continue;
        const float4 gv = ldg4(g, (((b * H + y) * W + x) * C4 + c4) * 4);
        const float ww = wy * wx;
        s = make_float4(fmaf(ww, gv.x, s.x), fmaf(ww, gv.y, s.y), fmaf(ww, gv.z, s.z), fmaf(ww, gv.w, s.w));
      }
    }
    if (accumulate) {
      const float4 t = ldg4(dlow, i * 4);
      s = make_float4(s.x + t.x, s.y + t.y, s.z + t.z, s.w + t.w);
    }
    stg4(dlow, i * 4, s);
  }
}

template <typename TA>
__global__ void elu_bwd_post_kernel(const TA* __restrict__ dy, const TA* __restrict__ y,
                                    const TA* __restrict__ res, TA* __restrict__ dst, size_t n4) {
#pragma unroll 2
  for (size_t i = blockIdx.x * (size_t)blockDim.x + threadIdx.x; i < n4; i += (size_t)gridDim.x * blockDim.x) {
    const float4 d = ldg4(dy, i * 4), yv = ldg4(y, i * 4);
    float4 v = make_float4(d.x * elu_grad(yv.x, 2), d.y * elu_grad(yv.y, 2), d.z * elu_grad(yv.z, 2),
                           d.w * elu_grad(yv.w, 2));
    if (res) {
      const float4 t = ldg4(res, i * 4);
      v = make_float4(v.x + t.x, v.y + t.y, v.z + t.z, v.w + t.w);
    }
    stg4(dst, i * 4, v);
  }
}

template <typename TA>
__global__ void add_kernel(const TA* __restrict__ a, const TA* __restrict__ b, TA* __restrict__ dst, size_t n4) {
#pragma unroll 2
  for (size_t i = blockIdx.x * (size_t)blockDim.x + threadIdx.x; i < n4; i += (size_t)gridDim.x * blockDim.x) {
    const float4 x = ldg4(a, i * 4), y = ldg4(b, i * 4);
    stg4(dst, i * 4, make_float4(x.x + y.x, x.y + y.y, x.z + y.z, x.w + y.w));
  }
}

__global__ __launch_bounds__(256) void sum_rows_kernel(const float* __restrict__ part, int K, int n, int stride,
                                                       float* __restrict__ out) {
  __shared__ double red[8][32];
  const int il = threadIdx.x & 31, kg = threadIdx.x >> 5;
  const int i = blockIdx.x * 32 + il;
  double s = 0.0;
  if (i < n)
    for (int k = kg; k < K; k += 8) s += part[(size_t)k * stride + i];
  red[kg][il] = s;
  __syncthreads();
  if (kg == 0 && i < n) {
    for (int g = 1; g < 8; ++g) s += red[g][il];
    out[i] = (float)s;
  }
}

static hipError_t sum_rows(const float* part, int K, int n, int stride, float* out, hipStream_t st) {
  hipLaunchKernelGGL(sum_rows_kernel, dim3((n + 31) / 32), dim3(256), 0, st, part, K, n, stride, out);
  return hipGetLastError();
}

#define SDP_H16(p) reinterpret_cast<const __bf16*>(p)
#define SDP_H16W(p) reinterpret_cast<__bf16*>(p)
hipError_t unpool(const float* dout, float* dst, int B, int H, int W, int C, hipStream_t st, bool h16) {
  const size_t n4 = (size_t)B * H * W * C / 4;
  if (h16) hipLaunchKernelGGL(unpool_kernel<__bf16>, dim3(grid_for(n4)), dim3(256), 0, st, SDP_H16(dout), SDP_H16W(dst), H, W, C, n4);
  else hipLaunchKernelGGL(unpool_kernel<float>, dim3(grid_for(n4)), dim3(256), 0, st, dout, dst, H, W, C, n4);
  return hipGetLastError();
}

hipError_t maxpool5_backward(const uint8_t* idx, const float* dp, const float* res, float* dst, int B, int H, int W, int C,
                             hipStream_t st, bool h16) {
  if (W % MPB_W || C % MPB_CB) return hipErrorInvalidValue;
  const int strips = B * (W / MPB_W) * (C / MPB_CB);
  int rpb = H;
  while (rpb > 8 && (long)strips * ((H + rpb - 1) / rpb) < 2048) rpb = (rpb + 1) / 2;
  const int nb = strips * ((H + rpb - 1) / rpb);
  if (h16) {
    if (C % MPH_C) return hipErrorInvalidValue;
    const int strips16 = B * (W / MPH_W) * (C / MPH_C);
    int rpb16 = H;
    while (rpb16 > 8 && (long)strips16 * ((H + rpb16 - 1) / rpb16) < 2048) rpb16 = (rpb16 + 1) / 2;
    hipLaunchKernelGGL(maxpool5_bwd_h16_kernel, dim3(strips16 * ((H + rpb16 - 1) / rpb16)), dim3(256), 0, st, SDP_H16(dp), idx,
                       SDP_H16(res), SDP_H16W(dst), H, W, C, rpb16);
  } else
    hipLaunchKernelGGL(maxpool5_bwd_kernel<float>, dim3(nb), dim3(256), 0, st, dp, reinterpret_cast<const uchar4*>(idx), res,
                       dst, H, W, C, rpb);
  return hipGetLastError();
}

hipError_t upsample_backward(const float* g, float* dlow, int B, int H, int W, int C, int accumulate, hipStream_t st, bool h16) {
  const size_t n4 = (size_t)B * (H / 2) * (W / 2) * C / 4;
  if (h16)
    hipLaunchKernelGGL(upsample_bwd_kernel<__bf16>, dim3(grid_for(n4)), dim3(256), 0, st, SDP_H16(g), SDP_H16W(dlow), H, W, C,
                       accumulate, n4);
  else
    hipLaunchKernelGGL(upsample_bwd_kernel<float>, dim3(grid_for(n4)), dim3(256), 0, st, g, dlow, H, W, C, accumulate, n4);
  return hipGetLastError();
}

hipError_t elu_backward_post(const float* dy, const float* y, const float* res, float* dst, size_t n, hipStream_t st, bool h16) {
  if (h16)
    hipLaunchKernelGGL(elu_bwd_post_kernel<__bf16>, dim3(grid_for(n / 4)), dim3(256), 0, st, SDP_H16(dy), SDP_H16(y), SDP_H16(res),
                       SDP_H16W(dst), n / 4);
  else
    hipLaunchKernelGGL(elu_bwd_post_kernel<float>, dim3(grid_for(n / 4)), dim3(256), 0, st, dy, y, res, dst, n / 4);
  return hipGetLastError();
}

hipError_t add_tensors(const float* a, const float* b, float* dst, size_t n, hipStream_t st, bool h16) {
  if (h16)
    hipLaunchKernelGGL(add_kernel<__bf16>, dim3(grid_for(n / 4)), dim3(256), 0, st, SDP_H16(a), SDP_H16(b), SDP_H16W(dst), n / 4);
  else
    hipLaunchKernelGGL(add_kernel<float>, dim3(grid_for(n / 4)), dim3(256), 0, st, a, b, dst, n / 4);
  return hipGetLastError();
}

SDP_DEV float linspace01_t(int i, int n) {
  if (n == 1) return 0.f;
  const float step = 1.0f / (float)(n - 1);
  return i < n / 2 ? step * (float)i : 1.0f - step * (float)(n - 1 - i);
}

constexpr int BW_ROWS = 8;
template <typename TA>
__global__ __launch_bounds__(256) void begin_wgrad_kernel(const float* __restrict__ x, const TA* __restrict__ dy,
                                                          float* __restrict__ part, int H, int W) {
  __shared__ float sp[4][3][66];
  __shared__ float sd[64][129];
  const int tid = threadIdx.x, co = tid & 127, half = tid >> 7;
  const int tiles_row = W / 64, rows_blk = H / BW_ROWS;
  const int per_img = rows_blk * tiles_row;
  const int b = blockIdx.x / per_img, t = blockIdx.x % per_img;
  const int y0 = (t / tiles_row) * BW_ROWS, x0 = (t % tiles_row) * 64;
  float acc[18];
#pragma unroll
  for (int k = 0; k < 18; ++k) acc[k] = 0.f;
  float db = 0.f;
  for (int r = 0; r < BW_ROWS; ++r) {
    const int y = y0 + r;
    __syncthreads();
    for (int i = tid; i < 4 * 3 * 66; i += 256) {
      const int ci = i / 198, rr = (i / 66) % 3, c = i % 66;
      const int yy = y - 1 + rr, xx = x0 - 1 + c;
      float v = 0.f;
      if (yy >= 0 && yy < H && xx >= 0 && xx < W) {
        if (ci < 2) v = 2.f * x[(((size_t)b * 2 + ci) * H + yy) * W + xx] - 1.f;
        else if (ci == 2) v = linspace01_t(xx, W);
        else v = linspace01_t(yy, H);
      }
      sp[ci][rr][c] = v;
    }
    for (int i = tid; i < 64 * 32; i += 256) {
      const int px = i >> 5, c4 = i & 31;
      const float4 v = ldg4(dy, (((size_t)b * H + y) * W + x0 + px) * 128 + c4 * 4);
      sd[px][c4 * 4] = v.x; sd[px][c4 * 4 + 1] = v.y; sd[px][c4 * 4 + 2] = v.z; sd[px][c4 * 4 + 3] = v.w;
    }
    __syncthreads();
    const int ci0 = half * 2;
    float wv[2][3][3];
#pragma unroll
    for (int c2 = 0; c2 < 2; ++c2)
#pragma unroll
      for (int rr = 0; rr < 3; ++rr) {
        wv[c2][rr][0] = sp[ci0 + c2][rr][0];
        wv[c2][rr][1] = sp[ci0 + c2][rr][1];
      }
    for (int px = 0; px < 64; ++px) {
#pragma unroll
      for (int c2 = 0; c2 < 2; ++c2)
#pragma unroll
        for (int rr = 0; rr < 3; ++rr) wv[c2][rr][2] = sp[ci0 + c2][rr][px + 2];
      const float g = sd[px][co];
      if (half == 0) db += g;
#pragma unroll
      for (int k = 0; k < 18; ++k) {
        const int c2 = k / 9, tap = k % 9;
        acc[k] = fmaf(g, wv[c2][tap / 3][tap % 3], acc[k]);
      }
#pragma unroll
      for (int c2 = 0; c2 < 2; ++c2)
#pragma unroll
        for (int rr = 0; rr < 3; ++rr) {
          wv[c2][rr][0] = wv[c2][rr][1];
          wv[c2][rr][1] = wv[c2][rr][2];
        }
    }
  }
  float* o = part + (size_t)blockIdx.x * (128 * 37);
#pragma unroll
  for (int k = 0; k < 18; ++k) o[co * 36 + half * 18 + k] = acc[k];
  if (half == 0) o[128 * 36 + co] = db;
}

hipError_t begin_conv_wgrad(const float* x, const float* dy, float* part, float* dw, float* db, int B, int H, int W,
                            hipStream_t st, bool h16) {
  if (H % BW_ROWS || W % 64) return hipErrorInvalidValue;
  const int nb = B * (H / BW_ROWS) * (W / 64);
  if (h16) hipLaunchKernelGGL(begin_wgrad_kernel<__bf16>, dim3(nb), dim3(256), 0, st, x, SDP_H16(dy), part, H, W);
  else hipLaunchKernelGGL(begin_wgrad_kernel<float>, dim3(nb), dim3(256), 0, st, x, dy, part, H, W);
  (void)sum_rows(part, nb, 128 * 36, 128 * 37, dw, st);
  return sum_rows(part + 128 * 36, nb, 128, 128 * 37, db, st);
}

template <typename TA>
__global__ __launch_bounds__(256) void end_dgrad_kernel(const float* __restrict__ dscore, const float* __restrict__ sigmas,
                                                        const int64_t* __restrict__ labels, const float* __restrict__ w,
                                                        const TA* __restrict__ o, const float* __restrict__ ss,
                                                        TA* __restrict__ g, int H, int W) {
  constexpr int C = 128;
  __shared__ float sd[2][3][66];
  __shared__ float sw[2 * C * 9];
  const int tid = threadIdx.x;
  const int tiles_row = W / 64, per_img = H * tiles_row;
  const int b = blockIdx.x / per_img, t = blockIdx.x % per_img;
  const int y = t / tiles_row, x0 = (t % tiles_row) * 64;
  const float inv = 1.f / sigmas[labels[b]];
  for (int i = tid; i < 2 * 3 * 66; i += 256) {
    const int co = i / 198, rr = (i / 66) % 3, c = i % 66;
    const int yy = y - 1 + rr, xx = x0 - 1 + c;
    sd[co][rr][c] = (yy >= 0 && yy < H && xx >= 0 && xx < W) ? dscore[(((size_t)b * 2 + co) * H + yy) * W + xx] * inv : 0.f;
  }
  for (int i = tid; i < 2 * C * 9; i += 256) sw[i] = w[i];
  __syncthreads();
  const int c4 = tid & 31, pl = tid >> 5;
  const float* ssb = ss + ((size_t)b * C + c4 * 4) * 2;
  const float4 s0 = *reinterpret_cast<const float4*>(ssb), s1 = *reinterpret_cast<const float4*>(ssb + 4);
  for (int px = pl; px < 64; px += 8) {
    float da[4] = {0.f, 0.f, 0.f, 0.f};
#pragma unroll
    for (int co = 0; co < 2; ++co)
#pragma unroll
      for (int tap = 0; tap < 9; ++tap) {
        const int kh = tap / 3, kw = tap % 3;
        const float dv = sd[co][2 - kh][px + 2 - kw];
#pragma unroll
        for (int k = 0; k < 4; ++k) da[k] = fmaf(dv, sw[(co * C + c4 * 4 + k) * 9 + tap], da[k]);
      }
    const size_t idx = (((size_t)b * H + y) * W + x0 + px) * C + c4 * 4;
    const float4 h = ldg4(o, idx);
    const float z0 = fmaf(h.x, s0.x, s0.y), z1 = fmaf(h.y, s0.z, s0.w), z2 = fmaf(h.z, s1.x, s1.y), z3 = fmaf(h.w, s1.z, s1.w);
    stg4(g, idx, make_float4(da[0] * elu_grad(z0, 1), da[1] * elu_grad(z1, 1), da[2] * elu_grad(z2, 1), da[3] * elu_grad(z3, 1)));
  }
}

constexpr int EW_ROWS = 16;
template <typename TA>
__global__ __launch_bounds__(256) void end_wgrad_kernel(const float* __restrict__ dscore, const float* __restrict__ sigmas,
                                                        const int64_t* __restrict__ labels, const TA* __restrict__ o,
                                                        const float* __restrict__ ss, float* __restrict__ part, int H,
                                                        int W) {
  constexpr int C = 128;
  __shared__ float sp[3 * 34 * C];
  __shared__ float sd[2][32];
  const int tid = threadIdx.x, ci = tid >> 1, co = tid & 1;
  const int tiles_row = W / 32, per_img = (H / EW_ROWS) * tiles_row;
  const int b = blockIdx.x / per_img, t = blockIdx.x % per_img;
  const int y0 = (t / tiles_row) * EW_ROWS, x0 = (t % tiles_row) * 32;
  const float inv = 1.f / sigmas[labels[b]];
  const float* ssb = ss + (size_t)b * C * 2;
  float acc[9];
#pragma unroll
  for (int k = 0; k < 9; ++k) acc[k] = 0.f;
  float db = 0.f;
  auto stage_row = [&](int yy) {
    const int slot = (yy - y0 + 1) % 3;
    for (int i = tid; i < 34 * 32; i += 256) {
      const int cc = i >> 5, c4 = i & 31;
      const int xx = x0 - 1 + cc;
      float4 v = make_float4(0.f, 0.f, 0.f, 0.f);
      if (yy >= 0 && yy < H && xx >= 0 && xx < W) {
        const float4 h = ldg4(o, (((size_t)b * H + yy) * W + xx) * C + c4 * 4);
        const float4 s0 = *reinterpret_cast<const float4*>(ssb + c4 * 8), s1 = *reinterpret_cast<const float4*>(ssb + c4 * 8 + 4);
        v = make_float4(elu(fmaf(h.x, s0.x, s0.y)), elu(fmaf(h.y, s0.z, s0.w)), elu(fmaf(h.z, s1.x, s1.y)),
                        elu(fmaf(h.w, s1.z, s1.w)));
      }
      *reinterpret_cast<float4*>(&sp[(slot * 34 + cc) * C + c4 * 4]) = v;
    }
  };
  stage_row(y0 - 1);
  stage_row(y0);
  for (int r = 0; r < EW_ROWS; ++r) {
    const int y = y0 + r;
    stage_row(y + 1);
    if (tid < 64) {
      const int c2 = tid >> 5, px = tid & 31;
      sd[c2][px] = dscore[(((size_t)b * 2 + c2) * H + y) * W + x0 + px] * inv;
    }
    __syncthreads();
    const int sl[3] = {r % 3, (r + 1) % 3, (r + 2) % 3};
    float wv[3][3];
#pragma unroll
    for (int kh = 0; kh < 3; ++kh) {
      wv[kh][0] = sp[(sl[kh] * 34 + 0) * C + ci];
      wv[kh][1] = sp[(sl[kh] * 34 + 1) * C + ci];
    }
    for (int px = 0; px < 32; ++px) {
#pragma unroll
      for (int kh = 0; kh < 3; ++kh) wv[kh][2] = sp[(sl[kh] * 34 + px + 2) * C + ci];
      const float gv = sd[co][px];
      if (ci == 0) db += gv;
#pragma unroll
      for (int tap = 0; tap < 9; ++tap) acc[tap] = fmaf(gv, wv[tap / 3][tap % 3], acc[tap]);
#pragma unroll
      for (int kh = 0; kh < 3; ++kh) {
        wv[kh][0] = wv[kh][1];
        wv[kh][1] = wv[kh][2];
      }
    }
    __syncthreads();
  }
  float* op = part + (size_t)blockIdx.x * (2 * C * 9 + 2);
#pragma unroll
  for (int tap = 0; tap < 9; ++tap) op[(co * C + ci) * 9 + tap] = acc[tap];
  if (ci == 0) op[2 * C * 9 + co] = db;
}

hipError_t end_conv_backward(const float* dscore, const float* sigmas, const int64_t* labels, const float* w,
                             const float* o, const float* ss, float* g, float* part, float* dw, float* db, int B, int H,
                             int W, hipStream_t st, bool h16) {
  if (H % EW_ROWS || W % 64) return hipErrorInvalidValue;
  const int nb = B * (H / EW_ROWS) * (W / 32);
  if (h16) {
    hipLaunchKernelGGL(end_dgrad_kernel<__bf16>, dim3(B * H * (W / 64)), dim3(256), 0, st, dscore, sigmas, labels, w,
                       SDP_H16(o), ss, SDP_H16W(g), H, W);
    hipLaunchKernelGGL(end_wgrad_kernel<__bf16>, dim3(nb), dim3(256), 0, st, dscore, sigmas, labels, SDP_H16(o), ss, part, H, W);
  } else {
    hipLaunchKernelGGL(end_dgrad_kernel<float>, dim3(B * H * (W / 64)), dim3(256), 0, st, dscore, sigmas, labels, w, o, ss, g,
                       H, W);
    hipLaunchKernelGGL(end_wgrad_kernel<float>, dim3(nb), dim3(256), 0, st, dscore, sigmas, labels, o, ss, part, H, W);
  }
  (void)sum_rows(part, nb, 2 * 128 * 9, 2 * 128 * 9 + 2, dw, st);
  return sum_rows(part + 2 * 128 * 9, nb, 2, 2 * 128 * 9 + 2, db, st);
}

size_t head_wgrad_part_floats(int B, int H, int W) {
  const size_t bw = (size_t)B * (H / BW_ROWS) * (W / 64) * 128 * 37;
  const size_t ew = (size_t)B * (H / EW_ROWS) * (W / 32) * (2 * 128 * 9 + 2);
  return bw > ew ? bw : ew;
}

constexpr int DSM_BLK = 64;
__global__ __launch_bounds__(256) void dsm_mask_sum_kernel(const float* __restrict__ mask, int n_img, float* part) {
  __shared__ float red[4];
  const int b = blockIdx.y, tid = threadIdx.x;
  const float* m = mask + (size_t)b * n_img;
  float s = 0.f;
  for (int i = blockIdx.x * 256 + tid; i < n_img; i += DSM_BLK * 256) s += m[i];
  s = wsum(s);
  if ((tid & 63) == 0) red[tid >> 6] = s;
  __syncthreads();
  if (tid == 0) part[b * DSM_BLK + blockIdx.x] = red[0] + red[1] + red[2] + red[3];
}

__global__ __launch_bounds__(256) void dsm_grad_kernel(const float* __restrict__ score, const float* __restrict__ noise,
                                                       const float* __restrict__ mask, const float* __restrict__ used_sigma,
                                                       const float* __restrict__ mpart, int B, int n_img, float power,
                                                       float* __restrict__ dscore, float* __restrict__ lpart) {
  __shared__ double red[4];
  const int b = blockIdx.y, tid = threadIdx.x;
  double np = 0.0;
  for (int k = 0; k < B * DSM_BLK; ++k) np += mpart[k];
  const float sg = used_sigma[b];
  const float inv2 = 1.f / (sg * sg);
  const double scale = (double)n_img / np * pow((double)sg, (double)power) / B;
  const size_t base = (size_t)b * n_img;
  double s = 0.0;
  for (int i = blockIdx.x * 256 + tid; i < n_img; i += DSM_BLK * 256) {
    const float m = mask[base + i];
    const float tgt = -inv2 * noise[base + i];
    const float r = m * (score[base + i] - tgt);
    s += (double)r * r;
    dscore[base + i] = (float)(scale * (double)(m * r));
  }
#pragma unroll
  for (int o = 32; o > 0; o >>= 1) s += __shfl_xor(s, o);
  if ((tid & 63) == 0) red[tid >> 6] = s;
  __syncthreads();
  if (tid == 0) lpart[b * DSM_BLK + blockIdx.x] = (float)(red[0] + red[1] + red[2] + red[3]);
}

__global__ void dsm_final_kernel(const float* __restrict__ mpart, const float* __restrict__ lpart,
                                 const float* __restrict__ used_sigma, int B, int n_img, float power, float* loss,
                                 float* loss_per) {
  if (threadIdx.x != 0 || blockIdx.x != 0) return;
  double np = 0.0;
  for (int k = 0; k < B * DSM_BLK; ++k) np += mpart[k];
  double tot = 0.0;
  for (int b = 0; b < B; ++b) {
    double s = 0.0;
    for (int k = 0; k < DSM_BLK; ++k) s += lpart[b * DSM_BLK + k];
    const double lb = 0.5 * s * n_img / np * pow((double)used_sigma[b], (double)power);
    if (loss_per) loss_per[b] = (float)lb;
    tot += lb;
  }
  *loss = (float)(tot / B);
}

hipError_t dsm_loss(const float* score, const float* noise, const float* mask, const float* used_sigma, int B, int n_img,
                    float power, float* dscore, float* loss, float* loss_per, float* part, hipStream_t st) {
  float* mpart = part;
  float* lpart = part + B * DSM_BLK;
  hipLaunchKernelGGL(dsm_mask_sum_kernel, dim3(DSM_BLK, B), dim3(256), 0, st, mask, n_img, mpart);
  hipLaunchKernelGGL(dsm_grad_kernel, dim3(DSM_BLK, B), dim3(256), 0, st, score, noise, mask, used_sigma, mpart, B, n_img,
                     power, dscore, lpart);
  hipLaunchKernelGGL(dsm_final_kernel, dim3(1), dim3(64), 0, st, mpart, lpart, used_sigma, B, n_img, power, loss, loss_per);
  return hipGetLastError();
}

template <int KIND>
__global__ void optim_ema_kernel(float* __restrict__ p, const float* __restrict__ g, float* __restrict__ s0,
                                 float* __restrict__ s1, float* __restrict__ s2, float* __restrict__ shadow, size_t n,
                                 OptimHyper h) {
  for (size_t i = blockIdx.x * (size_t)blockDim.x + threadIdx.x; i < n; i += (size_t)gridDim.x * blockDim.x) {
    float pi = p[i];
    float gi = g[i];
    if (h.weight_decay != 0.f) gi = gi + h.weight_decay * pi;
    if constexpr (KIND == OPT_ADAM) {
      float mi = s0[i];
      mi = mi + h.omb1 * (gi - mi);
      const float vi = s1[i] * h.b2 + h.omb2 * gi * gi;
      s0[i] = mi;
      s1[i] = vi;
      float vd = vi;
      if (s2) {
        vd = fmaxf(s2[i], vi);
        s2[i] = vd;
      }
      const float denom = sqrtf(vd) / h.bc2_sqrt + h.eps;
      pi = pi - h.step_size * (mi / denom);
    } else if constexpr (KIND == OPT_RMSPROP) {
      const float vi = s0[i] * h.b2 + h.omb2 * gi * gi;
      s0[i] = vi;
      pi = pi - h.step_size * (gi / (sqrtf(vi) + h.eps));
    } else {
      const float bi = h.first ? gi : __fadd_rn(__fmul_rn(s0[i], h.b1), gi);
      s0[i] = bi;
      pi = pi - h.step_size * bi;
    }
    p[i] = pi;
    if (shadow) shadow[i] = h.ommu * pi + h.mu * shadow[i];
  }
}

hipError_t optim_ema(int kind, float* p, const float* g, float* s0, float* s1, float* s2, float* shadow, size_t n,
                     const OptimHyper& h, hipStream_t st) {
  const dim3 grid(grid_for(n)), block(256);
  switch (kind) {
    case OPT_ADAM: hipLaunchKernelGGL(optim_ema_kernel<OPT_ADAM>, grid, block, 0, st, p, g, s0, s1, s2, shadow, n, h); break;
    case OPT_RMSPROP: hipLaunchKernelGGL(optim_ema_kernel<OPT_RMSPROP>, grid, block, 0, st, p, g, s0, s1, s2, shadow, n, h); break;
    case OPT_SGD: hipLaunchKernelGGL(optim_ema_kernel<OPT_SGD>, grid, block, 0, st, p, g, s0, s1, s2, shadow, n, h); break;
    default: return hipErrorInvalidValue;
  }
  return hipGetLastError();
}

}
```

Before: 368.9 image-steps/s.

## Fold 3x3 conv plus 2x2 avg-pool into a 4x4 stride-2 conv

```diff
diff --git a/simultaneous-diffusion-for-pointclouds_amd/csrc/common.h b/simultaneous-diffusion-for-pointclouds_amd/csrc/common.h
--- a/simultaneous-diffusion-for-pointclouds_amd/csrc/common.h
+++ b/simultaneous-diffusion-for-pointclouds_amd/csrc/common.h
@@ -87,6 +87,7 @@
   const float* epi_ss;
   int dact;
   int io16;
+  int s2;
 };
 
 struct WgradArgs {
diff --git a/simultaneous-diffusion-for-pointclouds_amd/csrc/conv.hip b/simultaneous-diffusion-for-pointclouds_amd/csrc/conv.hip
--- a/simultaneous-diffusion-for-pointclouds_amd/csrc/conv.hip
+++ b/simultaneous-diffusion-for-pointclouds_amd/csrc/conv.hip
@@ -70,6 +70,19 @@
   if (!a.circular && d != 1) { *why = "conv: zero padding only for d=1"; return hipErrorInvalidValue; }
   if (!a.pro_ss) { *why = "conv: prologue scale/shift table missing"; return hipErrorInvalidValue; }
   if (a.Cin > 1024 && a.ss_bstride == 0) { *why = "conv: identity table holds 1024 channels"; return hipErrorInvalidValue; }
+  if (a.s2) {
+    if (!sh16 || a.io16 || ks != 3 || pool || d != 1 || a.circular || a.up || a.pro_mode == PRO_NONE || a.dact ||
+        (a.H % 16) || (a.W % 32)) {
+      *why = "conv: the 4x4 stride-2 form needs a bf16 mode, a zero-padded 3x3 with an ELU prologue, H%16 and W%32";
+      return hipErrorInvalidValue;
+    }
+#ifndef SDP_CONV_BENCH_ONLY
+    return mode == MODE_F32X3 ? conv_launch_s2<MODE_F32X3>(a, st) : conv_launch_s2<MODE_BF16>(a, st);
+#else
+    *why = "conv: the 4x4 stride-2 form is not built into conv_bench";
+    return hipErrorInvalidValue;
+#endif
+  }
   if (a.io16) {
 #ifdef SDP_CONV_BENCH_ONLY
     if (mode == MODE_BF16 && ks == 3 && tc == 16 && !pool) return conv_launch_nj2<MODE_BF16, true, 4, true>(a, st);
diff --git a/simultaneous-diffusion-for-pointclouds_amd/csrc/conv_inst.hip b/simultaneous-diffusion-for-pointclouds_amd/csrc/conv_inst.hip
--- a/simultaneous-diffusion-for-pointclouds_amd/csrc/conv_inst.hip
+++ b/simultaneous-diffusion-for-pointclouds_amd/csrc/conv_inst.hip
@@ -60,6 +60,20 @@
   return hipGetLastError();
 }
 
+template <int MODE>
+hipError_t conv_launch_s2(ConvArgs a, hipStream_t st) {
+  using T = ConvTile<1, 16, 3, 4, 2>;
+  const int Ho = a.H / 2, Wo = a.W / 2;
+  a.tiles_per_img = Ho * Wo / (T::TR * 16);
+  a.groups_per_img = Ho * Wo / 128;
+  a.cpair = (SDP_CONV_CPAIR && a.Cout == 2 * T::NTILE) ? 1 : 0;
+  a.strip_w = a.cpair ? conv_strip_w(Ho / T::TR, Wo / 16) : 0;
+  dim3 grid(a.B * a.tiles_per_img * (a.cpair ? 2 : 1), a.cpair ? 1 : a.Cout / T::NTILE);
+  hipLaunchKernelGGL((conv_mfma_kernel<MODE, 1, 16, 3, false, true, true, 16, 4, false, 2, false, true>), grid, dim3(T::NTH),
+                     0, st, a);
+  return hipGetLastError();
+}
+
 template <int MODE, int WM, int TC, int KS, bool ZP, bool IO16>
 hipError_t dgrad_launch(ConvArgs a, hipStream_t st) {
   using T = ConvTile<WM, TC, KS, 4, 4, IO16>;
@@ -111,7 +125,10 @@
 template <> struct DgradShape<4> { static constexpr int WM = 1, TC = 32, KS = 3; static constexpr bool ZP = false; };
 template <> struct DgradShape<5> { static constexpr int WM = 1, TC = 16, KS = 3; static constexpr bool ZP = false; };
 
-#if defined(SDP_INST) && SDP_INST >= 3000
+#if defined(SDP_INST) && SDP_INST >= 4000
+static_assert(SDP_INST - 4000 == MODE_F32X3 || SDP_INST - 4000 == MODE_BF16, "SDP_INST: bad 4x4 stride-2 code");
+template hipError_t conv_launch_s2<SDP_INST - 4000>(ConvArgs, hipStream_t);
+#elif defined(SDP_INST) && SDP_INST >= 3000
 constexpr int kS = SDP_INST % 10;
 static_assert(kS == 0 || kS == 1 || kS == 7 || kS == 8, "SDP_INST: bad IO16 dgrad code");
 #if SDP_INST % 10 == 0
diff --git a/simultaneous-diffusion-for-pointclouds_amd/csrc/conv_kernel.h b/simultaneous-diffusion-for-pointclouds_amd/csrc/conv_kernel.h
--- a/simultaneous-diffusion-for-pointclouds_amd/csrc/conv_kernel.h
+++ b/simultaneous-diffusion-for-pointclouds_amd/csrc/conv_kernel.h
@@ -17,6 +17,10 @@
 #endif
 #ifndef SDP_STORE_AUX16
 #define SDP_STORE_AUX16 SDP_STORE_AUX
+#endif
+
+#ifndef SDP_S2_RING
+#define SDP_S2_RING 4
 #endif
 
 #ifdef SDP_TIMING
@@ -73,8 +77,13 @@
   static constexpr int stage_blk(int q, int Q, int NBLK) { return 2 + q * (NBLK - 2) / (Q > 0 ? Q : 1); }
 };
 
+constexpr int s2_pos(int phase, int t) {
+  const int rho = phase >> 1, gamma = phase & 1;
+  return ((rho ? 0 : 1) + (t >> 1)) * 3 + (gamma ? 0 : 1) + (t & 1);
+}
+
 template <int MODE, int WM, int TC, int KS, bool POOL, bool ZP, bool PELU, int SH = 32, int NW = 4, bool TRN = false,
-          int NJ = 4, bool IO16 = false>
+          int NJ = 4, bool IO16 = false, bool S2 = false>
 __global__ __launch_bounds__(64 * NW, NJ == 2 ? 2 : 1) void conv_mfma_kernel(ConvArgs a) {
 #if defined(__HIP_DEVICE_COMPILE__)
   static_assert(!IO16 || MODE == MODE_BF16, "the bf16 tape runs in bf16 mode");
@@ -86,9 +95,10 @@
   static_assert((SH == 32) == (MODE == MODE_F32), "bf16 modes: 16x16 shape; exact fp32: 32x32");
   static_assert(NW == 4 || (SH == 16 && !POOL), "2-wave workgroups: the 16x16 non-pooled forward only");
   static_assert(NJ == 4 || (SH == 16 && !POOL && KS == 3 && WM == 1), "32-Cout waves: the 16x16 3x3 tiles only");
+  static_assert(!S2 || (NJ == 2 && NW == 4 && TC == 16 && ZP && !TRN && !IO16), "4x4 stride-2: zero-padded 32-Cout-wave tiles");
   using T = ConvTile<WM, TC, KS, NW, NJ, IO16>;
   constexpr int NTH = T::NTH;
-  constexpr int NT = KS * KS;
+  constexpr int NT = S2 ? 4 : KS * KS;
   constexpr bool TRANS = TRN && SH == 16 && !POOL;
   constexpr int NU = T::NU;
   constexpr int XT = NT >= 4 ? 4 : NT;
@@ -103,7 +113,7 @@
 #endif
   SDP_T(0);
   const int wm = WM == 1 ? 0 : (wave & 1), wn = WM == 1 ? wave : (wave >> 1);
-  const int d = a.dil, Hs = a.H / d, Ws = a.W / d;
+  const int d = S2 ? 2 : a.dil, Hs = a.H / d, Ws = a.W / d;
   const int tiles_c = Ws / TC, tiles_rc = (Hs / T::TR) * tiles_c;
   const int nwg = gridDim.x;
   int t = (nwg & 7) ? (int)blockIdx.x : ((int)blockIdx.x & 7) * (nwg >> 3) + ((int)blockIdx.x >> 3);
@@ -130,7 +140,8 @@
   const int wrow0 = wm * T::RW;
 
   const int Cin = a.Cin, Cout = a.Cout;
-  const int nchunks = Cin / 32;
+  const int nck = Cin / 32;
+  const int nchunks = S2 ? 4 * nck : nck;
   const int NB = Cout / 32;
   const int f0 = n0 / 16 + wn * NJ;
   const int nbg0 = f0 / 2;
@@ -158,7 +169,7 @@
       __builtin_amdgcn_make_buffer_rsrc((void*)(c16 ? a.wf16 : a.wf), 0, 0x7fffffff, 0x00020000);
   const int wv0 = ((nbg0 + 0) * 64 + lane) * 64, wv1 = ((nbg0 + 1) * 64 + lane) * 64;
   typedef __attribute__((ext_vector_type(4))) unsigned u32x4;
-  constexpr int NBUF = (NT % 3 == 0) ? 3 : 2;
+  constexpr int NBUF = S2 ? SDP_S2_RING : (NT % 3 == 0) ? 3 : 2;
   uint4 bq[NBUF][NJ / 2][4];
   int wq16[NJ];
   const int wlo16 = __builtin_amdgcn_readfirstlane(c16 ? 1024 : 16);
@@ -196,6 +207,19 @@
 
   const char* inb = reinterpret_cast<const char*>(a.in) + (size_t)b * a.H * a.W * Cin * ES;
   const float* ssb = a.pro_ss + (size_t)b * a.ss_bstride;
+  auto chunk_cc = [&](int c) __attribute__((always_inline)) {
+    if constexpr (S2) return (c >= 2 * nck ? c - 2 * nck : c) >> 1;
+    else return c;
+  };
+  auto chunk_soff = [&](int c) __attribute__((always_inline)) {
+    if constexpr (S2) {
+      c = min(c, nchunks - 1);
+      const int rho = c >= 2 * nck ? 1 : 0, r = c - rho * 2 * nck;
+      return ((rho * a.W + (r & 1)) * Cin + (r >> 1) * 32) * ES;
+    } else {
+      return c * 32 * ES;
+    }
+  };
   const int my_cv = tid & (T::UPP - 1);
   float4 ssv[2][PPU];
   auto load_ss = [&](auto buf, int chunk) __attribute__((always_inline)) {
@@ -233,14 +257,14 @@
     const int base = __builtin_amdgcn_readfirstlane(((tid & ~63) + k * NTH) * 16);
     __builtin_amdgcn_raw_ptr_buffer_load_lds(
         irs, reinterpret_cast<__attribute__((address_space(3))) void*>(reinterpret_cast<uintptr_t>(raw + base)), 16,
-        uoff[k], chunk * 32 * ES, 0, SDP_DMA_AUX);
+        uoff[k], chunk_soff(chunk), 0, SDP_DMA_AUX);
   };
   const i32x4 irs_o = buffer_desc(inb, (uint32_t)(a.H * a.W * Cin * ES));
   auto load_unit_o = [&](auto kc, int chunk) __attribute__((always_inline)) {
     constexpr int k = decltype(kc)::value;
     if constexpr (SDP_KO & 1) return;
     const uint32_t base = (uint32_t)(uintptr_t)(raw + ((tid & ~63) + k * NTH) * 16);
-    dma16_lds_opaque(irs_o, base, uoff[k], chunk * 32 * ES);
+    dma16_lds_opaque(irs_o, base, uoff[k], chunk_soff(chunk));
   };
   auto xform_load = [&](auto kc) __attribute__((always_inline)) {
     constexpr int k = decltype(kc)::value;
@@ -350,7 +374,7 @@
   static_for<0, NU>([&](auto k) { load_unit(k, 0); });
   static_for<0, NU>([&](auto k) { xform_unit(k, std::integral_constant<int, 0>{}); });
   if (nchunks > 1) {
-    load_ss(std::integral_constant<int, 1>{}, 1);
+    load_ss(std::integral_constant<int, 1>{}, chunk_cc(1));
     static_for<0, NU>([&](auto k) { load_unit(k, 1); });
   }
   __syncthreads();
@@ -492,16 +516,16 @@
     tbar += __builtin_amdgcn_s_memtime() - tb0;
 #endif
   };
-  using XP = XformPlan<NU, NT, (MODE == MODE_BF16 && !IO16) ? 8 : 5>;
+  using XP = XformPlan<NU, NT, (MODE == MODE_BF16 && !IO16 && !S2) ? 8 : 5>;
   constexpr int NQ = MODE == MODE_F32X3 ? 8 : 4;
   constexpr int NWL = NJ * (MODE == MODE_F32X3 ? 2 : 1);
   constexpr int NBLK = 8 * NJ;
   static_assert(NQ <= NBLK / 2 && 2 * NWL <= NBLK, "the tap's fillers fit its blocks");
   using I0 = std::integral_constant<int, 0>;
   using I1 = std::integral_constant<int, 1>;
-  auto read_a1 = [&](const char* pat, auto tap_c, auto s_c, auto i_c, auto lo_c) __attribute__((always_inline)) {
-    constexpr int tap = decltype(tap_c)::value, s = decltype(s_c)::value, i = decltype(i_c)::value;
-    constexpr int kh = tap / 3, kw = tap % 3, mb = 4 * s + i;
+  auto read_a1 = [&](const char* pat, auto pos_c, auto s_c, auto i_c, auto lo_c) __attribute__((always_inline)) {
+    constexpr int pos = decltype(pos_c)::value, s = decltype(s_c)::value, i = decltype(i_c)::value;
+    constexpr int kh = pos / 3, kw = pos % 3, mb = 4 * s + i;
     constexpr int mr = mb / (TC / 16), mc = (mb % (TC / 16)) * 16;
     return *reinterpret_cast<const bf16x8*>(pat + ((wrow0 + mr + kh) * T::PC + mc + kw) * PSTRIDE + a_lane_off16 +
                                             (decltype(lo_c)::value ? 64 : 0));
@@ -514,22 +538,26 @@
     const u32x4 v = __builtin_amdgcn_raw_buffer_load_b128(wrs, wq16[nj], so, 0);
     bq[J][nj >> 1][2 * (nj & 1) + part] = make_uint4(v.x, v.y, v.z, v.w);
   };
-  auto do_chunk9 = [&](auto parity, int chunk) __attribute__((always_inline)) {
-    constexpr int P = decltype(parity)::value;
+  auto do_chunk9 = [&](auto parity, auto phase_c, int chunk) __attribute__((always_inline)) {
+    constexpr int P = decltype(parity)::value, PHS = decltype(phase_c)::value;
     const char* pat = lds + P * T::PATCH_BYTES;
     bf16x8 ca[2][4], cb[2][4];
     static_for<0, 4>([&](auto i) {
-      ca[0][i] = read_a1(pat, I0{}, I0{}, i, I0{});
-      if constexpr (MODE == MODE_F32X3) ca[1][i] = read_a1(pat, I0{}, I0{}, i, I1{});
+      using POS0 = std::integral_constant<int, S2 ? s2_pos(PHS, 0) : 0>;
+      ca[0][i] = read_a1(pat, POS0{}, I0{}, i, I0{});
+      if constexpr (MODE == MODE_F32X3) ca[1][i] = read_a1(pat, POS0{}, I0{}, i, I1{});
     });
-    load_ss(std::integral_constant<int, P>{}, min(chunk + 2, nchunks - 1));
+    load_ss(std::integral_constant<int, P>{}, chunk_cc(min(chunk + 2, nchunks - 1)));
     static_for<0, NT>([&](auto tap_c) {
       constexpr int tap = decltype(tap_c)::value;
-      constexpr int CUR = tap % 3, NXT = (tap + 2) % 3;
+      constexpr int DIST = NBUF - 1;
+      constexpr int CUR = tap % NBUF, NXT = (tap + DIST) % NBUF;
+      using POS = std::integral_constant<int, S2 ? s2_pos(PHS, tap) : tap>;
+      using POSN = std::integral_constant<int, S2 ? s2_pos(PHS, tap + 1 < NT ? tap + 1 : 0) : tap + 1>;
       constexpr int U0 = XP::first(tap), UN = XP::count(tap), Q = COPY ? UN : UN * PPU * XP::NSTG;
       constexpr int UNA = UN > 0 ? UN : 1;
-      const int wchunk = tap + 2 < NT ? chunk : min(chunk + 1, nchunks - 1);
-      constexpr int wtap = tap + 2 < NT ? tap + 2 : tap + 2 - NT;
+      const int wchunk = tap + DIST < NT ? chunk : min(chunk + 1, nchunks - 1);
+      constexpr int wtap = tap + DIST < NT ? tap + DIST : tap + DIST - NT;
       float4 xr[UNA];
       float py0[PPU * UNA], py1[PPU * UNA], pe0[PPU * UNA], pe1[PPU * UNA];
       uint32_t phi[PPU * UNA], plo[PPU * UNA];
@@ -655,13 +683,13 @@
         }
         if constexpr (blk < NQ) {
           constexpr int q = blk, ii = MODE == MODE_F32X3 ? (q >> 1) : q, lo = MODE == MODE_F32X3 ? (q & 1) : 0;
-          cb[lo][ii] = read_a1(pat, tap_c, I1{}, std::integral_constant<int, ii>{}, std::integral_constant<int, lo>{});
+          cb[lo][ii] = read_a1(pat, POS{}, I1{}, std::integral_constant<int, ii>{}, std::integral_constant<int, lo>{});
         }
         if constexpr ((blk & 1) && (blk >> 1) < NWL)
           load_b1(std::integral_constant<int, NXT>{}, std::integral_constant<int, (blk >> 1)>{}, wchunk, wtap);
         if constexpr (tap + 1 < NT && blk >= NBLK / 2 && blk < NBLK / 2 + NQ) {
           constexpr int q = blk - NBLK / 2, ii = MODE == MODE_F32X3 ? (q >> 1) : q, lo = MODE == MODE_F32X3 ? (q & 1) : 0;
-          ca[lo][ii] = read_a1(pat, std::integral_constant<int, tap + 1>{}, I0{}, std::integral_constant<int, ii>{},
+          ca[lo][ii] = read_a1(pat, POSN{}, I0{}, std::integral_constant<int, ii>{},
                                std::integral_constant<int, lo>{});
         }
         static_for<0, Q>([&](auto q_c) {
@@ -679,15 +707,26 @@
     __builtin_amdgcn_s_waitcnt(0xc07f);
     if constexpr (!(SDP_KO & 8)) __builtin_amdgcn_s_barrier();
   };
-  static_assert(NT % 2 == 1, "parity bookkeeping assumes an odd tap count");
+  static_assert(NT % 2 == 1 || (S2 && NT % NBUF == 0), "weight-ring slots repeat from chunk to chunk");
 #ifndef SDP_DGRAD16_TAPS
 #define SDP_DGRAD16_TAPS 0
 #endif
-  if constexpr (MODE != MODE_F32 && NT == 9 && (!TRANS || (IO16 && SDP_DGRAD16_TAPS))) {
+  if constexpr (S2) {
+    static_assert(MODE != MODE_F32 && NT % NBUF == 0, "4x4 stride-2: the tap schedule of the bf16 modes");
+    static_assert(XP::max_count() * PPU * XP::NSTG <= 2 * (NBLK - 2), "at most two transform stages per block");
+    for (int chunk = 0; chunk < 2 * nck; chunk += 2) {
+      do_chunk9(I0{}, I0{}, chunk);
+      do_chunk9(I1{}, I1{}, chunk + 1);
+    }
+    for (int chunk = 2 * nck; chunk < nchunks; chunk += 2) {
+      do_chunk9(I0{}, std::integral_constant<int, 2>{}, chunk);
+      do_chunk9(I1{}, std::integral_constant<int, 3>{}, chunk + 1);
+    }
+  } else if constexpr (MODE != MODE_F32 && NT == 9 && (!TRANS || (IO16 && SDP_DGRAD16_TAPS))) {
     static_assert(XP::max_count() * PPU * XP::NSTG <= 2 * (NBLK - 2), "at most two transform stages per block");
     for (int chunk = 0; chunk < nchunks; chunk += 2) {
-      do_chunk9(std::integral_constant<int, 0>{}, chunk);
-      do_chunk9(std::integral_constant<int, 1>{}, chunk + 1);
+      do_chunk9(I0{}, I0{}, chunk);
+      do_chunk9(I1{}, I0{}, chunk + 1);
     }
   } else {
     for (int chunk = 0; chunk < nchunks; chunk += 2) {
@@ -861,7 +900,8 @@
   } else if (SH == 16 && !TRANS && (!a.dact || TC < 32 || NW != 4)) {
     if constexpr (SH == 16 && !TRANS) {
     __builtin_amdgcn_s_waitcnt(0);
-    const int Ho = POOL ? a.H / 2 : a.H, Wo = POOL ? a.W / 2 : a.W;
+    const int Ho = (POOL || S2) ? a.H / 2 : a.H, Wo = (POOL || S2) ? a.W / 2 : a.W;
+    const int de = S2 ? 1 : d;
     const size_t bo = (size_t)b * Ho * Wo * Cout;
     const int img_bytes = Ho * Wo * Cout * ES;
     auto rs = [&](const float* p) {
@@ -874,7 +914,7 @@
     constexpr int NF = POOL ? CB : 8;
     constexpr int PER = POOL ? 2 : 4;
     constexpr int NV = NF * PER;
-    const int xs = (POOL ? 1 : d) * Cout * ES;
+    const int xs = (POOL ? 1 : de) * Cout * ES;
     int vbase[NF];
     static_for<0, NF>([&](auto fc) {
       constexpr int f = decltype(fc)::value;
@@ -883,7 +923,7 @@
         vbase[f] = (((sr0 >> 1) * Wo + ((sc0 + f * 16) >> 1) + 2 * lq) * Cout + co) * ES;
       } else {
         constexpr int mr = f / CB, mc = (f % CB) * 16;
-        const int y = (sr0 + wrow0 + mr) * d + ph_r, x = (sc0 + mc + 4 * lq) * d + ph_c;
+        const int y = (sr0 + wrow0 + mr) * de + ph_r, x = (sc0 + mc + 4 * lq) * de + ph_c;
         vbase[f] = ((y * Wo + x) * Cout + co) * ES;
       }
     });
@@ -945,7 +985,7 @@
           for (int r = 0; r < 4; ++r) v[f * 4 + r] = acc4[f][nj][r] + bias;
         });
       }
-      if (a.up) {
+      if (!S2 && a.up) {
         const int Hi = a.H / 2, Wi = a.W / 2;
         const float shh = (float)(Hi - 1) / (float)(a.H - 1), sww = (float)(Wi - 1) / (float)(a.W - 1);
         const size_t ub = (size_t)b * Hi * Wi * Cout + co;
@@ -954,7 +994,7 @@
         for (int i = 0; i < NV; ++i) {
           const int f = i / PER, k = i % PER;
           const int mr = f / CB, mc = (f % CB) * 16;
-          const int y = (sr0 + wrow0 + mr) * d + ph_r, x = (sc0 + mc + 4 * lq + k) * d + ph_c;
+          const int y = (sr0 + wrow0 + mr) * de + ph_r, x = (sc0 + mc + 4 * lq + k) * de + ph_c;
           const float fy = shh * (float)y, fx = sww * (float)x;
           const int y0 = (int)fy, x0 = (int)fx;
           const int yp = y0 < Hi - 1 ? 1 : 0, xp = x0 < Wi - 1 ? 1 : 0;
diff --git a/simultaneous-diffusion-for-pointclouds_amd/csrc/conv_launch.h b/simultaneous-diffusion-for-pointclouds_amd/csrc/conv_launch.h
--- a/simultaneous-diffusion-for-pointclouds_amd/csrc/conv_launch.h
+++ b/simultaneous-diffusion-for-pointclouds_amd/csrc/conv_launch.h
@@ -13,6 +13,9 @@
 hipError_t conv_launch_nj2(ConvArgs a, hipStream_t st);
 
 template <int MODE>
+hipError_t conv_launch_s2(ConvArgs a, hipStream_t st);
+
+template <int MODE>
 hipError_t dgrad_launch_half(ConvArgs a, hipStream_t st);
 
 template <int MODE, int NW, bool IO16 = false>
diff --git a/simultaneous-diffusion-for-pointclouds_amd/csrc/net.hip b/simultaneous-diffusion-for-pointclouds_amd/csrc/net.hip
--- a/simultaneous-diffusion-for-pointclouds_amd/csrc/net.hip
+++ b/simultaneous-diffusion-for-pointclouds_amd/csrc/net.hip
@@ -39,6 +39,7 @@
     int dil = 1;
     bool circular = true;
     bool pool = false;
+    bool s2 = false;
   };
 
   void conv(const Buf& in, const std::string& wkey, const Buf& out, const Opt& o) {
@@ -46,7 +47,9 @@
     ConvArgs a{};
     a.in = in.p;
     a.wf = net->mode == MODE_F32 ? reinterpret_cast<const uint4*>(net->P(wkey + ".weight#frag")) : nullptr;
-    a.wf16 = net->mode == MODE_F32 ? nullptr : reinterpret_cast<const uint4*>(net->P(wkey + ".weight#frag16"));
+    a.wf16 = net->mode == MODE_F32 ? nullptr
+                                   : reinterpret_cast<const uint4*>(net->P(wkey + (o.s2 ? ".weight#pool4x4" : ".weight#frag16")));
+    a.s2 = o.s2 ? 1 : 0;
     a.bias = o.bias ? net->P(wkey + ".bias") : nullptr;
     a.out = out.p;
     a.res = o.res;
@@ -74,6 +77,11 @@
                 std::to_string(out.C) + " @" + std::to_string(in.H) + "x" + std::to_string(in.W) + " d" +
                 std::to_string(o.dil) + (o.pool ? " pool" : "");
       rec.flops = 2.0 * B * in.H * in.W * (double)in.C * out.C * ks * ks;
+      if (o.s2) {
+        rec.cls = "conv4x4s2 " + std::to_string(in.C) + "->" + std::to_string(out.C) + " @" + std::to_string(in.H) + "x" +
+                  std::to_string(in.W);
+        rec.flops = 2.0 * B * out.H * out.W * (double)in.C * out.C * 16;
+      }
       rec.bytes = 4.0 * B * ((double)in.H * in.W * in.C + (double)out.H * out.W * out.C) + 4.0 * out.C * in.C * ks * ks;
       rec.a = net->event();
       rec.b = net->event();
@@ -118,6 +126,8 @@
                 [&] { chk(maxpool5(X.p, P.p, B, X.H, X.W, X.C, st), "maxpool5"); });
   }
   static int tiles(const Buf& b) { return b.H * b.W / 128; }
+
+  bool pool_as_s2() const { return net->mode != MODE_F32; }
 
   void resblock(const std::string& k, const Buf& x, const Buf& t1, const Buf& t2, const Buf& out, bool down, int dil,
                 bool want_stats, int x_tiles, float x_cnt) {
@@ -140,7 +150,8 @@
       os.circular = false;
       conv(xp, k + ".shortcut.conv", t2, os);
       o2.circular = false;
-      o2.pool = true;
+      o2.pool = !pool_as_s2();
+      o2.s2 = pool_as_s2();
       o2.res = t2.p;
       conv(t1, k + ".conv2.conv", out, o2);
     } else if (down) {
@@ -226,7 +237,8 @@
   f.resblock("res1.0", FA, FB, FD, FC, false, 1, true, H * W / 64, 64.f);
   f.resblock("res1.1", FC, FB, FD, L1, false, 1, true, Fwd::tiles(FC), 128.f);
   f.resblock("res2.0", L1, FB, QA, QB, true, 1, true, Fwd::tiles(L1), 128.f);
-  f.resblock("res2.1", QB, QA, QC, L2, false, 1, true, Fwd::tiles(L1), 32.f);
+  if (f.pool_as_s2()) f.resblock("res2.1", QB, QA, QC, L2, false, 1, true, Fwd::tiles(QB), 128.f);
+  else f.resblock("res2.1", QB, QA, QC, L2, false, 1, true, Fwd::tiles(L1), 32.f);
   f.resblock("res3.0", L2, QA, QB, QC, true, 2, true, Fwd::tiles(L2), 128.f);
   f.resblock("res3.1", QC, QA, QB, L3, false, 2, true, Fwd::tiles(QC), 128.f);
   f.resblock("res4.0", L3, QA, QB, QC, true, 4, true, Fwd::tiles(L3), 128.f);
diff --git a/simultaneous-diffusion-for-pointclouds_amd/csrc/net_internal.h b/simultaneous-diffusion-for-pointclouds_amd/csrc/net_internal.h
--- a/simultaneous-diffusion-for-pointclouds_amd/csrc/net_internal.h
+++ b/simultaneous-diffusion-for-pointclouds_amd/csrc/net_internal.h
@@ -111,6 +111,12 @@
     auto it = host.find(k);
     return it != host.end() && it->second.shape.size() == 4 && k != "begin_conv.weight" && k != "end_conv.weight";
   }
+  bool is_pool3x3_w(const std::string& k) const {
+    static const std::string suffix = ".conv2.conv.weight";
+    auto it = host.find(k);
+    return k.size() > suffix.size() && k.compare(k.size() - suffix.size(), suffix.size(), suffix) == 0 &&
+           it != host.end() && it->second.shape.size() == 4 && it->second.shape[2] == 3 && it->second.shape[3] == 3;
+  }
   std::vector<sdp::PackDesc> pack_host;
   sdp::PackDesc* pack_dev = nullptr;
   size_t pack_dev_n = 0, pack_total = 0;
@@ -120,13 +126,14 @@
     for (auto& kv : host) {
       if (!is_conv_w(kv.first)) continue;
       const auto& s = kv.second.shape;
-      for (int dg = 0; dg < 5; ++dg) {
+      for (int dg = 0; dg < 6; ++dg) {
         if (dg == 0 && mode != sdp::MODE_F32) continue;
         if (dg == 1 || dg == 2) continue;
         if (dg == 3 && mode == sdp::MODE_F32) continue;
         if (dg == 4 && (!train_packs || mode == sdp::MODE_F32)) continue;
-        const std::string fk = kv.first + (dg == 0 ? "#frag" : dg == 3 ? "#frag16" : "#dfrag16");
-        const int nt = (int)(s[2] * s[3]);
+        if (dg == 5 && (mode == sdp::MODE_F32 || !is_pool3x3_w(kv.first))) continue;
+        const std::string fk = kv.first + (dg == 0 ? "#frag" : dg == 3 ? "#frag16" : dg == 4 ? "#dfrag16" : "#pool4x4");
+        const int nt = dg == 5 ? 16 : (int)(s[2] * s[3]);
         const size_t n = (size_t)s[0] * s[1] * nt;
         if (!dev.count(fk)) {
           void* p = nullptr;
diff --git a/simultaneous-diffusion-for-pointclouds_amd/csrc/train_aux.hip b/simultaneous-diffusion-for-pointclouds_amd/csrc/train_aux.hip
--- a/simultaneous-diffusion-for-pointclouds_amd/csrc/train_aux.hip
+++ b/simultaneous-diffusion-for-pointclouds_amd/csrc/train_aux.hip
@@ -58,6 +58,37 @@
   return pk;
 }
 
+SDP_DEV uint32_t pack_slot16p(const float* __restrict__ w, int Cout, int Cin, int mode, size_t i) {
+  const int NF = Cout / 16, nck = Cin / 32;
+  const int word = i & 3;
+  const int lane = (i >> 2) & 63;
+  const int hl = (i >> 8) & 1;
+  size_t r = i >> 9;
+  const int nf = r % NF;
+  r /= NF;
+  const int tap = r % 4;
+  const int ch = (int)(r / 4);
+  const int rho = ch >= 2 * nck ? 1 : 0, rr = ch - rho * 2 * nck, gamma = rr & 1, cc = rr >> 1;
+  const int u = 2 * (tap >> 1) + 1 - rho, v = 2 * (tap & 1) + 1 - gamma;
+  const int co = nf * 16 + (lane & 15);
+  uint32_t pk = 0;
+  for (int e = 0; e < 2; ++e) {
+    const int ci = cc * 32 + 8 * (lane >> 4) + word * 2 + e;
+    const float* w3 = w + ((size_t)co * Cin + ci) * 9;
+    float sum = 0.f;
+    for (int p = 0; p < 2; ++p)
+      for (int q = 0; q < 2; ++q) {
+        const int kh = u - p, kw = v - q;
+        if (kh >= 0 && kh < 3 && kw >= 0 && kw < 3) sum += w3[kh * 3 + kw];
+      }
+    const float f = 0.25f * sum;
+    const __bf16 hi = (__bf16)f;
+    const __bf16 qv = (hl && mode == MODE_F32X3) ? (__bf16)(f - (float)hi) : hi;
+    pk |= (uint32_t)__builtin_bit_cast(uint16_t, qv) << (16 * e);
+  }
+  return pk;
+}
+
 __global__ void pack_weights_kernel(const float* __restrict__ w, uint32_t* __restrict__ out, int Cout, int Cin, int NT,
                                     int mode, int dgrad) {
   const size_t n = (size_t)Cout * Cin * NT;
@@ -69,8 +100,9 @@
   const PackDesc e = d[blockIdx.y];
   const size_t n = (size_t)e.Cout * e.Cin * e.NT;
   for (size_t j = blockIdx.x * (size_t)blockDim.x + threadIdx.x; j < n; j += (size_t)gridDim.x * blockDim.x)
-    e.out[j] = e.dgrad >= 3 ? pack_slot16(e.w, e.Cout, e.Cin, e.NT, mode, e.dgrad == 4, j)
-                            : pack_slot(e.w, e.Cout, e.Cin, e.NT, mode, e.dgrad, j);
+    e.out[j] = e.dgrad == 5   ? pack_slot16p(e.w, e.Cout, e.Cin, mode, j)
+               : e.dgrad >= 3 ? pack_slot16(e.w, e.Cout, e.Cin, e.NT, mode, e.dgrad == 4, j)
+                              : pack_slot(e.w, e.Cout, e.Cin, e.NT, mode, e.dgrad, j);
 }
 
 hipError_t pack_weights_multi(const PackDesc* d, int nd, size_t total, int mode, hipStream_t st) {
```

Result: faster. 375.6 image-steps/s, median of 6 (+1.8%).
